# Ruslan361/iterative_solvers

Hardware: AMD Instinct MI355X
Metric: cg_iters_per_sec (higher is better)
Workload: dtype f64; 1 GPU; 4096x4096 L-shaped Dirichlet Poisson fp64, matrix-free CG, fixed 2641 iterations; n=4096, unknowns=12574721, rule=rel2

## Files before the change

### include/mi355cg.h

```cpp
#ifndef MI355CG_H
#define MI355CG_H

#include <stddef.h>

#ifdef __cplusplus
extern "C" {
#endif

#define MI355CG_OK            0
#define MI355CG_ERR_INVALID   1
#define MI355CG_ERR_HIP       2
#define MI355CG_ERR_STATE     3

#define MI355CG_F64           0
#define MI355CG_F32_MIXED     1

#define MI355CG_RULE_MSG_MAXNORM  0
#define MI355CG_RULE_REL_2NORM    1

#define MI355CG_STOP_ITERATIONS   0
#define MI355CG_STOP_PRECISION    1
#define MI355CG_STOP_RESIDUAL     2
#define MI355CG_STOP_EXACT_ERROR  3
#define MI355CG_STOP_INTERRUPTED  4

typedef struct mi355cg_ctx *mi355cg_handle;

typedef void (*mi355cg_iter_cb)(void *user, int iteration, double precision, double residual, double error);

typedef struct mi355cg_params {
    int    rule;
    int    max_iterations;
    double eps_precision;
    double eps_residual;
    double eps_exact_error;
    double eps_rel;
    int    use_true_solution;
    int    callback_every;
    int    diagnostics;
    int    sync_every;
    int    fixed_iterations;
    double inner_eps;
} mi355cg_params;

typedef struct mi355cg_results {
    int    iterations;
    int    converged;
    int    stop_reason;
    double final_residual_norm;
    double final_precision;
    double final_error_norm;
    double r_norm2;
    double initial_r_norm2;
    double solve_seconds;
    double refine_true_rel;
    int    refine_outer;
    double loop_seconds;
} mi355cg_results;

int  mi355cg_create(int n, int m, double a, double b, double c, double d,
                    int dtype, int device, mi355cg_handle *out);
int  mi355cg_create_csr(long long nrows, const int *row_map, const int *entries, const double *values,
                        int device, mi355cg_handle *out);
int  mi355cg_set_true_solution(mi355cg_handle h, const double *u);
void mi355cg_destroy(mi355cg_handle h);
const char *mi355cg_last_error(void);
const char *mi355cg_version(void);

long long mi355cg_size(mi355cg_handle h);
int  mi355cg_get_rhs(mi355cg_handle h, double *out);
int  mi355cg_get_true_solution(mi355cg_handle h, double *out);
int  mi355cg_get_node_coords(mi355cg_handle h, double *xs, double *ys);
int  mi355cg_set_rhs(mi355cg_handle h, const double *b);
int  mi355cg_setup_on_device(mi355cg_handle h);

int  mi355cg_apply(mi355cg_handle h, const double *x, double *y);
int  mi355cg_apply_device(mi355cg_handle h, const double *x_dev, double *y_dev);

void mi355cg_default_params(mi355cg_params *p, int rule);
int  mi355cg_solve(mi355cg_handle h, const mi355cg_params *params,
                   mi355cg_iter_cb cb, void *user, const volatile int *stop_flag,
                   mi355cg_results *out);
int  mi355cg_get_solution(mi355cg_handle h, double *x);
int  mi355cg_get_recursive_residual(mi355cg_handle h, double *r);
int  mi355cg_get_true_residual(mi355cg_handle h, double *ax_minus_b);

int  mi355cg_set_profiling(mi355cg_handle h, int enable);
int  mi355cg_get_kernel_time(mi355cg_handle h, int kernel, double *avg_ms, long long *launches);
int  mi355cg_get_layout(mi355cg_handle h, long long *padded_len, int *pitch_bottom, int *pitch_upper,
                        int *grid_stencil, int *grid_update, int *rows_per_item);

int  mi355cg_slab_rows(int n, int world, int rank, int *y_lo, int *y_hi);
int  mi355cg_create_part(int n, int m, double a, double b, double c, double d, int dtype, int device,
                         int y_lo, int y_hi, int x_lo, int x_hi, mi355cg_handle *out);
int  mi355cg_checksum(mi355cg_handle h, int which, double *out2);
int  mi355cg_create_slab(int n, int m, double a, double b, double c, double d, int dtype, int device,
                         int y_lo, int y_hi, mi355cg_handle *out);
int  mi355cg_owned_range(mi355cg_handle h, long long *packed_begin, long long *packed_len, int *y_lo, int *y_hi);
int  mi355cg_dist_begin(mi355cg_handle h, const mi355cg_params *params, void *stream);
int  mi355cg_dist_reduce(mi355cg_handle h, int which , int with_rows, void *stream);
int  mi355cg_dist_sums_ptr(mi355cg_handle h, int which, void **dev_ptr, int *count );
int  mi355cg_dist_record_layout(mi355cg_handle h, int *header, int *row_slot, int *width);
int  mi355cg_dist_scatter_ghosts(mi355cg_handle h, int vector ,
                                 const double *gathered_records, int nranks, int rank, void *stream);
int  mi355cg_dist_stencil(mi355cg_handle h, const double *gathered_update_sums, int nranks, int estride,
                          int rows , void *stream);
int  mi355cg_dist_flip(mi355cg_handle h);
int  mi355cg_dist_update(mi355cg_handle h, const double *gathered_stencil_sums, int nranks, int estride,
                         int rows , void *stream);
int  mi355cg_dist_update_reads_ghosts(mi355cg_handle h);
int  mi355cg_dist_check(mi355cg_handle h, const double *gathered_update_sums, int nranks, int estride, void *stream);
int  mi355cg_dist_summary(mi355cg_handle h, mi355cg_results *out, int *done);
int  mi355cg_dist_finish(mi355cg_handle h, void *stream);
int  mi355cg_dist_history(mi355cg_handle h, int iteration, double *precision, double *residual, double *error);
int  mi355cg_dist_halo(mi355cg_handle h, int vector ,
                       void **send_lo, void **recv_lo, long long *n_send_lo,
                       void **send_hi, void **recv_hi, long long *n_send_hi);
int  mi355cg_dist_halo_recv_counts(mi355cg_handle h, long long *n_from_lo, long long *n_from_hi);

#define MI355CG_DECOMP_ROWS 0
#define MI355CG_DECOMP_2D   1
typedef struct mi355cg_team_s *mi355cg_team;
typedef struct mi355cg_halo_msg {
    int id;
    int peer;
    int send;
    int kind;
    int y0, y1, x0, x1;
    long long count;
} mi355cg_halo_msg;
int  mi355cg_decompose(int n, int world, int decomp, int rank, int *y_lo, int *y_hi, int *x_lo, int *x_hi);
int  mi355cg_halo_plan(int n, int world, int decomp, int rank, int max_msgs, int *n_msgs, mi355cg_halo_msg *msgs);
int  mi355cg_debug_plan(int n, int world, int decomp, int rank, int which, int *n_panels, int *panels,
                        int *grid, int *n_items, int *cls);
int  mi355cg_team_create_local(int n, int m, double a, double b, double c, double d, int world,
                               const int *devices, int ndevices, int decomp, mi355cg_team *out);
int  mi355cg_team_unique_id(void *id128);
int  mi355cg_team_create_rccl(int n, int m, double a, double b, double c, double d, int world, int rank, int device,
                              const void *id128, int decomp, mi355cg_team *out);
void mi355cg_team_destroy(mi355cg_team t);
int  mi355cg_team_solve(mi355cg_team t, const mi355cg_params *params, mi355cg_iter_cb cb, void *user,
                        const volatile int *stop_flag, mi355cg_results *out);
int  mi355cg_team_info(mi355cg_team t, int *world, int *nlocal, int *decomp, long long *size);
int  mi355cg_team_describe(mi355cg_team t, char *buf, int len);
int  mi355cg_team_part(mi355cg_team t, int local_index, mi355cg_handle *part, int *rank);
int  mi355cg_team_get_vector(mi355cg_team t, int which, double *global_packed);
int  mi355cg_team_checksum(mi355cg_team t, int which, double *out2);
int  mi355cg_team_set_vector(mi355cg_team t, int which, const double *global_packed);
int  mi355cg_team_set_dtype(mi355cg_team t, int dtype);
int  mi355cg_team_setup_on_device(mi355cg_team t);
int  mi355cg_team_set_profiling(mi355cg_team t, int enable);
int  mi355cg_team_phase_times(mi355cg_team t, double *kernel_ms, double *comm_ms, double *wall_ms);

#ifdef __cplusplus
}
#endif
#endif
```

### iterative_solvers_amd/_capi.py

```python
from __future__ import annotations

import ctypes as C
import os

import numpy as np

from . import build as _build

OK, ERR_INVALID, ERR_HIP, ERR_STATE = 0, 1, 2, 3
F64, F32_MIXED = 0, 1
RULE_MSG_MAXNORM, RULE_REL_2NORM = 0, 1
STOP_ITERATIONS, STOP_PRECISION, STOP_RESIDUAL, STOP_EXACT_ERROR, STOP_INTERRUPTED = range(5)

EXPORTS = [
    "mi355cg_create", "mi355cg_create_csr", "mi355cg_set_true_solution", "mi355cg_destroy", "mi355cg_last_error", "mi355cg_version", "mi355cg_size",
    "mi355cg_get_rhs", "mi355cg_get_true_solution", "mi355cg_get_node_coords", "mi355cg_set_rhs",
    "mi355cg_apply", "mi355cg_apply_device", "mi355cg_default_params", "mi355cg_solve",
    "mi355cg_get_solution", "mi355cg_get_recursive_residual", "mi355cg_get_true_residual",
    "mi355cg_set_profiling", "mi355cg_get_kernel_time", "mi355cg_get_layout",
    "mi355cg_slab_rows", "mi355cg_create_slab", "mi355cg_owned_range", "mi355cg_dist_begin",
    "mi355cg_dist_reduce", "mi355cg_dist_sums_ptr", "mi355cg_dist_record_layout", "mi355cg_dist_scatter_ghosts", "mi355cg_dist_stencil", "mi355cg_dist_flip",
    "mi355cg_dist_update", "mi355cg_dist_update_reads_ghosts", "mi355cg_dist_check", "mi355cg_dist_summary", "mi355cg_dist_finish", "mi355cg_dist_history",
    "mi355cg_dist_halo", "mi355cg_dist_halo_recv_counts",
    "mi355cg_create_part", "mi355cg_checksum", "mi355cg_decompose", "mi355cg_halo_plan",
    "mi355cg_team_create_local", "mi355cg_team_unique_id", "mi355cg_team_create_rccl", "mi355cg_team_destroy",
    "mi355cg_team_solve", "mi355cg_team_info", "mi355cg_team_part", "mi355cg_team_get_vector", "mi355cg_team_set_vector", "mi355cg_team_checksum",
    "mi355cg_team_set_profiling", "mi355cg_team_phase_times", "mi355cg_team_describe", "mi355cg_setup_on_device", "mi355cg_team_setup_on_device", "mi355cg_debug_plan",
    "mi355cg_team_set_dtype",
]
DECOMP_ROWS, DECOMP_2D = 0, 1


class Params(C.Structure):
    _fields_ = [("rule", C.c_int), ("max_iterations", C.c_int),
                ("eps_precision", C.c_double), ("eps_residual", C.c_double),
                ("eps_exact_error", C.c_double), ("eps_rel", C.c_double),
                ("use_true_solution", C.c_int), ("callback_every", C.c_int),
                ("diagnostics", C.c_int), ("sync_every", C.c_int), ("fixed_iterations", C.c_int),
                ("inner_eps", C.c_double)]


class Results(C.Structure):
    _fields_ = [("iterations", C.c_int), ("converged", C.c_int), ("stop_reason", C.c_int),
                ("final_residual_norm", C.c_double), ("final_precision", C.c_double),
                ("final_error_norm", C.c_double), ("r_norm2", C.c_double),
                ("initial_r_norm2", C.c_double), ("solve_seconds", C.c_double),
                ("refine_true_rel", C.c_double), ("refine_outer", C.c_int), ("loop_seconds", C.c_double)]


class HaloMsg(C.Structure):
    _fields_ = [("id", C.c_int), ("peer", C.c_int), ("send", C.c_int), ("kind", C.c_int),
                ("y0", C.c_int), ("y1", C.c_int), ("x0", C.c_int), ("x1", C.c_int), ("count", C.c_longlong)]


ITER_CB = C.CFUNCTYPE(None, C.c_void_p, C.c_int, C.c_double, C.c_double, C.c_double)
_DP = np.ctypeslib.ndpointer(dtype=np.float64, flags="C_CONTIGUOUS")

_lib = None


class Mi355cgError(RuntimeError):
    def __init__(self, code: int, text: str):
        super().__init__(f"mi355cg error {code}: {text}")
        self.code = code


def lib_path() -> str:
    return _build.LIB_PATH


def load():
    global _lib
    if _lib is not None:
        return _lib
    path = os.environ.get("MI355CG_LIB") or _build.LIB_PATH
    if path == _build.LIB_PATH and _build.needs_build():
        try:
            _build.build()
        except Exception as e:
            if not os.path.exists(path):
                raise RuntimeError(f"libmi355cg.so is missing and could not be built: {e}") from e
    try:
        import torch
    except ImportError:
        pass
    L = C.CDLL(path)
    H = C.c_void_p
    L.mi355cg_create.argtypes = [C.c_int, C.c_int] + [C.c_double] * 4 + [C.c_int, C.c_int, C.POINTER(H)]
    _IPn = np.ctypeslib.ndpointer(dtype=np.int32, flags="C_CONTIGUOUS")
    L.mi355cg_create_csr.argtypes = [C.c_longlong, _IPn, _IPn, _DP, C.c_int, C.POINTER(H)]
    L.mi355cg_set_true_solution.argtypes = [H, _DP]
    L.mi355cg_destroy.argtypes = [H]
    L.mi355cg_destroy.restype = None
    L.mi355cg_last_error.restype = C.c_char_p
    L.mi355cg_version.restype = C.c_char_p
    L.mi355cg_size.argtypes = [H]
    L.mi355cg_size.restype = C.c_longlong
    for name in ("mi355cg_get_rhs", "mi355cg_get_true_solution", "mi355cg_set_rhs",
                 "mi355cg_get_solution", "mi355cg_get_recursive_residual", "mi355cg_get_true_residual"):
        getattr(L, name).argtypes = [H, _DP]
    L.mi355cg_get_node_coords.argtypes = [H, _DP, _DP]
    L.mi355cg_apply.argtypes = [H, _DP, _DP]
    L.mi355cg_apply_device.argtypes = [H, C.c_void_p, C.c_void_p]
    L.mi355cg_default_params.argtypes = [C.POINTER(Params), C.c_int]
    L.mi355cg_default_params.restype = None
    L.mi355cg_solve.argtypes = [H, C.POINTER(Params), ITER_CB, C.c_void_p, C.c_void_p, C.POINTER(Results)]
    L.mi355cg_set_profiling.argtypes = [H, C.c_int]
    L.mi355cg_get_kernel_time.argtypes = [H, C.c_int, C.POINTER(C.c_double), C.POINTER(C.c_longlong)]
    L.mi355cg_get_layout.argtypes = [H, C.POINTER(C.c_longlong)] + [C.POINTER(C.c_int)] * 5
    LLP, IP, VPP = C.POINTER(C.c_longlong), C.POINTER(C.c_int), C.POINTER(C.c_void_p)
    L.mi355cg_slab_rows.argtypes = [C.c_int, C.c_int, C.c_int, IP, IP]
    L.mi355cg_create_slab.argtypes = [C.c_int, C.c_int] + [C.c_double] * 4 + [C.c_int] * 4 + [C.POINTER(H)]
    L.mi355cg_owned_range.argtypes = [H, LLP, LLP, IP, IP]
    L.mi355cg_dist_begin.argtypes = [H, C.POINTER(Params), C.c_void_p]
    L.mi355cg_dist_reduce.argtypes = [H, C.c_int, C.c_int, C.c_void_p]
    L.mi355cg_dist_sums_ptr.argtypes = [H, C.c_int, VPP, IP]
    L.mi355cg_dist_record_layout.argtypes = [H, IP, IP, IP]
    L.mi355cg_dist_scatter_ghosts.argtypes = [H, C.c_int, C.c_void_p, C.c_int, C.c_int, C.c_void_p]
    L.mi355cg_dist_stencil.argtypes = [H, C.c_void_p, C.c_int, C.c_int, C.c_int, C.c_void_p]
    L.mi355cg_dist_flip.argtypes = [H]
    L.mi355cg_dist_update.argtypes = [H, C.c_void_p, C.c_int, C.c_int, C.c_int, C.c_void_p]
    L.mi355cg_dist_update_reads_ghosts.argtypes = [H]
    L.mi355cg_dist_check.argtypes = [H, C.c_void_p, C.c_int, C.c_int, C.c_void_p]
    L.mi355cg_dist_summary.argtypes = [H, C.POINTER(Results), IP]
    L.mi355cg_dist_finish.argtypes = [H, C.c_void_p]
    DBP = C.POINTER(C.c_double)
    L.mi355cg_dist_history.argtypes = [H, C.c_int, DBP, DBP, DBP]
    L.mi355cg_dist_halo.argtypes = [H, C.c_int, VPP, VPP, LLP, VPP, VPP, LLP]
    L.mi355cg_dist_halo_recv_counts.argtypes = [H, LLP, LLP]
    L.mi355cg_create_part.argtypes = [C.c_int, C.c_int] + [C.c_double] * 4 + [C.c_int] * 6 + [C.POINTER(H)]
    L.mi355cg_checksum.argtypes = [H, C.c_int, DBP]
    L.mi355cg_decompose.argtypes = [C.c_int] * 4 + [IP] * 4
    L.mi355cg_halo_plan.argtypes = [C.c_int] * 5 + [IP, C.POINTER(HaloMsg)]
    L.mi355cg_team_create_local.argtypes = [C.c_int, C.c_int] + [C.c_double] * 4 + [C.c_int, IP, C.c_int, C.c_int, C.POINTER(H)]
    L.mi355cg_team_unique_id.argtypes = [C.c_void_p]
    L.mi355cg_team_create_rccl.argtypes = [C.c_int, C.c_int] + [C.c_double] * 4 + [C.c_int, C.c_int, C.c_int, C.c_void_p, C.c_int, C.POINTER(H)]
    L.mi355cg_team_destroy.argtypes = [H]
    L.mi355cg_team_destroy.restype = None
    L.mi355cg_team_solve.argtypes = [H, C.POINTER(Params), ITER_CB, C.c_void_p, C.c_void_p, C.POINTER(Results)]
    L.mi355cg_team_info.argtypes = [H, IP, IP, IP, LLP]
    L.mi355cg_team_part.argtypes = [H, C.c_int, C.POINTER(H), IP]
    L.mi355cg_team_get_vector.argtypes = [H, C.c_int, _DP]
    L.mi355cg_team_set_vector.argtypes = [H, C.c_int, _DP]
    L.mi355cg_team_checksum.argtypes = [H, C.c_int, DBP]
    L.mi355cg_debug_plan.argtypes = [C.c_int] * 5 + [IP, IP, IP, IP, IP]
    L.mi355cg_setup_on_device.argtypes = [H]
    L.mi355cg_team_setup_on_device.argtypes = [H]
    L.mi355cg_team_set_dtype.argtypes = [H, C.c_int]
    L.mi355cg_team_set_profiling.argtypes = [H, C.c_int]
    L.mi355cg_team_phase_times.argtypes = [H, DBP, DBP, DBP]
    L.mi355cg_team_describe.argtypes = [H, C.c_char_p, C.c_int]
    _lib = L
    return L


def check(rc: int):
    if rc != OK:
        raise Mi355cgError(rc, load().mi355cg_last_error().decode("utf-8", "replace"))
```

### iterative_solvers_amd/csrc/cg_kernels.h

```cpp
#pragma once
#include <hip/hip_runtime.h>
#include <cfloat>
#include <cmath>

namespace mi355cg {

constexpr int kBlock = 256;
constexpr int kWave = 64;
constexpr int kWaves = kBlock / kWave;
constexpr int kHist = 512;
constexpr int kMaxPanels = 8;
constexpr int kRing = 8;

#ifdef MI355CG_WAVE_TIMING
constexpr int kWtWaves = 16384, kWtStamps = 6;
__device__ unsigned long long g_wave_dbg[2][kWtStamps * kWtWaves];
#define MI355CG_WT_BEGIN unsigned long long wt_[kWtStamps]; for (int i_ = 0; i_ < kWtStamps; ++i_) wt_[i_] = 0; wt_[0] = wall_clock64();
#define MI355CG_WT_STAMP(I) wt_[I] = wall_clock64();
#define MI355CG_WT_MID wt_[kWtStamps - 2] = wall_clock64();
#define MI355CG_WT_END(K) do { if ((threadIdx.x & 63) == 0) { const int w_ = blockIdx.x * 4 + threadIdx.x / 64; \
    if (w_ < kWtWaves) { wt_[kWtStamps - 1] = wall_clock64(); for (int i_ = 0; i_ < kWtStamps; ++i_) g_wave_dbg[K][kWtStamps * w_ + i_] = wt_[i_]; } } } while (0)
#else
#define MI355CG_WT_BEGIN
#define MI355CG_WT_STAMP(I)
#define MI355CG_WT_MID
#define MI355CG_WT_END(K)
#endif

struct Geom {
    int N, half, cb, xlim;
    int Pb, Pu;
    int y_lo, y_hi;
    long long base0;
    long long own_begin, own_len;
    double A, xk, yk;
};

__host__ __device__ inline long long row_off(const Geom& g, int y) {
    return y <= g.half ? (long long)y * g.Pb - g.cb
                       : (long long)(g.half + 1) * g.Pb + (long long)(y - g.half - 1) * g.Pu;
}
__host__ __device__ inline bool node_interior(const Geom& g, int x, int y) {
    return y >= 1 && y <= g.N - 1 && x <= g.N - 1 && x >= (y <= g.half ? g.half + 1 : 1);
}

struct Panel { int y0, y1, s0, ns, ty, nchunks, item0, gc; };
constexpr int kXcds = 8;
struct WorkList { Panel p[kMaxPanels]; int np; int nitems; int ncls; int cls0[kXcds + 1]; };
struct ItemSeq { int first, step, begin, end; };
__device__ inline ItemSeq item_seq(const WorkList& wl, int wave) {
    if (wl.ncls == kXcds) {
        const int cls = blockIdx.x % kXcds, nb = (gridDim.x - cls + kXcds - 1) / kXcds;
        int begin = wl.cls0[0], end = wl.cls0[1];
#pragma unroll
        for (int k = 1; k < kXcds; ++k) if (k == cls) { begin = wl.cls0[k]; end = wl.cls0[k + 1]; }
        return ItemSeq{begin + (int)(blockIdx.x / kXcds) * kWaves + wave, nb * kWaves, begin, end};
    }
    return ItemSeq{(int)blockIdx.x * kWaves + wave, (int)gridDim.x * kWaves, 0, wl.nitems};
}

struct CgState {
    double alpha, beta;
    double rr;
    double rr_prev;
    double rz;
    double r0norm;
    double rnorm2;
    double rmax, dmax, emax, d2, e2;
    int it, done, reason, converged, first;
    int stop;
    double alpha_hist[kRing];
};
struct HistEntry { double dmax, rmax, emax, rnorm2, d2, e2, tr2; };

struct StateLite { double alpha, rr, rr_prev, rz, r0norm; int it, done, first, stop; };
template <typename V> __device__ inline V scalar_load(const V* p) {
    return *(const __attribute__((address_space(4))) V*)p;
}
__device__ __attribute__((noinline)) void copy_state(CgState* dst, const CgState* src) { *dst = *src; }
__device__ inline StateLite load_state_lite(const CgState* p) {
    StateLite L;
    L.alpha = scalar_load(&p->alpha); L.rr = scalar_load(&p->rr); L.rr_prev = scalar_load(&p->rr_prev);
    L.rz = scalar_load(&p->rz); L.r0norm = scalar_load(&p->r0norm);
    L.it = scalar_load(&p->it); L.done = scalar_load(&p->done); L.first = scalar_load(&p->first); L.stop = scalar_load(&p->stop);
    return L;
}

struct RuleParams {
    int rule;
    int max_iterations;
    double eps_precision, eps_residual, eps_exact_error, eps_rel;
    int use_u;
    int fixed_iterations;
};

enum { FA_PAP = 0, FA_RZ = 1, FA_LO = 2, FA_COUNT = 4 };
enum { FB_RR = 0, FB_D2 = 1, FB_E2 = 2, FB_LO = 3, FB_RMAX = 6, FB_DMAX = 7, FB_EMAX = 8, FB_COUNT = 9 };
constexpr int kNumSumsA = 2, kNumSumsB = 3;
constexpr int FB_STOP = FB_COUNT, FB_LL_COUNT = FB_COUNT + 1;

struct dd { double hi, lo; };
__device__ inline dd dd_zero() { return dd{0.0, 0.0}; }
__device__ inline dd two_sum(double a, double b) { const double s = a + b, bb = s - a; return dd{s, (a - (s - bb)) + (b - bb)}; }
__device__ inline dd dd_add(dd a, dd b) {
    const dd s = two_sum(a.hi, b.hi);
    const double lo = s.lo + (a.lo + b.lo);
    const double hi = s.hi + lo;
    return dd{hi, lo - (hi - s.hi)};
}
__device__ inline void dd_acc_prod(dd& acc, double a, double b) {
#ifdef MI355CG_PLAIN_DOT
    acc.hi += a * b;
#elif defined(MI355CG_DOT2)
    const double p = a * b;
    const dd s = two_sum(acc.hi, p);
    acc.hi = s.hi;
    acc.lo += s.lo + fma(a, b, -p);
#else
    const double p = a * b;
    acc = dd_add(acc, dd{p, fma(a, b, -p)});
#endif
}
__device__ inline double dd_value(dd a) { return a.hi + a.lo; }

__device__ inline double wave_sum(double v) {
#pragma unroll
    for (int o = 32; o > 0; o >>= 1) v += __shfl_down(v, o, kWave);
    return v;
}
__device__ inline double wave_max(double v) {
#pragma unroll
    for (int o = 32; o > 0; o >>= 1) v = fmax(v, __shfl_down(v, o, kWave));
    return v;
}
template <bool IS_MAX>
__device__ inline double block_reduce(double v, double* lds ) {
    v = IS_MAX ? wave_max(v) : wave_sum(v);
    const int lane = threadIdx.x & (kWave - 1), w = threadIdx.x / kWave;
    __syncthreads();
    if (lane == 0) lds[w] = v;
    __syncthreads();
    double t = lds[0];
// ... 3 lines not shown
}
template <bool IS_MAX>
__device__ inline double reduce_parts(const double* __restrict__ part, int n, int es, double* lds) {
    double v = 0.0;
    for (int i = threadIdx.x; i < n; i += kBlock) v = IS_MAX ? fmax(v, part[(long long)i * es]) : v + part[(long long)i * es];
    return block_reduce<IS_MAX>(v, lds);
}

__device__ inline dd wave_sum_dd(dd v) {
#pragma unroll
    for (int o = 32; o > 0; o >>= 1) v = dd_add(v, dd{__shfl_down(v.hi, o, kWave), __shfl_down(v.lo, o, kWave)});
    return v;
}
__device__ inline dd block_reduce_dd(dd v, double* lds) {
    v = wave_sum_dd(v);
    const int lane = threadIdx.x & (kWave - 1), w = threadIdx.x / kWave;
    __syncthreads();
    if (lane == 0) { lds[2 * w] = v.hi; lds[2 * w + 1] = v.lo; }
    __syncthreads();
    dd t{lds[0], lds[1]};
#pragma unroll
    for (int k = 1; k < kWaves; ++k) t = dd_add(t, dd{lds[2 * k], lds[2 * k + 1]});
    return t;
}
struct PreParts { double hi0, lo0, hi1, lo1; };
__device__ inline PreParts prefetch_parts(const double* __restrict__ part_hi, const double* __restrict__ part_lo, int n, int es) {
    PreParts p{0.0, 0.0, 0.0, 0.0};
    const int i0 = threadIdx.x, i1 = threadIdx.x + kBlock;
    if (i0 < n) { p.hi0 = part_hi[(long long)i0 * es]; p.lo0 = part_lo[(long long)i0 * es]; }
    if (i1 < n) { p.hi1 = part_hi[(long long)i1 * es]; p.lo1 = part_lo[(long long)i1 * es]; }
    return p;
}
__device__ inline dd reduce_parts_dd_pre(const PreParts& pre, const double* __restrict__ part_hi, const double* __restrict__ part_lo, int n, int es, double* lds) {
    dd v = dd_zero();
    if ((int)threadIdx.x < n) v = dd_add(v, dd{pre.hi0, pre.lo0});
    if ((int)threadIdx.x + kBlock < n) v = dd_add(v, dd{pre.hi1, pre.lo1});
    for (int i = threadIdx.x + 2 * kBlock; i < n; i += kBlock) v = dd_add(v, dd{part_hi[(long long)i * es], part_lo[(long long)i * es]});
    return block_reduce_dd(v, lds);
}
struct PreMax { double v0, v1; };
__device__ inline PreMax prefetch_max(const double* __restrict__ part, int n, int es) {
    PreMax p{0.0, 0.0};
    if ((int)threadIdx.x < n) p.v0 = part[(long long)threadIdx.x * es];
    if ((int)threadIdx.x + kBlock < n) p.v1 = part[(long long)(threadIdx.x + kBlock) * es];
    return p;
}
template <bool IS_MAX> __device__ inline double block_reduce(double v, double* lds);
__device__ inline double reduce_max_pre(const PreMax& pre, const double* __restrict__ part, int n, int es, double* lds) {
    double v = fmax(pre.v0, pre.v1);
    for (int i = threadIdx.x + 2 * kBlock; i < n; i += kBlock) v = fmax(v, part[(long long)i * es]);
    return block_reduce<true>(v, lds);
}
__device__ inline dd reduce_parts_dd(const double* __restrict__ part_hi, const double* __restrict__ part_lo, int n, int es, double* lds) {
    dd v = dd_zero();
    for (int i = threadIdx.x; i < n; i += kBlock) v = dd_add(v, dd{part_hi[(long long)i * es], part_lo[(long long)i * es]});
    return block_reduce_dd(v, lds);
}

struct Decision { int done, reason, converged; double beta, rr, rnorm2, r0norm, rmax, dmax, emax, d2, e2; };

__device__ inline Decision decide_after_update(const StateLite& s, const RuleParams& rp, double rr, double rmax,
                                               double dmax, double emax, double d2, double e2, bool stop = false) {
    Decision d;
    d.rr = rr; d.rnorm2 = sqrt(rr); d.rmax = rmax; d.dmax = dmax; d.emax = emax; d.d2 = d2; d.e2 = e2;
    d.r0norm = s.first ? d.rnorm2 : s.r0norm;
    d.done = 0; d.reason = 0 ; d.converged = 0; d.beta = 0.0;
    if (rp.rule == 1 ) {
        const bool go = s.it < rp.max_iterations && (rp.fixed_iterations || d.rnorm2 > rp.eps_rel * d.r0norm);
        if (!go) { d.done = 1; d.converged = d.rnorm2 <= rp.eps_rel * d.r0norm; }
        if (!s.first) d.beta = rr / s.rr;
    } else {
        if (s.it >= 1 && !rp.fixed_iterations) {
            if (rp.eps_precision > 0 && dmax < rp.eps_precision) { d.done = 1; d.converged = 1; d.reason = 1; }
            else if (rp.eps_residual > 0 && rmax < rp.eps_residual) { d.done = 1; d.converged = 1; d.reason = 2; }
            else if (rp.eps_exact_error > 0 && rp.use_u && emax < rp.eps_exact_error) { d.done = 1; d.converged = 1; d.reason = 3; }
        }
        if (!d.done && !(s.it < rp.max_iterations)) d.done = 1;
        if (!s.first) d.beta = (d.rnorm2 * d.rnorm2) / s.rz;
    }
    if (!d.done && (stop || s.stop)) { d.done = 1; d.reason = 4 ; d.converged = 0; }
    return d;
}

__device__ inline void write_state_after_decision(CgState* out, HistEntry* hist, const CgState* in, const StateLite& s, const Decision& d) {
    copy_state(out, in);
    CgState* o = out;
    o->rr_prev = s.rr; o->rr = d.rr; o->rnorm2 = d.rnorm2; o->r0norm = d.r0norm; o->beta = d.beta;
    o->rmax = d.rmax; o->dmax = d.dmax; o->emax = d.emax; o->d2 = d.d2; o->e2 = d.e2;
    o->done = d.done; o->reason = d.reason; o->converged = d.converged;
    if (hist) {
        HistEntry* h = hist + (s.it % kHist);
        h->dmax = d.dmax; h->rmax = d.rmax; h->emax = d.emax; h->rnorm2 = d.rnorm2; h->d2 = d.d2; h->e2 = d.e2;
    }
}

__device__ inline Decision reduce_and_decide(const StateLite& s, const RuleParams& rp, const double* partB,
                                             int nB, int strideB, int esB, int want_diag, double* lds, const PreParts* pre_rr = nullptr,
                                             const PreMax* pre_max = nullptr ) {
    const double rr = pre_rr ? dd_value(reduce_parts_dd_pre(*pre_rr, partB + FB_RR * strideB, partB + (FB_RR + FB_LO) * strideB, nB, esB, lds))
                             : dd_value(reduce_parts_dd(partB + FB_RR * strideB, partB + (FB_RR + FB_LO) * strideB, nB, esB, lds));
    double rmax = 0, dmax = 0, emax = 0, d2 = 0, e2 = 0;
    if (rp.rule == 0 || want_diag) {
        if (pre_max) {
            rmax = reduce_max_pre(pre_max[0], partB + FB_RMAX * strideB, nB, esB, lds);
            dmax = reduce_max_pre(pre_max[1], partB + FB_DMAX * strideB, nB, esB, lds);
            if (rp.use_u) emax = reduce_max_pre(pre_max[2], partB + FB_EMAX * strideB, nB, esB, lds);
        } else {
            rmax = reduce_parts<true>(partB + FB_RMAX * strideB, nB, esB, lds);
            dmax = reduce_parts<true>(partB + FB_DMAX * strideB, nB, esB, lds);
            if (rp.use_u) emax = reduce_parts<true>(partB + FB_EMAX * strideB, nB, esB, lds);
        }
    }
    if (want_diag) {
        d2 = dd_value(reduce_parts_dd(partB + FB_D2 * strideB, partB + (FB_D2 + FB_LO) * strideB, nB, esB, lds));
        if (rp.use_u) e2 = dd_value(reduce_parts_dd(partB + FB_E2 * strideB, partB + (FB_E2 + FB_LO) * strideB, nB, esB, lds));
    }
    return decide_after_update(s, rp, rr, rmax, dmax, emax, d2, e2);
}
typedef unsigned long long u64;
constexpr int kRecWords = 16;
constexpr int kLLWords = 2 * kRecWords;
constexpr int kRecStopWord = 9;
constexpr int kMaxRecDst = 16;
constexpr int kReasonTransport = 5;
constexpr int kMaxPartSlots = 1024;
__device__ inline u64 ld_sys(const u64* p) { return __hip_atomic_load(p, __ATOMIC_RELAXED, __HIP_MEMORY_SCOPE_SYSTEM); }
__device__ inline void st_sys(u64* p, u64 v) { __hip_atomic_store(p, v, __ATOMIC_RELAXED, __HIP_MEMORY_SCOPE_SYSTEM); }
__device__ inline u64 flagged(unsigned stamp, unsigned data) { return ((u64)stamp << 32) | data; }

struct FlagSpec {
    u64* part;
    unsigned stamp;
};
__device__ inline void store_flagged(const FlagSpec& fs, int slot, int nfields, const double* v) {
    u64* w = fs.part + (long long)slot * (2 * nfields);
    for (int f = 0; f < nfields; ++f) {
        const u64 bits = __builtin_bit_cast(u64, v[f]);
        st_sys(w + 2 * f, flagged(fs.stamp, (unsigned)bits));
        st_sys(w + 2 * f + 1, flagged(fs.stamp, (unsigned)(bits >> 32)));
    }
}
__device__ inline void store_flagged_zero(const FlagSpec& fs, int slot, int nfields) {
    if (!fs.part) return;
    u64* w = fs.part + (long long)slot * (2 * nfields);
    for (int k = 0; k < 2 * nfields; ++k) st_sys(w + k, flagged(fs.stamp, 0u));
}

struct RecSpec {
    int ndst;
    u64* const* dst;
    u64* const* flag;
    int slot_words;
    int slot;
    unsigned seq;
    u64 flag_value;
};
struct RecSrc {
    const u64* mbox;
    int world, me;
    unsigned stamp;
    u64 budget;
};
__device__ inline bool gather_records(const RecSrc& src, double* recs) {
    unsigned* out = reinterpret_cast<unsigned*>(recs);
    const int n = src.world * kLLWords;
    int bad = 0;
    for (int i = threadIdx.x; i < n; i += kBlock) {
        if (i / kLLWords == src.me) continue;
        u64 v = ld_sys(src.mbox + i);
        if ((unsigned)(v >> 32) != src.stamp) {
            const u64 t0 = wall_clock64();
            unsigned spins = 0;
            for (;;) {
                __builtin_amdgcn_s_sleep(2);
                v = ld_sys(src.mbox + i);
                if ((unsigned)(v >> 32) == src.stamp) break;
// ... 181 lines not shown
    if constexpr (sizeof(V) == 16) return __builtin_bit_cast(V, __builtin_amdgcn_raw_buffer_load_b128(r, voff, soff, 0));
    else if constexpr (sizeof(V) == 8) return __builtin_bit_cast(V, __builtin_amdgcn_raw_buffer_load_b64(r, voff, soff, 0));
    else { static_assert(sizeof(V) == 4, "buf_load: 4, 8 or 16 bytes"); return __builtin_bit_cast(V, __builtin_amdgcn_raw_buffer_load_b32(r, voff, soff, 0)); }
}
template <typename V> __device__ inline void buf_store(V v, rsrc_t r, int voff, int soff) {
    typedef unsigned int u4 __attribute__((ext_vector_type(4)));
    typedef unsigned int u2 __attribute__((ext_vector_type(2)));
    if constexpr (sizeof(V) == 16) {
        u4 d = __builtin_bit_cast(u4, v);
        __builtin_amdgcn_raw_buffer_store_b128(d, r, voff, soff, 0);
        asm volatile("s_nop 1" : "+v"(d));
    }
    else if constexpr (sizeof(V) == 8) __builtin_amdgcn_raw_buffer_store_b64(__builtin_bit_cast(u2, v), r, voff, soff, 0);
    else { static_assert(sizeof(V) == 4, "buf_store: 4, 8 or 16 bytes"); __builtin_amdgcn_raw_buffer_store_b32(__builtin_bit_cast(unsigned int, v), r, voff, soff, 0); }
}
__device__ inline int dpp_from_below(int v) { return __builtin_amdgcn_update_dpp(0, v, 0x138 , 0xf, 0xf, false); }
__device__ inline int dpp_from_above(int v) { return __builtin_amdgcn_update_dpp(0, v, 0x130 , 0xf, 0xf, false); }
__device__ inline float lane_below(float v) { return __builtin_bit_cast(float, dpp_from_below(__builtin_bit_cast(int, v))); }
__device__ inline float lane_above(float v) { return __builtin_bit_cast(float, dpp_from_above(__builtin_bit_cast(int, v))); }
__device__ inline double lane_below(double v) {
    const unsigned long long u = __builtin_bit_cast(unsigned long long, v);
    const unsigned lo = (unsigned)dpp_from_below((int)(unsigned)u), hi = (unsigned)dpp_from_below((int)(unsigned)(u >> 32));
    return __builtin_bit_cast(double, ((unsigned long long)hi << 32) | lo);
}
__device__ inline double lane_above(double v) {
    const unsigned long long u = __builtin_bit_cast(unsigned long long, v);
    const unsigned lo = (unsigned)dpp_from_above((int)(unsigned)u), hi = (unsigned)dpp_from_above((int)(unsigned)(u >> 32));
    return __builtin_bit_cast(double, ((unsigned long long)hi << 32) | lo);
}
template <typename T> __device__ inline int row_step(const Geom& g, int y) { return (y + 1 <= g.half ? g.Pb : g.Pu) * (int)sizeof(T); }

template <typename T> __device__ inline int lane_off(const Geom& g, int x, bool bottom_row) {
    return (x < g.xlim && x >= (bottom_row ? g.cb : 0)) ? x * (int)sizeof(T) : kOob;
}
template <typename T, int VEC> __device__ inline int edge_off(const Geom& g, int x, int lane, bool bottom_row) {
    const int xe = lane == 0 ? x - 1 : x + VEC;
    const bool edge = lane == 0 || lane == kWave - 1;
    return (edge && xe >= (bottom_row ? g.cb : 0) && xe < g.xlim) ? xe * (int)sizeof(T) : kOob;
}

struct Item { int strip, ya, yb, gc; };
__device__ inline Item decode_item(const WorkList& wl, int item) {
    Panel P = wl.p[0];
#pragma unroll
    for (int k = 1; k < kMaxPanels; ++k) if (k < wl.np && item >= wl.p[k].item0) P = wl.p[k];
    const int local = item - P.item0;
    const int chunk = local / P.ns;
    Item it;
    it.strip = P.s0 + (local - chunk * P.ns);
    it.ya = P.y0 + chunk * P.ty;
    it.yb = min(P.y1, it.ya + P.ty - 1);
    it.gc = (it.strip == P.s0 ? (P.gc & 1) : 0) | (it.strip == P.s0 + P.ns - 1 ? (P.gc & 2) : 0);
    return it;
}

struct ItemAddr {
    int nrows, ystart;
    long long base_el;
    int so_first, so_c0;
    int gc; bool bot;
    int x;
    int vo_own, ve_own, vo_first, vo_last;
};
template <typename T, int VEC, bool DESC>
__device__ inline ItemAddr item_addr(const Geom& g, const Item& it, int lane) {
    constexpr int DIR = DESC ? -1 : 1;
    ItemAddr A;
    A.x = it.strip * (kWave * VEC) + lane * VEC;
    A.nrows = it.yb - it.ya + 1;
    A.ystart = DESC ? it.yb : it.ya;
    const int y0 = it.ya - 1;
    A.base_el = row_off(g, y0) - g.base0;
    A.bot = it.ya <= g.half;
    A.vo_own = lane_off<T>(g, A.x, A.bot);
    A.ve_own = edge_off<T, VEC>(g, A.x, lane, A.bot);
    A.vo_first = lane_off<T>(g, A.x, A.ystart - DIR <= g.half);
    A.vo_last = lane_off<T>(g, A.x, A.ystart + DIR * A.nrows <= g.half);
    A.so_first = DESC ? (int)((row_off(g, it.yb + 1) - row_off(g, y0)) * (long long)sizeof(T)) : 0;
    A.so_c0 = DESC ? (int)((row_off(g, it.yb) - row_off(g, y0)) * (long long)sizeof(T)) : row_step<T>(g, y0);
    A.gc = it.gc;
    return A;
}

template <typename T, int VEC, bool FUSED, bool MSG, int DEPTH, bool NOAP, bool GC>
__global__ __launch_bounds__(kBlock) void k_stencil(const StencilArgs<T> a) {
    static_assert(DEPTH >= 1 && DEPTH <= 3, "the compute cursor takes its item from the fetch cursor: DEPTH <= rows fetched per item (>= 3)");
    typedef typename VecOf<T, VEC>::type vec_t;
    __shared__ double lds[2 * kWaves];
    const Geom& g = a.g;
    const int lane = threadIdx.x & (kWave - 1);
    const int wave = __builtin_amdgcn_readfirstlane(threadIdx.x / kWave);
    const ItemSeq seq = item_seq(a.wl, wave);
    MI355CG_WT_BEGIN
    struct Raw { vec_t r, p; T re, pe; };

    int f_item = seq.first;
    bool f_have = f_item < seq.end;
    ItemAddr F{};
    int f_idx = 0, f_so = 0, f_y = 0;
    rsrc_t rs_p = make_rsrc(a.pin), rs_r = make_rsrc(a.pin);
    const int dq_nsub = min(kQueueSubs, (int)(gridDim.x / kXcds)), dq_sub = (int)(blockIdx.x / kXcds) % dq_nsub;
    int* const dq = a.dq.mine ? a.dq.mine + ((int)(blockIdx.x % kXcds) * kQueueSubs + dq_sub) * kQueuePitch : nullptr;
    if (a.dq.other && blockIdx.x == 0 && threadIdx.x < kXcds * kQueueSubs) a.dq.other[threadIdx.x * kQueuePitch] = 0;
    int dq_ticket = 0;
    auto enter = [&](int item) {
        if (dq) dq_ticket = queue_take(dq, lane);
        F = item_addr<T, VEC, false>(g, decode_item(a.wl, item), lane);
        rs_p = make_rsrc(a.pin + F.base_el);
        rs_r = make_rsrc(FUSED ? a.r + F.base_el : a.pin + F.base_el);
        f_idx = -1; f_so = F.so_first; f_y = F.ystart - 1;
    };
    auto fetch = [&]() -> Raw {
        if (f_have && f_idx > F.nrows) {
            f_item = dq ? seq.begin + seq.step + __builtin_amdgcn_readfirstlane(dq_ticket) * dq_nsub + dq_sub : f_item + seq.step;
            f_have = f_item < seq.end;
            if (f_have) enter(f_item);
        }
        const bool own = f_idx >= 0 && f_idx < F.nrows;
        int vo = own ? F.vo_own : (f_idx < 0 ? F.vo_first : F.vo_last);
        int ve = own ? F.ve_own : kOob;
        if (!f_have) { vo = kOob; ve = kOob; }
        Raw w;
        w.p = buf_load<vec_t>(rs_p, vo, f_so);
        if (FUSED) w.r = buf_load<vec_t>(rs_r, vo, f_so);
        else for (int j = 0; j < VEC; ++j) w.r[j] = (T)0;
        w.pe = buf_load<T>(rs_p, ve, f_so);
        if (FUSED) w.re = buf_load<T>(rs_r, ve, f_so); else w.re = (T)0;
        f_so += row_step<T>(g, f_y); ++f_y; ++f_idx;
        return w;
    };

    bool c_have = f_have;
    ItemAddr C{};
    int c_idx = -1, c_so = 0, c_y = 0, c_ve_gc = kOob;
    bool in_j[VEC];
#pragma unroll
    for (int j = 0; j < VEC; ++j) in_j[j] = false;
    rsrc_t rs_po = make_rsrc(a.pin), rs_ap = make_rsrc(a.pin);
    auto promote = [&]() {
        C = F;
        rs_po = make_rsrc(FUSED ? a.pout + C.base_el : a.pin + C.base_el);
        rs_ap = make_rsrc(NOAP ? a.pin + C.base_el : a.ap + C.base_el);
        c_idx = -1; c_so = C.so_c0; c_y = C.ystart;
        const int xint0 = C.bot ? g.half + 1 : 1;
#pragma unroll
        for (int j = 0; j < VEC; ++j) in_j[j] = (C.x + j >= xint0) && (C.x + j <= g.N - 1);
        if (GC) c_ve_gc = ((lane == 0 && (C.gc & 1)) || (lane == kWave - 1 && (C.gc & 2))) ? C.ve_own : kOob;
    };

    if (f_have) { enter(f_item); promote(); }
    Raw q[DEPTH];
#pragma unroll
    for (int k = 0; k < DEPTH; ++k) q[k] = fetch();

    T beta = (T)0;
    if (FUSED && a.src.mbox) {
        __shared__ double recs[kMaxRecDst * kRecWords];
        const PreParts pre = prefetch_parts(a.partB + FB_RR * a.strideB, a.partB + (FB_RR + FB_LO) * a.strideB, a.nB, 1);
        PreMax pmax[3] = {{0, 0}, {0, 0}, {0, 0}};
        if (MSG) {
#pragma unroll
            for (int k = 0; k < 3; ++k) pmax[k] = prefetch_max(a.partB + (FB_RMAX + k) * a.strideB, a.nB, 1);
        }
        const StateLite s = load_state_lite(a.s_in);
        if (s.done) {
            if (threadIdx.x == 0) { store_flagged_zero(a.fl, a.slotA + blockIdx.x, FA_COUNT); if (blockIdx.x == 0) copy_state(a.s_out, a.s_in); }
            return;
        }
        MI355CG_WT_STAMP(1)
        own_record_B(recs, a.src.me, a.partB, a.nB, a.strideB, MSG ? 1 : 0, lds, &pre, MSG ? pmax : nullptr);
        if (!gather_records(a.src, recs)) {
            if (threadIdx.x == 0) { store_flagged_zero(a.fl, a.slotA + blockIdx.x, FA_COUNT); if (blockIdx.x == 0) fail_transport(a.s_out, a.s_in); }
            return;
        }
        const Decision d = decide_from_records(s, a.rp, recs, a.src.world, MSG, false);
        MI355CG_WT_STAMP(2)
        if (blockIdx.x == 0 && threadIdx.x == 0) write_state_after_decision(a.s_out, a.hist, a.s_in, s, d);
        if (d.done) { if (threadIdx.x == 0) store_flagged_zero(a.fl, a.slotA + blockIdx.x, FA_COUNT); return; }
        beta = (T)d.beta;
    } else if (FUSED) {
        const PreParts pre = prefetch_parts(a.partB + FB_RR * a.strideB, a.partB + (FB_RR + FB_LO) * a.strideB, a.nB, a.esB);
        PreMax pmax[3] = {{0, 0}, {0, 0}, {0, 0}};
        if (MSG) {
#pragma unroll
            for (int k = 0; k < 3; ++k) pmax[k] = prefetch_max(a.partB + (FB_RMAX + k) * a.strideB, a.nB, a.esB);
        }
        const StateLite s = load_state_lite(a.s_in);
        if (s.done) { if (blockIdx.x == 0 && threadIdx.x == 0) copy_state(a.s_out, a.s_in); return; }
        MI355CG_WT_STAMP(1)
        const Decision d = reduce_and_decide(s, a.rp, a.partB, a.nB, a.strideB, a.esB, a.want_diag, lds, &pre, MSG ? pmax : nullptr);
        MI355CG_WT_STAMP(2)
        if (blockIdx.x == 0 && threadIdx.x == 0) write_state_after_decision(a.s_out, a.hist, a.s_in, s, d);
        if (d.done) return;
        beta = (T)d.beta;
    }

    MI355CG_WT_MID
    const T cA = (T)g.A, cxk = (T)g.xk, cyk = (T)g.yk;
    dd acc_pap = dd_zero(), acc_rz = dd_zero();
    auto is_ghost = [&](int yy) { return (yy == g.y_lo - 1 || yy == g.y_hi + 1) && yy >= 1 && yy <= g.N - 1; };
    vec_t pn_b, pn_c, r_c;
    T pne_c = (T)0;
#pragma unroll
    for (int j = 0; j < VEC; ++j) { pn_b[j] = (T)0; pn_c[j] = (T)0; r_c[j] = (T)0; }

    while (c_have) {
#pragma unroll
        for (int k = 0; k < DEPTH; ++k) {
            if (c_have) {
                const Raw w = q[k];
                q[k] = fetch();
                vec_t pn; T pne;
                if (FUSED) {
#pragma unroll
                    for (int j = 0; j < VEC; ++j) pn[j] = w.r[j] + beta * w.p[j];
                    pne = w.re + beta * w.pe;
                } else { pn = w.p; pne = w.pe; }

                if (c_idx < 0) {
                    pn_b = pn;
                    if (FUSED && a.store_ghosts && is_ghost(C.ystart - 1)) buf_store(pn, rs_po, C.vo_first, C.so_first);
                } else if (c_idx == 0) {
                    pn_c = pn; pne_c = pne; r_c = w.r;
                } else {
                    T left0 = lane_below(pn_c[VEC - 1]);
                    T rightL = lane_above(pn_c[0]);
                    if (lane == 0) left0 = pne_c;
                    if (lane == kWave - 1) rightL = pne_c;
                    vec_t out;
#pragma unroll
                    for (int j = 0; j < VEC; ++j) {
                        const T c = pn_c[j];
                        const T L = j == 0 ? left0 : pn_c[j - 1];
                        const T R = j == VEC - 1 ? rightL : pn_c[j + 1];
                        T v = cA * c;
                        v = v + cxk * L;
                        v = v + cxk * R;
                        v = v + cyk * pn[j];
                        v = v + cyk * pn_b[j];
                        out[j] = in_j[j] ? v : (T)0;
                        dd_acc_prod(acc_pap, (double)c, (double)out[j]);
                        if (MSG) dd_acc_prod(acc_rz, (double)r_c[j], (double)c);
                    }
                    if (!NOAP) buf_store(out, rs_ap, C.vo_own, c_so);
                    if (FUSED) buf_store(pn_c, rs_po, C.vo_own, c_so);
                    if (FUSED && GC) buf_store(pne_c, rs_po, c_ve_gc, c_so);
                    c_so += row_step<T>(g, c_y); ++c_y;
                    pn_b = pn_c; pn_c = pn; pne_c = pne; r_c = w.r;
                }
                if (c_idx == C.nrows) {
                    if (FUSED && a.store_ghosts && is_ghost(c_y)) buf_store(pn, rs_po, C.vo_last, c_so);
                    c_have = f_have;
                    if (c_have) promote();
                } else ++c_idx;
            }
        }
    }

    MI355CG_WT_END(0);
    const dd tp = block_reduce_dd(acc_pap, lds);
    dd tz = dd_zero();
    if (MSG) tz = block_reduce_dd(acc_rz, lds);
    if (threadIdx.x == 0 && a.partA) {
        const int b = a.slotA + blockIdx.x, st = a.strideA;
        a.partA[FA_PAP * st + b] = tp.hi; a.partA[(FA_PAP + FA_LO) * st + b] = tp.lo;
        a.partA[FA_RZ * st + b] = tz.hi;  a.partA[(FA_RZ + FA_LO) * st + b] = tz.lo;
        if (FUSED && a.fl.part) { const double v[FA_COUNT] = {tp.hi, tz.hi, tp.lo, tz.lo}; store_flagged(a.fl, b, FA_COUNT, v); }
    }
}

template <typename T>
struct UpdateArgs {
    long long begin, nvec;
    T* x; T* r; const T* p; const T* ap; const T* u;
    const double* partA; int nA, strideA, esA;
    double* partB; int strideB;
    const CgState* s_in; CgState* s_out;
    int rule;
    int init;
    double r0norm_resume;
};

template <typename T, int VEC, bool HAS_U>
__global__ __launch_bounds__(kBlock) void k_update(const UpdateArgs<T> a) {
    typedef typename VecOf<T, VEC>::type vec_t;
    __shared__ double lds[2 * kWaves];
    StateLite s{};
    double alpha_d = 0.0, rz = 0.0;
    if (a.init == 1) {
        s.first = 1; s.it = 0;
    } else if (a.init == 2) {
        s = load_state_lite(a.s_in);
    } else {
        s = load_state_lite(a.s_in);
        if (s.done) { if (blockIdx.x == 0 && threadIdx.x == 0) copy_state(a.s_out, a.s_in); return; }
        const double pap = dd_value(reduce_parts_dd(a.partA + FA_PAP * a.strideA, a.partA + (FA_PAP + FA_LO) * a.strideA, a.nA, a.esA, lds));
        if (a.rule == 0) {
            rz = dd_value(reduce_parts_dd(a.partA + FA_RZ * a.strideA, a.partA + (FA_RZ + FA_LO) * a.strideA, a.nA, a.esA, lds));
            alpha_d = rz / pap;
        } else {
            alpha_d = s.rr / pap;
        }
    }
    const T alpha = (T)alpha_d;

    dd s_rr = dd_zero(), s_d2 = dd_zero(), s_e2 = dd_zero();
    double s_rmax = 0, s_dmax = 0, s_emax = 0;
    const long long stride = (long long)gridDim.x * kBlock;
    vec_t* __restrict__ X = reinterpret_cast<vec_t*>(a.x);
    vec_t* __restrict__ R = reinterpret_cast<vec_t*>(a.r);
    const vec_t* __restrict__ Pp = reinterpret_cast<const vec_t*>(a.p);
    const vec_t* __restrict__ Q = reinterpret_cast<const vec_t*>(a.ap);
    const vec_t* __restrict__ Uu = reinterpret_cast<const vec_t*>(a.u);

    auto elem = [&](long long i, const vec_t& x0, const vec_t& pv, const vec_t& r0, const vec_t& qv, const vec_t& uv) {
        vec_t xn, rn;
#pragma unroll
        for (int j = 0; j < VEC; ++j) {
            xn[j] = x0[j] + alpha * pv[j];
            rn[j] = r0[j] - alpha * qv[j];
            const double rd = (double)rn[j];
            dd_acc_prod(s_rr, rd, rd);
            s_rmax = fmax(s_rmax, fabs(rd));
            const double dx = (double)(xn[j] - x0[j]);
            s_dmax = fmax(s_dmax, fabs(dx));
            dd_acc_prod(s_d2, dx, dx);
            if (HAS_U) {
                const double ee = (double)(xn[j] - uv[j]);
                s_emax = fmax(s_emax, fabs(ee));
                dd_acc_prod(s_e2, ee, ee);
            }
        }
        X[i] = xn; R[i] = rn;
    };
    long long i = a.begin + (long long)blockIdx.x * kBlock + threadIdx.x;
    const long long end = a.begin + a.nvec;
    for (; i + stride < end; i += 2 * stride) {
        const long long j0 = i, j1 = i + stride;
        const vec_t xa = X[j0], pa = Pp[j0], ra = R[j0], qa = Q[j0];
        const vec_t xb = X[j1], pb = Pp[j1], rb = R[j1], qb = Q[j1];
// ... 27 lines not shown
            } else {
                copy_state(a.s_out, a.s_in);
                if (a.init == 2) {
                    if (s.done) o->rr = s.rr_prev;
                    o->done = 0; o->reason = 0; o->converged = 0; o->alpha = 0.0; o->r0norm = a.r0norm_resume;
                    for (int i = 0; i < kRing; ++i) o->alpha_hist[i] = 0.0;
                } else { o->it = s.it + 1; o->first = 0; o->alpha = alpha_d; o->rz = rz; o->alpha_hist[(s.it + 1) & (kRing - 1)] = alpha_d; }
            }
        }
    }
}

template <typename T>
struct FreshArgs {
    long long begin, nvec;
    const T* b; T* x; T* r; T* p0; const T* u;
    double* partB; int strideB;
    CgState* s_out;
};
template <typename T, int VEC, bool HAS_U>
__global__ __launch_bounds__(kBlock) void k_init_fresh(const FreshArgs<T> a) {
    typedef typename VecOf<T, VEC>::type vec_t;
    __shared__ double lds[2 * kWaves];
    dd s_rr = dd_zero(), s_e2 = dd_zero();
    double s_rmax = 0, s_emax = 0;
    const long long stride = (long long)gridDim.x * kBlock;
    const vec_t* __restrict__ B = reinterpret_cast<const vec_t*>(a.b);
    const vec_t* __restrict__ Uu = reinterpret_cast<const vec_t*>(a.u);
    vec_t* __restrict__ X = reinterpret_cast<vec_t*>(a.x);
    vec_t* __restrict__ R = reinterpret_cast<vec_t*>(a.r);
    vec_t* __restrict__ P = reinterpret_cast<vec_t*>(a.p0);
    vec_t zero;
#pragma unroll
    for (int j = 0; j < VEC; ++j) zero[j] = (T)0;
    const long long end = a.begin + a.nvec;
    for (long long i = a.begin + (long long)blockIdx.x * kBlock + threadIdx.x; i < end; i += stride) {
        const vec_t bv = B[i];
        vec_t uv; if (HAS_U) uv = Uu[i];
#pragma unroll
        for (int j = 0; j < VEC; ++j) {
            const double rd = (double)bv[j];
            dd_acc_prod(s_rr, rd, rd);
            s_rmax = fmax(s_rmax, fabs(rd));
            if (HAS_U) {
                const double ee = (double)((T)0 - uv[j]);
                s_emax = fmax(s_emax, fabs(ee));
                dd_acc_prod(s_e2, ee, ee);
            }
        }
        X[i] = zero; R[i] = bv; P[i] = zero;
    }
    const dd t_rr = block_reduce_dd(s_rr, lds);
    const double t_rmax = block_reduce<true>(s_rmax, lds);
    double t_emax = 0; dd t_e2 = dd_zero();
    if (HAS_U) { t_emax = block_reduce<true>(s_emax, lds); t_e2 = block_reduce_dd(s_e2, lds); }
    if (threadIdx.x == 0) {
        const int b = blockIdx.x, st = a.strideB;
        a.partB[FB_RR * st + b] = t_rr.hi; a.partB[(FB_RR + FB_LO) * st + b] = t_rr.lo;
        a.partB[FB_D2 * st + b] = 0.0; a.partB[(FB_D2 + FB_LO) * st + b] = 0.0;
        a.partB[FB_E2 * st + b] = t_e2.hi; a.partB[(FB_E2 + FB_LO) * st + b] = t_e2.lo;
        a.partB[FB_RMAX * st + b] = t_rmax; a.partB[FB_DMAX * st + b] = 0.0; a.partB[FB_EMAX * st + b] = t_emax;
        if (blockIdx.x == 0) { *a.s_out = CgState{}; a.s_out->first = 1; }
    }
}

template <typename T>
struct UpdateStArgs {
    Geom g;
    WorkList wl;
    const T* p;
    const T* pprev[kRing - 1];
    T* r; T* x; const T* u;
    const double* partA; int nA, strideA, esA;
    RecSrc src;
    double* partB; int strideB, slotB;
    const CgState* s_in; CgState* s_out;
    int rule;
    int reverse;
    const int* stop_req;
    FlagSpec fl;
    QueueSpec dq;
};

template <typename T, int VEC, int XM, bool HAS_U, int DEPTH, bool DESC>
__global__ __launch_bounds__(kBlock) void k_update_st(const UpdateStArgs<T> a) {
    static_assert(DEPTH >= 1 && DEPTH <= 3, "see k_stencil");
    typedef typename VecOf<T, VEC>::type vec_t;
    __shared__ double lds[2 * kWaves];
    const Geom& g = a.g;
    const int lane = threadIdx.x & (kWave - 1);
    const int wave = __builtin_amdgcn_readfirstlane(threadIdx.x / kWave);
    const ItemSeq seq = item_seq(a.wl, wave);
    MI355CG_WT_BEGIN
    int stop_word = 0;
    if (blockIdx.x == 0 && a.stop_req) stop_word = scalar_load(a.stop_req);
    constexpr bool FULL = XM == 1;
    constexpr int NP = XM >= 2 ? XM - 1 : 0;
    struct Raw { vec_t p, r, x, u, pp[NP > 0 ? NP : 1]; T pe; };

    int f_item = seq.first;
    bool f_have = f_item < seq.end;
    ItemAddr F{};
    int f_idx = 0, f_so = 0, f_y = 0;
    rsrc_t rs_p = make_rsrc(a.p), rs_r = rs_p, rs_x = rs_p, rs_u = rs_p;
    rsrc_t rs_pp[NP > 0 ? NP : 1] = {rs_p};
    const int dq_nsub = min(kQueueSubs, (int)(gridDim.x / kXcds)), dq_sub = (int)(blockIdx.x / kXcds) % dq_nsub;
    int* const dq = a.dq.mine ? a.dq.mine + ((int)(blockIdx.x % kXcds) * kQueueSubs + dq_sub) * kQueuePitch : nullptr;
    if (a.dq.other && blockIdx.x == 0 && threadIdx.x < kXcds * kQueueSubs) a.dq.other[threadIdx.x * kQueuePitch] = 0;
    int dq_ticket = 0;
    auto enter = [&](int idx) {
        if (dq) dq_ticket = queue_take(dq, lane);
        F = item_addr<T, VEC, DESC>(g, decode_item(a.wl, a.reverse ? seq.end - 1 - (idx - seq.begin) : idx), lane);
        rs_p = make_rsrc(a.p + F.base_el);
        rs_r = make_rsrc(a.r + F.base_el);
        rs_x = make_rsrc(XM != 0 ? a.x + F.base_el : a.p + F.base_el);
#pragma unroll
        for (int i = 0; i < NP; ++i) rs_pp[i] = make_rsrc(a.pprev[i] + F.base_el);
        rs_u = make_rsrc((FULL && HAS_U) ? a.u + F.base_el : a.p + F.base_el);
        f_idx = -1; f_so = F.so_first; f_y = DESC ? F.ystart + 1 : F.ystart - 1;
    };
    auto fetch = [&]() -> Raw {
        if (f_have && f_idx > F.nrows) {
            f_item = dq ? seq.begin + seq.step + __builtin_amdgcn_readfirstlane(dq_ticket) * dq_nsub + dq_sub : f_item + seq.step;
            f_have = f_item < seq.end;
            if (f_have) enter(f_item);
        }
        const bool own = f_have && f_idx >= 0 && f_idx < F.nrows;
        int vo = own ? F.vo_own : (f_idx < 0 ? F.vo_first : F.vo_last);
        if (!f_have) vo = kOob;
        const int vown = own ? F.vo_own : kOob;
        Raw w;
        w.p = buf_load<vec_t>(rs_p, vo, f_so);
        w.r = buf_load<vec_t>(rs_r, vown, f_so);
        if (XM != 0) w.x = buf_load<vec_t>(rs_x, vown, f_so);
#pragma unroll
        for (int i = 0; i < NP; ++i) w.pp[i] = buf_load<vec_t>(rs_pp[i], vown, f_so);
        if (FULL && HAS_U) w.u = buf_load<vec_t>(rs_u, vown, f_so);
        w.pe = buf_load<T>(rs_p, own ? F.ve_own : kOob, f_so);
        if (DESC) { f_so -= row_step<T>(g, f_y - 1); --f_y; } else { f_so += row_step<T>(g, f_y); ++f_y; }
        ++f_idx;
        return w;
    };

    bool c_have = f_have;
    ItemAddr C{};
    int c_idx = -1, c_so = 0, c_y = 0;
    bool in_j[VEC];
#pragma unroll
    for (int j = 0; j < VEC; ++j) in_j[j] = false;
    rsrc_t rs_ro = rs_p, rs_xo = rs_p;
    auto promote = [&]() {
        C = F;
        rs_ro = make_rsrc(a.r + C.base_el);
        rs_xo = make_rsrc(XM != 0 ? a.x + C.base_el : a.p + C.base_el);
        c_idx = -1; c_so = C.so_c0; c_y = C.ystart;
        const int xint0 = C.bot ? g.half + 1 : 1;
#pragma unroll
        for (int j = 0; j < VEC; ++j) in_j[j] = (C.x + j >= xint0) && (C.x + j <= g.N - 1);
    };

    if (f_have) { enter(f_item); promote(); }
    Raw q[DEPTH];
#pragma unroll
    for (int k = 0; k < DEPTH; ++k) q[k] = fetch();

    double alpha_d, rz = 0.0;
    StateLite s;
    if (a.src.mbox) {
        __shared__ double recs[kMaxRecDst * kRecWords];
        const PreParts pre = prefetch_parts(a.partA + FA_PAP * a.strideA, a.partA + (FA_PAP + FA_LO) * a.strideA, a.nA, 1);
        PreParts pre_rz{0, 0, 0, 0};
        if (FULL) pre_rz = prefetch_parts(a.partA + FA_RZ * a.strideA, a.partA + (FA_RZ + FA_LO) * a.strideA, a.nA, 1);
        s = load_state_lite(a.s_in);
        if (s.done) {
            if (threadIdx.x == 0) { store_flagged_zero(a.fl, a.slotB + blockIdx.x, FB_LL_COUNT); if (blockIdx.x == 0) copy_state(a.s_out, a.s_in); }
            return;
        }
        {
            double* R = recs + a.src.me * kRecWords;
            if (threadIdx.x < kRecWords) R[threadIdx.x] = 0.0;
            const dd pap = reduce_parts_dd_pre(pre, a.partA + FA_PAP * a.strideA, a.partA + (FA_PAP + FA_LO) * a.strideA, a.nA, 1, lds);
            dd rzd = dd_zero();
            if (a.rule == 0) rzd = FULL ? reduce_parts_dd_pre(pre_rz, a.partA + FA_RZ * a.strideA, a.partA + (FA_RZ + FA_LO) * a.strideA, a.nA, 1, lds)
                                        : reduce_parts_dd(a.partA + FA_RZ * a.strideA, a.partA + (FA_RZ + FA_LO) * a.strideA, a.nA, 1, lds);
            __syncthreads();
            if (threadIdx.x == 0) { R[FA_PAP] = pap.hi; R[FA_PAP + FA_LO] = pap.lo; R[FA_RZ] = rzd.hi; R[FA_RZ + FA_LO] = rzd.lo; }
        }
        if (!gather_records(a.src, recs)) {
            if (threadIdx.x == 0) { store_flagged_zero(a.fl, a.slotB + blockIdx.x, FB_LL_COUNT); if (blockIdx.x == 0) fail_transport(a.s_out, a.s_in); }
            return;
        }
        alpha_from_records(s, a.rule, recs, a.src.world, &alpha_d, &rz);
    } else {
        const PreParts pre = prefetch_parts(a.partA + FA_PAP * a.strideA, a.partA + (FA_PAP + FA_LO) * a.strideA, a.nA, a.esA);
        PreParts pre_rz{0, 0, 0, 0};
        if (FULL) pre_rz = prefetch_parts(a.partA + FA_RZ * a.strideA, a.partA + (FA_RZ + FA_LO) * a.strideA, a.nA, a.esA);
        s = load_state_lite(a.s_in);
        if (s.done) { if (blockIdx.x == 0 && threadIdx.x == 0) copy_state(a.s_out, a.s_in); return; }
        const double pap = dd_value(reduce_parts_dd_pre(pre, a.partA + FA_PAP * a.strideA, a.partA + (FA_PAP + FA_LO) * a.strideA, a.nA, a.esA, lds));
        if (a.rule == 0) {
            rz = FULL ? dd_value(reduce_parts_dd_pre(pre_rz, a.partA + FA_RZ * a.strideA, a.partA + (FA_RZ + FA_LO) * a.strideA, a.nA, a.esA, lds))
                      : dd_value(reduce_parts_dd(a.partA + FA_RZ * a.strideA, a.partA + (FA_RZ + FA_LO) * a.strideA, a.nA, a.esA, lds));
            alpha_d = rz / pap;
        } else {
            alpha_d = s.rr / pap;
        }
    }
    const T alpha = (T)alpha_d;
    MI355CG_WT_MID
    T aprev[NP > 0 ? NP : 1] = {(T)0};
#pragma unroll
    for (int i = 0; i < NP; ++i) aprev[i] = (T)scalar_load(&a.s_in->alpha_hist[(s.it - i) & (kRing - 1)]);
    const T cA = (T)g.A, cxk = (T)g.xk, cyk = (T)g.yk;
    dd s_rr = dd_zero(), s_d2 = dd_zero(), s_e2 = dd_zero();
    double s_rmax = 0, s_dmax = 0, s_emax = 0;
    vec_t p_b;
    Raw c;
#pragma unroll
    for (int j = 0; j < VEC; ++j) { p_b[j] = (T)0; c.p[j] = (T)0; c.r[j] = (T)0; c.x[j] = (T)0; c.u[j] = (T)0; for (int i = 0; i < (NP > 0 ? NP : 1); ++i) c.pp[i][j] = (T)0; }
    c.pe = (T)0;

    while (c_have) {
#pragma unroll
        for (int k = 0; k < DEPTH; ++k) {
            if (c_have) {
                const Raw w = q[k];
                q[k] = fetch();
                if (c_idx < 0) {
                    p_b = w.p;
                } else if (c_idx == 0) {
                    c = w;
                } else {
                    T left0 = lane_below(c.p[VEC - 1]);
                    T rightL = lane_above(c.p[0]);
                    if (lane == 0) left0 = c.pe;
                    if (lane == kWave - 1) rightL = c.pe;
                    const vec_t& top = DESC ? p_b : w.p;
                    const vec_t& bot = DESC ? w.p : p_b;
                    vec_t rn, xn;
#pragma unroll
                    for (int j = 0; j < VEC; ++j) {
                        const T cc = c.p[j];
                        const T L = j == 0 ? left0 : c.p[j - 1];
                        const T R = j == VEC - 1 ? rightL : c.p[j + 1];
                        T v = cA * cc;
                        v = v + cxk * L;
                        v = v + cxk * R;
                        v = v + cyk * top[j];
                        v = v + cyk * bot[j];
                        const T apj = in_j[j] ? v : (T)0;
                        rn[j] = c.r[j] - alpha * apj;
                        const double rd = (double)rn[j];
                        dd_acc_prod(s_rr, rd, rd);
                        s_rmax = fmax(s_rmax, fabs(rd));
                        if (XM >= 2) {
                            T t = c.x[j];
#pragma unroll
                            for (int i = NP - 1; i >= 0; --i) t = t + aprev[i] * c.pp[i][j];
                            xn[j] = t + alpha * cc;
                        }
                        if (FULL) {
                            xn[j] = c.x[j] + alpha * cc;
                            const double dx = (double)(xn[j] - c.x[j]);
                            s_dmax = fmax(s_dmax, fabs(dx));
                            dd_acc_prod(s_d2, dx, dx);
                            if (HAS_U) {
                                const double ee = (double)(xn[j] - c.u[j]);
                                s_emax = fmax(s_emax, fabs(ee));
                                dd_acc_prod(s_e2, ee, ee);
                            }
                        }
                    }
                    buf_store(rn, rs_ro, C.vo_own, c_so);
                    if (XM != 0) buf_store(xn, rs_xo, C.vo_own, c_so);
                    if (DESC) { c_so -= row_step<T>(g, c_y - 1); --c_y; } else { c_so += row_step<T>(g, c_y); ++c_y; }
                    p_b = c.p; c = w;
                }
                if (c_idx == C.nrows) {
                    c_have = f_have;
                    if (c_have) promote();
                } else ++c_idx;
            }
        }
    }

    MI355CG_WT_END(1);
    const dd t_rr = block_reduce_dd(s_rr, lds);
    const double t_rmax = block_reduce<true>(s_rmax, lds);
    double t_dmax = 0, t_emax = 0; dd t_d2 = dd_zero(), t_e2 = dd_zero();
    if (FULL) { t_dmax = block_reduce<true>(s_dmax, lds); t_d2 = block_reduce_dd(s_d2, lds); }
    if (FULL && HAS_U) { t_emax = block_reduce<true>(s_emax, lds); t_e2 = block_reduce_dd(s_e2, lds); }
    if (threadIdx.x == 0) {
        const int b = a.slotB + blockIdx.x, st = a.strideB;
        a.partB[FB_RR * st + b] = t_rr.hi; a.partB[(FB_RR + FB_LO) * st + b] = t_rr.lo;
        a.partB[FB_D2 * st + b] = t_d2.hi; a.partB[(FB_D2 + FB_LO) * st + b] = t_d2.lo;
        a.partB[FB_E2 * st + b] = t_e2.hi; a.partB[(FB_E2 + FB_LO) * st + b] = t_e2.lo;
        a.partB[FB_RMAX * st + b] = t_rmax; a.partB[FB_DMAX * st + b] = t_dmax; a.partB[FB_EMAX * st + b] = t_emax;
        if (a.fl.part) {
            const double v[FB_LL_COUNT] = {t_rr.hi, t_d2.hi, t_e2.hi, t_rr.lo, t_d2.lo, t_e2.lo, t_rmax, t_dmax, t_emax, (blockIdx.x == 0 && stop_word) ? 1.0 : 0.0};
            store_flagged(a.fl, b, FB_LL_COUNT, v);
        }
        if (blockIdx.x == 0) {
            copy_state(a.s_out, a.s_in);
            CgState* o = a.s_out;
            o->it = s.it + 1; o->first = 0; o->alpha = alpha_d; o->rz = rz; o->alpha_hist[(s.it + 1) & (kRing - 1)] = alpha_d;
            o->stop = stop_word != 0;
        }
    }
}

struct CheckArgs {
    const double* partB; int nB, strideB, esB;
    RecSrc src;
    const CgState* s_in;
    CgState* summary;
    HistEntry* hist;
    RuleParams rp;
    int want_diag;
};
__global__ __launch_bounds__(kBlock) void k_check(const CheckArgs a) {
    __shared__ double lds[2 * kWaves];
    const StateLite s = load_state_lite(a.s_in);
    if (s.done) { if (threadIdx.x == 0) copy_state(a.summary, a.s_in); return; }
    Decision d;
    if (a.src.mbox) {
        __shared__ double recs[kMaxRecDst * kRecWords];
        own_record_B(recs, a.src.me, a.partB, a.nB, a.strideB, 2, lds);
        if (!gather_records(a.src, recs)) { if (threadIdx.x == 0) fail_transport(a.summary, a.s_in); return; }
        d = decide_from_records(s, a.rp, recs, a.src.world, true, true);
    } else d = reduce_and_decide(s, a.rp, a.partB, a.nB, a.strideB, a.esB, 1, lds);
    if (threadIdx.x == 0) write_state_after_decision(a.summary, a.hist, a.s_in, s, d);
}

template <typename T> struct FlushArgs { const T* p[kRing - 1]; T a[kRing - 1]; int n; };
template <typename T, int VEC>
__global__ __launch_bounds__(kBlock) void k_flush_x(const Geom g, const WorkList wl, T* x, const FlushArgs<T> f) {
    typedef typename VecOf<T, VEC>::type vec_t;
    const int lane = threadIdx.x & (kWave - 1);
    const int wave = __builtin_amdgcn_readfirstlane(threadIdx.x / kWave);
    for (int item = blockIdx.x * kWaves + wave; item < wl.nitems; item += gridDim.x * kWaves) {
        const Item it = decode_item(wl, item);
        const int x0 = it.strip * (kWave * VEC) + lane * VEC;
        if (x0 < (it.ya <= g.half ? g.cb : 0) || x0 >= g.xlim) continue;
        for (int y = it.ya; y <= it.yb; ++y) {
            const long long off = row_off(g, y) - g.base0 + x0;
            vec_t xn = *reinterpret_cast<const vec_t*>(x + off);
#pragma unroll
            for (int k = 0; k < kRing - 1; ++k) if (k < f.n) {
                const vec_t pv = *reinterpret_cast<const vec_t*>(f.p[k] + off);
#pragma unroll
                for (int j = 0; j < VEC; ++j) xn[j] = xn[j] + f.a[k] * pv[j];
            }
            *reinterpret_cast<vec_t*>(x + off) = xn;
        }
    }
}

template <typename T, int VEC>
__global__ __launch_bounds__(kBlock) void k_checksum(const Geom g, const WorkList wl, const T* v, double* part) {
    typedef typename VecOf<T, VEC>::type vec_t;
    __shared__ double lds[2 * kWaves];
    const int lane = threadIdx.x & (kWave - 1);
    const int wave = __builtin_amdgcn_readfirstlane(threadIdx.x / kWave);
    dd s1 = dd_zero(), s2 = dd_zero();
    for (int item = blockIdx.x * kWaves + wave; item < wl.nitems; item += gridDim.x * kWaves) {
        const Item it = decode_item(wl, item);
        const int x0 = it.strip * (kWave * VEC) + lane * VEC;
        if (x0 < (it.ya <= g.half ? g.cb : 0) || x0 >= g.xlim) continue;
        for (int y = it.ya; y <= it.yb; ++y) {
            const vec_t t = *reinterpret_cast<const vec_t*>(v + (row_off(g, y) - g.base0 + x0));
#pragma unroll
            for (int j = 0; j < VEC; ++j) { s1 = dd_add(s1, dd{(double)t[j], 0.0}); dd_acc_prod(s2, (double)t[j], (double)t[j]); }
        }
    }
    const dd t1 = block_reduce_dd(s1, lds), t2 = block_reduce_dd(s2, lds);
    if (threadIdx.x == 0) {
        const int n = gridDim.x, b = blockIdx.x;
        part[b] = t1.hi; part[n + b] = t1.lo; part[2 * n + b] = t2.hi; part[3 * n + b] = t2.lo;
    }
}

template <typename T>
__global__ __launch_bounds__(kBlock) void k_err_maxnorm(long long begin, long long len, const T* x, const T* u, double* part) {
    __shared__ double lds[2 * kWaves];
    const long long stride = (long long)gridDim.x * kBlock;
    double m = 0.0;
    for (long long i = begin + (long long)blockIdx.x * kBlock + threadIdx.x; i < begin + len; i += stride)
        m = fmax(m, fabs((double)(x[i] - u[i])));
    const double t = block_reduce<true>(m, lds);
    if (threadIdx.x == 0) part[blockIdx.x] = t;
}
// ... 130 lines not shown
```

### iterative_solvers_amd/csrc/mi355cg.hip

```cpp
#include "../../include/mi355cg.h"
#include "cg_kernels.h"
#include "csr_kernels.h"
#include "grid_setup.h"

#include <algorithm>
#include <chrono>
#include <cstdarg>
#include <cstdio>
#include <cstdlib>
#include <cstring>
#include <string>
#include <thread>
#include <vector>

using namespace mi355cg;

namespace {

thread_local std::string g_err;

int fail(int code, const char* fmt, ...) {
    char buf[512];
    va_list ap; va_start(ap, fmt); vsnprintf(buf, sizeof buf, fmt, ap); va_end(ap);
    g_err = buf;
// ... 4 lines not shown
    do {                                                                                             \
        hipError_t e_ = (expr);                                                                      \
        if (e_ != hipSuccess)                                                                        \
            return fail(MI355CG_ERR_HIP, "%s failed: %s (%s:%d)", #expr, hipGetErrorString(e_), __FILE__, __LINE__); \
    } while (0)

int env_int(const char* name, int dflt) {
    const char* v = getenv(name);
    return (v && *v) ? atoi(v) : dflt;
}

inline long long round_up(long long v, long long m) { return (v + m - 1) / m * m; }

constexpr int kRecHeader = kRecWords;
constexpr int kStripCols = 128;

struct EventPool {
    std::vector<hipEvent_t> ev;
    size_t used = 0;
    hipEvent_t get() {
        if (used == ev.size()) { hipEvent_t e; if (hipEventCreate(&e) != hipSuccess) return nullptr; ev.push_back(e); }
        return ev[used++];
    }
    void reset() { used = 0; }
    void destroy() { for (auto e : ev) hipEventDestroy(e); ev.clear(); used = 0; }
};

struct Plan { WorkList wl{}; int grid = 0; int ty = 0; };

}

struct mi355cg_ctx {
    int device = 0;
    int dtype = MI355CG_F64;
    hipStream_t stream = nullptr;
    GridParams gp;
    Geom g{};
    int s_lo = 0, s_hi = 0;
    long long storage_len = 0;
    long long pk_begin = 0, pk_len = 0;
    PackGeom pg{};
    Plan whole, interior, edge;
    Plan whole32;
    int depth = 2;
    bool has_gc = false;
    int nB_own = 0;
    int strideA = 0, strideB = 0;

    double *x = nullptr, *r = nullptr, *p[kRing] = {}, *ap = nullptr, *b = nullptr, *u = nullptr;
    int xsteps = 4;
    double* scratch[2] = {nullptr, nullptr};
    float *xf = nullptr, *rf = nullptr, *pf[kRing] = {}, *apf = nullptr;
    double* packed = nullptr;
    double *partA = nullptr, *partB = nullptr, *partR = nullptr;
    double *sumsA = nullptr, *sumsB = nullptr;
    int rec_width = 0;
    mi355cg_params dist_prm{};
    bool dist_active = false, is_slab = false;
    CgState *sA = nullptr, *sB = nullptr, *summary = nullptr;
    int* qctr = nullptr;
    int dyn_rows = 0;
    int* stop_h = nullptr;
    int* stop_dev = nullptr;
    HistEntry* hist = nullptr;
    CgState* summary_h = nullptr;
    HistEntry* hist_h = nullptr;
    double* partR_h = nullptr;

    std::vector<double> rhs_h, u_h;
    bool host_rhs_valid = true, host_u_valid = true;
    bool have_u_dev = false, solved = false;
    bool is_csr = false;
    long long csr_n = 0, csr_nnz = 0;
    int *csr_row_map = nullptr, *csr_entries = nullptr; double* csr_values = nullptr;
    int grid_csr = 0, grid_update = 0;
    int cur = 0;
    int nA_dist = 0;

    struct ChunkGraph { int m, cur; std::vector<char> flags; hipGraphExec_t exec; };
    std::vector<ChunkGraph> graphs;
    mi355cg_params graph_prm{};
    bool graph_stop = false;
    int use_graph = -1;

    hipEvent_t ev_loop[2] = {nullptr, nullptr};
    bool profiling = false;
    EventPool events;
    std::vector<std::pair<hipEvent_t, hipEvent_t>> ev_pairs[2];
    double kernel_ms[2] = {0, 0};
    long long kernel_launches[2] = {0, 0};
};

namespace {

long long phys_start(const Geom& g, int y) { return row_off(g, y) + (y <= g.half ? g.cb : 0); }
long long phys_end(const Geom& g, int y) { return phys_start(g, y) + (y <= g.half ? g.Pb : g.Pu); }
int strips_total(const GridParams& gp, int vec) { return (gp.n - 1) / (kWave * vec) + 1; }
int first_bottom_strip(const GridParams& gp, int vec) { return (gp.half + 1) / (kWave * vec); }

void own_cols(const mi355cg_ctx* c, int y, int* xa, int* xb) {
    const int lo = y <= c->gp.half ? c->gp.half + 1 : 1, hi = c->gp.n;
    *xa = std::max(lo, c->s_lo * kStripCols);
    *xb = std::max(*xa, std::min(hi, c->s_hi * kStripCols));
}

void build_geom(mi355cg_ctx* c, int vec, int y_lo, int y_hi) {
    Geom& g = c->g;
    const GridParams& gp = c->gp;
    g.N = gp.n; g.half = gp.half;
    g.Pu = (int)round_up(g.N + 1, 32);
    g.cb = g.half & ~31;
    g.Pb = g.Pu - g.cb;
    g.xlim = (int)round_up(g.N + 1, vec);
    g.y_lo = y_lo; g.y_hi = y_hi;
    g.base0 = 0;
    g.base0 = phys_start(g, y_lo - 1);
    c->storage_len = phys_end(g, y_hi + 1) - g.base0;
    g.own_begin = phys_start(g, y_lo) - g.base0;
    g.own_len = phys_end(g, y_hi) - phys_start(g, y_lo);
    g.A = gp.A; g.xk = gp.x_k; g.yk = gp.y_k;
    PackGeom& pg = c->pg;
    pg.g = g;
    const int yb0 = y_lo, yb1 = std::min(y_hi, gp.half), yu0 = std::max(y_lo, gp.half + 1), yu1 = y_hi;
    int xa = 0, xb = 0;
    pg.nb_rows = std::max(0, yb1 - yb0 + 1); pg.yb0 = yb0;
    own_cols(c, gp.half, &xa, &xb); pg.xb0 = xa; pg.wb = pg.nb_rows ? xb - xa : 0;
    pg.nu_rows = std::max(0, yu1 - yu0 + 1); pg.yu0 = yu0;
    own_cols(c, gp.half + 1, &xa, &xb); pg.xu0 = xa; pg.wu = pg.nu_rows ? xb - xa : 0;
    pg.pk_len = (long long)pg.nb_rows * pg.wb + (long long)pg.nu_rows * pg.wu;
    c->pk_len = pg.pk_len;
    c->pk_begin = packed_row_begin(gp, y_lo);
}

struct Rect { int y0, y1, s0, s1, gc; };
int region_rects(const GridParams& gp, int vec, int ya, int yb, int sa, int sb, Rect out[2]) {
    const int ns_all = strips_total(gp, vec), s0b = first_bottom_strip(gp, vec);
    int nr = 0;
    sb = std::min(sb, ns_all);
    if (ya <= gp.half && yb >= 1) {
        const int s0 = std::max(sa, s0b);
        if (s0 < sb) out[nr++] = Rect{std::max(ya, 1), std::min(yb, gp.half), s0, sb, (sa > s0b ? 1 : 0) | (sb < ns_all ? 2 : 0)};
    }
    if (yb > gp.half && sa < sb)
        out[nr++] = Rect{std::max(ya, gp.half + 1), std::min(yb, gp.n - 1), sa, sb, (sa > 0 ? 1 : 0) | (sb < ns_all ? 2 : 0)};
    return nr;
}

long long add_panel(WorkList& wl, int y0, int y1, int s0, int s1, int ty, int gc) {
    const int rows = y1 - y0 + 1, ns = s1 - s0;
    if (rows <= 0 || ns <= 0) return 0;
    if (ty <= 0) return (long long)rows * ns;
    if (wl.np >= kMaxPanels) return 0;
    Panel& P = wl.p[wl.np++];
    P.y0 = y0; P.y1 = y1; P.s0 = s0; P.ns = ns; P.gc = gc;
    P.nchunks = (rows + ty - 1) / ty;
    P.ty = (rows + P.nchunks - 1) / P.nchunks;
    P.nchunks = (rows + P.ty - 1) / P.ty;
    P.item0 = wl.nitems;
    wl.nitems += P.ns * P.nchunks;
    return (long long)rows * ns;
}

Plan make_plan(const std::vector<Rect>& rects, int max_rows, int fixed_ty = 0, int dyn_rows = 0) {
    Plan pl{};
    const int target_waves = std::max(kWaves, env_int("MI355CG_WAVES", 2048));
    const int max_blocks = std::max(1, env_int("MI355CG_BLOCKS", 512));
    const int waves = std::min(target_waves, max_blocks * kWaves);
    const long long item_rows = std::max(1, env_int("MI355CG_ITEM_ROWS", max_rows));
    long long strip_rows = 0;
    WorkList dry{};
    for (auto& r : rects) strip_rows += add_panel(dry, r.y0, r.y1, r.s0, r.s1, 0, 0);
    if (strip_rows == 0) return pl;
    const bool classes = env_int("MI355CG_XCD_CLASSES", 1) != 0 && fixed_ty == 0 && max_blocks >= kXcds && strip_rows >= 4LL * waves;
    auto build = [&](int ty) {
        WorkList wl{};
        wl.ncls = 1;
        for (auto& r : rects) add_panel(wl, r.y0, r.y1, r.s0, r.s1, ty, r.gc);
        if (classes) {
            wl.ncls = kXcds;
            for (int k = 0; k <= kXcds; ++k) wl.cls0[k] = (int)((long long)wl.nitems * k / kXcds);
        }
        return wl;
    };
    auto fits = [&](const WorkList& wl, long long rounds) {
        if (wl.ncls == kXcds) { for (int k = 0; k < kXcds; ++k) if (wl.cls0[k + 1] - wl.cls0[k] > rounds * (waves / kXcds)) return false; return true; }
        return wl.nitems <= rounds * waves;
    };
    int ty = fixed_ty;
    if (ty <= 0 && dyn_rows > 0 && classes) {
        ty = dyn_rows;
        pl.wl = build(ty);
    } else if (ty <= 0) {
        const long long rounds = std::max<long long>(1, (strip_rows + waves * item_rows - 1) / (waves * item_rows));
        ty = (int)std::max<long long>(std::min<long long>(8, item_rows), (strip_rows + rounds * waves - 1) / (rounds * waves));
        for (int tries = 0; tries < 64; ++tries) {
            pl.wl = build(ty);
            if (fits(pl.wl, rounds)) break;
            ++ty;
        }
    } else {
        pl.wl = build(ty);
    }
    pl.ty = ty;
    pl.grid = std::max(1, std::min(max_blocks, (pl.wl.nitems + kWaves - 1) / kWaves));
    if (pl.wl.ncls == kXcds) pl.grid = std::min(max_blocks / kXcds * kXcds, (pl.grid + kXcds - 1) / kXcds * kXcds);
    return pl;
}
constexpr int kMaxRowsF64 = 800, kMaxRowsF32 = 64;

void build_plans(mi355cg_ctx* c) {
    const Geom& g = c->g;
    const GridParams& gp = c->gp;
    Rect rr[2];
    const int nr = region_rects(gp, 2, g.y_lo, g.y_hi, c->s_lo, c->s_hi, rr);
    std::vector<Rect> whole(rr, rr + nr);
    c->whole = make_plan(whole, kMaxRowsF64);
    c->dyn_rows = std::max(0, env_int("MI355CG_DYN_ROWS", c->whole.ty >= 96 ? 16 : 0));
    if (c->dyn_rows > 0) {
        const Plan dyn = make_plan(whole, kMaxRowsF64, 0, c->dyn_rows);
        if (dyn.wl.ncls == kXcds && dyn.wl.nitems >= 2 * kWaves * dyn.grid) c->whole = dyn; else c->dyn_rows = 0;
    }
    c->has_gc = false;
    for (auto& r : whole) if (r.gc) c->has_gc = true;
    std::vector<Rect> inner, rows, cols;
    for (auto& r : whole) {
        const int yi0 = std::max(r.y0, g.y_lo + 1), yi1 = std::min(r.y1, g.y_hi - 1);
        const int si0 = r.s0 + ((r.gc & 1) ? 1 : 0), si1 = r.s1 - ((r.gc & 2) ? 1 : 0);
        if (r.y0 <= g.y_lo && g.y_lo <= r.y1) rows.push_back(Rect{g.y_lo, g.y_lo, r.s0, r.s1, r.gc});
        if (g.y_hi > g.y_lo && r.y0 <= g.y_hi && g.y_hi <= r.y1) rows.push_back(Rect{g.y_hi, g.y_hi, r.s0, r.s1, r.gc});
        if (yi0 > yi1) continue;
        if (si0 < si1) inner.push_back(Rect{yi0, yi1, si0, si1, 0});
        if (si0 >= si1) { cols.push_back(Rect{yi0, yi1, r.s0, r.s1, r.gc}); continue; }
        if (r.gc & 1) cols.push_back(Rect{yi0, yi1, r.s0, r.s0 + 1, 1});
        if (r.gc & 2) cols.push_back(Rect{yi0, yi1, r.s1 - 1, r.s1, 2});
    }
    c->interior = make_plan(inner, kMaxRowsF64);
    Plan e_rows = make_plan(rows, kMaxRowsF64, 1), e_cols = make_plan(cols, kMaxRowsF64, c->interior.ty > 0 ? c->interior.ty : 0);
    c->edge = e_rows;
    c->edge.wl.ncls = 1;
    for (int k = 0; k < e_cols.wl.np && c->edge.wl.np < kMaxPanels; ++k) {
        Panel P = e_cols.wl.p[k];
        P.item0 = c->edge.wl.nitems;
        c->edge.wl.p[c->edge.wl.np++] = P;
        c->edge.wl.nitems += P.ns * P.nchunks;
    }
    c->edge.grid = std::max(1, std::min(std::max(1, env_int("MI355CG_BLOCKS", 512)), (c->edge.wl.nitems + kWaves - 1) / kWaves));
    if (c->edge.wl.nitems == 0) c->edge.grid = 0;
    if (c->dtype == MI355CG_F32_MIXED || (c->s_lo == 0 && c->s_hi == strips_total(gp, 2))) {
        Rect r4[2];
        const int n4 = region_rects(gp, 4, g.y_lo, g.y_hi, 0, strips_total(gp, 4), r4);
        c->whole32 = make_plan(std::vector<Rect>(r4, r4 + n4), kMaxRowsF32);
    }
    c->depth = env_int("MI355CG_DEPTH", 3) == 2 ? 2 : 3;
    c->use_graph = env_int("MI355CG_GRAPH", -1);
    c->nB_own = c->whole.grid;
}

int flat_grid(long long n) { return (int)std::max<long long>(1, std::min<long long>(2048, (n + kBlock - 1) / kBlock)); }

struct PartSrc { const double* ptr; int n, fstride, estride; RecSrc rec; };
struct Where { hipStream_t stream; const Plan* plan; int slot; };

Where whole_part(const mi355cg_ctx* c) { return Where{c->stream, &c->whole, 0}; }
PartSrc own_partB(const mi355cg_ctx* c) { return PartSrc{c->partB, c->nB_own, c->strideB, 1}; }
PartSrc own_partA(const mi355cg_ctx* c) { return PartSrc{c->partA, c->whole.grid, c->strideA, 1}; }

template <typename T, int VEC> Geom kernel_geom(const mi355cg_ctx* c) { Geom g = c->g; g.xlim = (int)round_up(c->g.N + 1, VEC); return g; }

template <typename T, int VEC>
void launch_apply(const mi355cg_ctx* c, const T* v, T* out, const Where& w) {
    if (w.plan->wl.nitems == 0) return;
    StencilArgs<T> a{};
    a.g = kernel_geom<T, VEC>(c); a.wl = w.plan->wl;
    a.pin = v; a.ap = out; a.partA = nullptr;
    hipLaunchKernelGGL((k_stencil<T, VEC, false, false, 2, false, false>), dim3(w.plan->grid), dim3(kBlock), 0, w.stream, a);
}

struct IterCfg { RuleParams rp; int want_diag; bool has_u; bool x2 = false; };

template <typename T, int VEC>
void launch_iteration_stencil(mi355cg_ctx* c, const IterCfg& cfg, const T* r, T* const p[kRing], const Where& w, const PartSrc& pb, const FlagSpec* fl = nullptr) {
    if (w.plan->wl.nitems == 0) return;
    StencilArgs<T> a{};
    a.g = kernel_geom<T, VEC>(c); a.wl = w.plan->wl;
    a.r = r; a.pin = p[c->cur]; a.pout = p[(c->cur + 1) % c->xsteps]; a.ap = nullptr;
    a.partB = pb.ptr; a.nB = pb.n; a.strideB = pb.fstride; a.esB = pb.estride; a.src = pb.rec;
    a.partA = c->partA; a.strideA = c->strideA; a.slotA = w.slot;
    a.s_in = c->sB; a.s_out = c->sA; a.hist = c->hist; a.rp = cfg.rp; a.want_diag = cfg.want_diag;
    a.store_ghosts = c->is_slab ? 1 : 0;
    if (fl) a.fl = *fl;
    if (VEC == 2 && c->dyn_rows > 0 && w.plan == &c->whole) a.dq = QueueSpec{c->qctr, c->qctr + kXcds * kQueueSubs * kQueuePitch};
    const dim3 grid(w.plan->grid), block(kBlock);
    const bool msg = cfg.rp.rule == MI355CG_RULE_MSG_MAXNORM, gc = c->has_gc, d3 = c->depth == 3;
#define MI355CG_ST(MSG, D, GC) hipLaunchKernelGGL((k_stencil<T, VEC, true, MSG, D, true, GC>), grid, block, 0, w.stream, a)
    if constexpr (VEC == 2) {
        if (msg) { if (gc) { if (d3) MI355CG_ST(true, 3, true); else MI355CG_ST(true, 2, true); } else { if (d3) MI355CG_ST(true, 3, false); else MI355CG_ST(true, 2, false); } }
        else     { if (gc) { if (d3) MI355CG_ST(false, 3, true); else MI355CG_ST(false, 2, true); } else { if (d3) MI355CG_ST(false, 3, false); else MI355CG_ST(false, 2, false); } }
    } else {
        if (d3) MI355CG_ST(false, 3, false); else MI355CG_ST(false, 2, false);
    }
#undef MI355CG_ST
}

template <typename T, int VEC>
void launch_iteration_update(mi355cg_ctx* c, const IterCfg& cfg, T* x, T* r, T* const p[kRing], const T* u, const Where& w, const PartSrc& pa, const FlagSpec* fl = nullptr) {
    if (w.plan->wl.nitems == 0) return;
    UpdateStArgs<T> a{};
    a.g = kernel_geom<T, VEC>(c); a.wl = w.plan->wl;
    a.p = p[c->cur]; a.r = r; a.x = x; a.u = u;
    for (int i = 0; i < kRing - 1; ++i) a.pprev[i] = p[(c->cur + 2 * kRing * c->xsteps - 1 - i) % c->xsteps];
    a.partA = pa.ptr; a.nA = pa.n; a.strideA = pa.fstride; a.esA = pa.estride; a.src = pa.rec;
    a.partB = c->partB; a.strideB = c->strideB; a.slotB = w.slot;
    a.s_in = c->sA; a.s_out = c->sB; a.rule = cfg.rp.rule; a.reverse = 1;
    if (fl) a.fl = *fl;
    if (VEC == 2 && c->dyn_rows > 0 && w.plan == &c->whole) a.dq = QueueSpec{c->qctr + kXcds * kQueueSubs * kQueuePitch, c->qctr};
    a.stop_req = w.slot == 0 ? c->stop_dev : nullptr;
    const dim3 grid(w.plan->grid), block(kBlock);
    const bool d3 = c->depth == 3 && !(cfg.x2 && c->cur == 0 && c->xsteps == 8);
#define MI355CG_UST(XM, HASU) do { if (d3) hipLaunchKernelGGL((k_update_st<T, VEC, XM, HASU, 3, true>), grid, block, 0, w.stream, a); \
                                   else hipLaunchKernelGGL((k_update_st<T, VEC, XM, HASU, 2, true>), grid, block, 0, w.stream, a); } while (0)
    if (cfg.x2) {
        if (c->cur != 0) MI355CG_UST(0, false); else if (c->xsteps == 8) MI355CG_UST(8, false); else if (c->xsteps == 4) MI355CG_UST(4, false); else MI355CG_UST(2, false);
    }
    else if constexpr (VEC == 2) { if (cfg.has_u) MI355CG_UST(1, true); else MI355CG_UST(1, false); }
#undef MI355CG_UST
}

template <typename T, int VEC>
void launch_update_flat(mi355cg_ctx* c, const IterCfg& cfg, T* x, T* r, const T* p, const T* ap, const T* u, hipStream_t stream,
                        int grid, double resume_r0norm = -1.0) {
    UpdateArgs<T> a{};
    a.begin = c->g.own_begin / VEC; a.nvec = c->g.own_len / VEC;
    a.x = x; a.r = r; a.p = p; a.ap = ap; a.u = u;
    a.partA = c->partA; a.nA = 0; a.strideA = c->strideA; a.esA = 1;
    a.partB = c->partB; a.strideB = c->strideB;
    a.s_in = c->sA; a.s_out = c->sB; a.rule = cfg.rp.rule; a.init = 1;
    if (resume_r0norm >= 0.0) { a.init = 2; a.r0norm_resume = resume_r0norm; a.s_in = c->sB; }
    if (cfg.has_u) hipLaunchKernelGGL((k_update<T, VEC, true>), dim3(grid), dim3(kBlock), 0, stream, a);
    else hipLaunchKernelGGL((k_update<T, VEC, false>), dim3(grid), dim3(kBlock), 0, stream, a);
}

template <typename T, int VEC>
void launch_flush_x(const mi355cg_ctx* c, const Plan& plan, T* x, T* const p[kRing], const CgState& fin, hipStream_t stream) {
    const int pending = fin.it % c->xsteps;
    if (plan.wl.nitems == 0 || pending == 0) return;
    FlushArgs<T> f{};
    f.n = pending;
    for (int j = 0; j < pending; ++j) { const int k = fin.it - pending + 1 + j; f.p[j] = p[k % c->xsteps]; f.a[j] = (T)fin.alpha_hist[k & (kRing - 1)]; }
    hipLaunchKernelGGL((k_flush_x<T, VEC>), dim3(std::max(1, std::min(1024, (plan.wl.nitems + kWaves - 1) / kWaves))), dim3(kBlock), 0, stream,
                       kernel_geom<T, VEC>(c), plan.wl, x, f);
}

void launch_check(mi355cg_ctx* c, const IterCfg& cfg, hipStream_t stream, const PartSrc& pb) {
    CheckArgs a{};
    a.partB = pb.ptr; a.nB = pb.n; a.strideB = pb.fstride; a.esB = pb.estride; a.src = pb.rec;
    a.s_in = c->sB; a.summary = c->summary; a.hist = c->hist; a.rp = cfg.rp; a.want_diag = cfg.want_diag;
    hipLaunchKernelGGL(k_check, dim3(1), dim3(kBlock), 0, stream, a);
}

IterCfg make_cfg(const mi355cg_params* prm) {
    IterCfg cfg{};
    const bool msg = prm->rule == MI355CG_RULE_MSG_MAXNORM;
    cfg.rp.rule = prm->rule; cfg.rp.max_iterations = prm->max_iterations;
    cfg.rp.eps_precision = prm->eps_precision; cfg.rp.eps_residual = prm->eps_residual;
    cfg.rp.eps_exact_error = prm->eps_exact_error; cfg.rp.eps_rel = prm->eps_rel;
    cfg.rp.fixed_iterations = prm->fixed_iterations;
    const bool diag = !msg && prm->diagnostics;
    cfg.has_u = (msg && prm->use_true_solution) || diag;
    cfg.rp.use_u = cfg.has_u ? 1 : 0;
    cfg.want_diag = diag ? 1 : 0;
    cfg.x2 = !msg && !diag;
    return cfg;
}

template <typename T>
int upload_packed(mi355cg_ctx* c, const double* host_packed, T* storage) {
    if (c->is_csr) {
        HIPCK(hipMemcpyAsync(storage, host_packed, sizeof(double) * c->pk_len, hipMemcpyHostToDevice, c->stream));
        HIPCK(hipStreamSynchronize(c->stream));
        return MI355CG_OK;
    }
    if (c->is_slab) HIPCK(hipDeviceSynchronize());
    if (c->pk_len == 0) return MI355CG_OK;
    HIPCK(hipMemcpyAsync(c->packed, host_packed, sizeof(double) * c->pk_len, hipMemcpyHostToDevice, c->stream));
    hipLaunchKernelGGL((k_unpack<T>), dim3(flat_grid(c->pk_len)), dim3(kBlock), 0, c->stream, c->pg, c->packed, storage);
    HIPCK(hipGetLastError());
    HIPCK(hipStreamSynchronize(c->stream));
    return MI355CG_OK;
}
template <typename T>
int download_packed(mi355cg_ctx* c, const T* storage, double* host_packed) {
    if (c->is_csr) {
        HIPCK(hipMemcpyAsync(host_packed, storage, sizeof(double) * c->pk_len, hipMemcpyDeviceToHost, c->stream));
        HIPCK(hipStreamSynchronize(c->stream));
        return MI355CG_OK;
    }
    if (c->is_slab) HIPCK(hipDeviceSynchronize());
    if (c->pk_len == 0) return MI355CG_OK;
    hipLaunchKernelGGL((k_pack<T>), dim3(flat_grid(c->pk_len)), dim3(kBlock), 0, c->stream, c->pg, storage, c->packed);
    HIPCK(hipGetLastError());
    HIPCK(hipMemcpyAsync(host_packed, c->packed, sizeof(double) * c->pk_len, hipMemcpyDeviceToHost, c->stream));
    HIPCK(hipStreamSynchronize(c->stream));
    return MI355CG_OK;
}

int alloc_vec(double** p, long long n) {
    HIPCK(hipMalloc((void**)p, sizeof(double) * n));
    HIPCK(hipMemset(*p, 0, sizeof(double) * n));
    return MI355CG_OK;
}

int ensure_host_copies(mi355cg_ctx* c) {
    if (!c->host_rhs_valid) { c->rhs_h.resize(c->pk_len); if (int rc = download_packed<double>(c, c->b, c->rhs_h.data())) return rc; c->host_rhs_valid = true; }
    if (!c->host_u_valid) { c->u_h.resize(c->pk_len); if (int rc = download_packed<double>(c, c->u, c->u_h.data())) return rc; c->host_u_valid = true; }
    return MI355CG_OK;
}
int ensure_f32_vectors(mi355cg_ctx* c) {
    if (c->xsteps > 4) return fail(MI355CG_ERR_INVALID, "MI355CG_XSTEPS=8 is fp64 only");
    if (c->whole32.wl.nitems == 0) return fail(MI355CG_ERR_INVALID, "the fp32 kernels march 256-column strips: a part of a 2-D decomposition (cut on 128 columns) cannot run them; use row slabs");
    if (c->g.own_begin % 4 != 0 || c->g.own_len % 4 != 0) return fail(MI355CG_ERR_STATE, "a part's owned range is not a whole number of float4");
    float** fv[] = {&c->xf, &c->apf, &c->pf[0], &c->pf[1], &c->pf[2], &c->pf[3]};
    for (int k = 0; k < 2 + c->xsteps; ++k) {
        if (*fv[k]) continue;
        if (hipMalloc((void**)fv[k], sizeof(float) * c->storage_len) != hipSuccess || hipMemset(*fv[k], 0, sizeof(float) * c->storage_len) != hipSuccess)
            return fail(MI355CG_ERR_HIP, "fp32 vector allocation failed");
    }
    HIPCK(hipDeviceSynchronize());
    return MI355CG_OK;
}

int ensure_u_on_device(mi355cg_ctx* c) {
    if (c->have_u_dev) return MI355CG_OK;
    if (!c->host_u_valid) return fail(MI355CG_ERR_STATE, "no exact solution on host or device");
    if (int rc = upload_packed<double>(c, c->u_h.data(), c->u)) return rc;
    c->have_u_dev = true;
    return MI355CG_OK;
}
int ensure_scratch(mi355cg_ctx* c) {
    for (auto& s : c->scratch) if (!s) { if (int rc = alloc_vec(&s, c->storage_len)) return rc; }
    HIPCK(hipDeviceSynchronize());
// ... 239 lines not shown
    prof_collect(c);
    mi355cg_results res{};
    res.iterations = total; res.converged = converged ? 1 : 0;
    res.stop_reason = interrupted ? MI355CG_STOP_INTERRUPTED : (converged ? MI355CG_STOP_RESIDUAL : MI355CG_STOP_ITERATIONS);
    res.final_residual_norm = res.final_precision = res.final_error_norm = DBL_MAX;
    res.r_norm2 = rnorm; res.initial_r_norm2 = bnorm;
    res.refine_outer = outer; res.refine_true_rel = bnorm > 0 ? rnorm / bnorm : 0.0;
    res.solve_seconds = std::chrono::duration<double>(std::chrono::steady_clock::now() - t0).count();
    if (out) *out = res;
    return MI355CG_OK;
}

}

extern "C" {

const char* mi355cg_last_error(void) { return g_err.c_str(); }
const char* mi355cg_version(void) { return "mi355cg 0.2 (gfx950)"; }

static int create_impl(int n, int m, double a, double b, double c_, double d, int dtype, int device,
                       int y_lo, int y_hi, int s_lo, int s_hi, bool part, mi355cg_handle* out) {
    if (!out) return fail(MI355CG_ERR_INVALID, "out is null");
    *out = nullptr;
    if (dtype != MI355CG_F64 && dtype != MI355CG_F32_MIXED) return fail(MI355CG_ERR_INVALID, "unknown dtype %d", dtype);
    GridParams gp;
    if (!grid_params_init(&gp, n, m, a, b, c_, d))
        return fail(MI355CG_ERR_INVALID, "grid %dx%d rejected: the L-shaped index map is only consistent for n == m, even, >= 6", n, m);
    int ndev = 0;
    if (hipGetDeviceCount(&ndev) != hipSuccess || ndev <= 0)
        return fail(MI355CG_ERR_HIP, "no HIP device available (libmi355cg has no CPU fallback)");
    if (device < 0 || device >= ndev) return fail(MI355CG_ERR_INVALID, "device %d out of range (0..%d)", device, ndev - 1);
    HIPCK(hipSetDevice(device));

    const int ns_all = strips_total(gp, 2);
    if (!part) { y_lo = 1; y_hi = gp.n - 1; s_lo = 0; s_hi = ns_all; }
    if (y_lo < 1 || y_hi > gp.n - 1 || y_lo > y_hi)
        return fail(MI355CG_ERR_INVALID, "part rows [%d, %d] outside 1..%d", y_lo, y_hi, gp.n - 1);
    if (s_lo < 0 || s_hi > ns_all || s_lo >= s_hi)
        return fail(MI355CG_ERR_INVALID, "part strips [%d, %d) outside 0..%d", s_lo, s_hi, ns_all);
    if (dtype == MI355CG_F32_MIXED && part) return fail(MI355CG_ERR_INVALID, "F32_MIXED is single-GPU only");
    mi355cg_ctx* c = new mi355cg_ctx();
    c->device = device; c->dtype = dtype; c->gp = gp; c->is_slab = part;
    c->s_lo = s_lo; c->s_hi = s_hi;
    build_geom(c, 2, y_lo, y_hi);
    build_plans(c);
    c->strideA = std::max({c->whole.grid, c->interior.grid + c->edge.grid, c->whole32.grid, 1});
    c->strideB = c->strideA;

    int rc = MI355CG_OK;
    auto cleanup = [&]() { mi355cg_destroy(c); return rc; };
    if (hipStreamCreateWithFlags(&c->stream, hipStreamNonBlocking) != hipSuccess) { rc = fail(MI355CG_ERR_HIP, "hipStreamCreate failed"); return cleanup(); }
    const long long L = c->storage_len;
    { const int m = env_int("MI355CG_XSTEPS", 4); c->xsteps = m == 2 ? 2 : ((m == 8 && dtype == MI355CG_F64) ? 8 : 4); }
    double** vecs[] = {&c->x, &c->r, &c->p[0], &c->p[1], &c->ap, &c->b, &c->u, &c->p[2], &c->p[3], &c->p[4], &c->p[5], &c->p[6], &c->p[7]};
    for (int k = 0; k < 7 + (c->xsteps - 2); ++k) if ((rc = alloc_vec(vecs[k], L))) return cleanup();
    if (dtype == MI355CG_F32_MIXED) {
        float** fv[] = {&c->xf, &c->rf, &c->pf[0], &c->pf[1], &c->apf, &c->pf[2], &c->pf[3], &c->pf[4], &c->pf[5], &c->pf[6], &c->pf[7]};
        const int nfv = 5 + (c->xsteps - 2);
        for (int k = 0; k < nfv; ++k) {
            float** v = fv[k];
            if (hipMalloc((void**)v, sizeof(float) * L) != hipSuccess || hipMemset(*v, 0, sizeof(float) * L) != hipSuccess) {
                rc = fail(MI355CG_ERR_HIP, "fp32 vector allocation failed"); return cleanup();
            }
        }
    }
    if ((rc = alloc_vec(&c->packed, std::max<long long>(c->pk_len, 1)))) return cleanup();
    if ((rc = alloc_vec(&c->partA, (long long)FA_COUNT * c->strideA))) return cleanup();
    if ((rc = alloc_vec(&c->partB, (long long)FB_COUNT * c->strideB))) return cleanup();
    if ((rc = alloc_vec(&c->partR, 2048))) return cleanup();
    c->rec_width = kRecHeader + 2 * c->g.Pu;
    if ((rc = alloc_vec(&c->sumsA, c->rec_width))) return cleanup();
    if ((rc = alloc_vec(&c->sumsB, c->rec_width))) return cleanup();
    if (hipMalloc((void**)&c->sA, sizeof(CgState)) != hipSuccess || hipMalloc((void**)&c->sB, sizeof(CgState)) != hipSuccess ||
        hipMalloc((void**)&c->summary, sizeof(CgState)) != hipSuccess || hipMalloc((void**)&c->hist, sizeof(HistEntry) * kHist) != hipSuccess ||
        hipHostMalloc((void**)&c->summary_h, sizeof(CgState)) != hipSuccess || hipHostMalloc((void**)&c->hist_h, sizeof(HistEntry) * kHist) != hipSuccess ||
        hipHostMalloc((void**)&c->partR_h, sizeof(double) * 2048) != hipSuccess) {
        rc = fail(MI355CG_ERR_HIP, "state allocation failed"); return cleanup();
    }
    hipMemset(c->sA, 0, sizeof(CgState)); hipMemset(c->sB, 0, sizeof(CgState)); hipMemset(c->summary, 0, sizeof(CgState));
    hipMemset(c->hist, 0, sizeof(HistEntry) * kHist);
    if (hipMalloc((void**)&c->qctr, sizeof(int) * 2 * kXcds * kQueueSubs * kQueuePitch) != hipSuccess || hipMemset(c->qctr, 0, sizeof(int) * 2 * kXcds * kQueueSubs * kQueuePitch) != hipSuccess) { rc = fail(MI355CG_ERR_HIP, "queue counter allocation failed"); return cleanup(); }
    if (hipHostMalloc((void**)&c->stop_h, sizeof(int)) != hipSuccess) { rc = fail(MI355CG_ERR_HIP, "stop word allocation failed"); return cleanup(); }
    *c->stop_h = 0;
    HIPCK(hipDeviceSynchronize());

    if (env_int("MI355CG_DEVICE_SETUP", 0)) {
        c->host_rhs_valid = false; c->host_u_valid = false;
        if ((rc = mi355cg_setup_on_device(c))) return cleanup();
    } else {
        c->rhs_h.resize(c->pk_len); c->u_h.resize(c->pk_len);
        grid_fill_box(gp, c->g.y_lo, c->g.y_hi, s_lo * kStripCols, s_hi == ns_all ? gp.n : s_hi * kStripCols, c->rhs_h.data(), c->u_h.data(), nullptr, nullptr);
        if ((rc = upload_packed<double>(c, c->rhs_h.data(), c->b))) return cleanup();
    }
    *out = c;
    return MI355CG_OK;
}

int mi355cg_create(int n, int m, double a, double b, double c_, double d, int dtype, int device, mi355cg_handle* out) {
    return create_impl(n, m, a, b, c_, d, dtype, device, 0, 0, 0, 0, false, out);
}
int mi355cg_create_slab(int n, int m, double a, double b, double c_, double d, int dtype, int device,
                        int y_lo, int y_hi, mi355cg_handle* out) {
    GridParams gp;
    if (!grid_params_init(&gp, n, m, a, b, c_, d)) return fail(MI355CG_ERR_INVALID, "grid %dx%d rejected: the L-shaped index map is only consistent for n == m, even, >= 6", n, m);
    return create_impl(n, m, a, b, c_, d, dtype, device, y_lo, y_hi, 0, strips_total(gp, 2), true, out);
}
int mi355cg_create_part(int n, int m, double a, double b, double c_, double d, int dtype, int device,
                        int y_lo, int y_hi, int x_lo, int x_hi, mi355cg_handle* out) {
    GridParams gp;
    if (!grid_params_init(&gp, n, m, a, b, c_, d)) return fail(MI355CG_ERR_INVALID, "grid %dx%d rejected: the L-shaped index map is only consistent for n == m, even, >= 6", n, m);
    const int ns_all = strips_total(gp, 2);
    if (x_lo % kStripCols != 0 || (x_hi % kStripCols != 0 && x_hi < gp.n))
        return fail(MI355CG_ERR_INVALID, "part columns [%d, %d): x-cuts must be multiples of %d", x_lo, x_hi, kStripCols);
    return create_impl(n, m, a, b, c_, d, dtype, device, y_lo, y_hi, x_lo / kStripCols, x_hi >= gp.n ? ns_all : x_hi / kStripCols, true, out);
}

int mi355cg_create_csr(long long nrows, const int* row_map, const int* entries, const double* values,
                       int device, mi355cg_handle* out) {
    if (!out) return fail(MI355CG_ERR_INVALID, "out is null");
    *out = nullptr;
    if (nrows <= 0 || !row_map || !entries || !values) return fail(MI355CG_ERR_INVALID, "bad CSR arguments");
    if (row_map[0] != 0) return fail(MI355CG_ERR_INVALID, "row_map[0] must be 0");
    const long long nnz = row_map[nrows];
    for (long long i = 0; i < nrows; ++i) if (row_map[i + 1] < row_map[i]) return fail(MI355CG_ERR_INVALID, "row_map is not monotone at row %lld", i);
    for (long long j = 0; j < nnz; ++j) if (entries[j] < 0 || entries[j] >= nrows) return fail(MI355CG_ERR_INVALID, "column index %d out of range at entry %lld", entries[j], j);
    int ndev = 0;
    if (hipGetDeviceCount(&ndev) != hipSuccess || ndev <= 0) return fail(MI355CG_ERR_HIP, "no HIP device available (libmi355cg has no CPU fallback)");
    if (device < 0 || device >= ndev) return fail(MI355CG_ERR_INVALID, "device %d out of range (0..%d)", device, ndev - 1);
    HIPCK(hipSetDevice(device));
    mi355cg_ctx* c = new mi355cg_ctx();
    c->device = device; c->dtype = MI355CG_F64; c->is_csr = true;
    c->csr_n = nrows; c->csr_nnz = nnz;
    c->gp.size = nrows; c->pk_begin = 0; c->pk_len = nrows; c->storage_len = nrows; c->pg.pk_len = nrows;
    c->g.own_begin = 0; c->g.own_len = nrows;
    const long long nblk = (nrows + kBlock - 1) / kBlock;
    c->grid_csr = (int)std::max<long long>(1, std::min<long long>(2048, nblk));
    c->grid_update = (int)std::max<long long>(1, std::min<long long>(512, nblk));
    c->strideA = c->grid_csr; c->strideB = c->grid_update; c->nB_own = c->grid_update;
    int rc = MI355CG_OK;
    auto cleanup = [&]() { mi355cg_destroy(c); return rc; };
    if (hipStreamCreateWithFlags(&c->stream, hipStreamNonBlocking) != hipSuccess) { rc = fail(MI355CG_ERR_HIP, "hipStreamCreate failed"); return cleanup(); }
    double** vecs[] = {&c->x, &c->r, &c->p[0], &c->p[1], &c->ap, &c->b, &c->u};
    for (auto v : vecs) if ((rc = alloc_vec(v, nrows))) return cleanup();
    if ((rc = alloc_vec(&c->partA, (long long)FA_COUNT * c->strideA))) return cleanup();
    if ((rc = alloc_vec(&c->partB, (long long)FB_COUNT * c->strideB))) return cleanup();
    if ((rc = alloc_vec(&c->partR, 2048))) return cleanup();
    if (hipMalloc((void**)&c->csr_row_map, sizeof(int) * (nrows + 1)) != hipSuccess || hipMalloc((void**)&c->csr_entries, sizeof(int) * std::max<long long>(nnz, 1)) != hipSuccess ||
        hipMalloc((void**)&c->csr_values, sizeof(double) * std::max<long long>(nnz, 1)) != hipSuccess ||
        hipMalloc((void**)&c->sA, sizeof(CgState)) != hipSuccess || hipMalloc((void**)&c->sB, sizeof(CgState)) != hipSuccess ||
        hipMalloc((void**)&c->summary, sizeof(CgState)) != hipSuccess || hipMalloc((void**)&c->hist, sizeof(HistEntry) * kHist) != hipSuccess ||
        hipHostMalloc((void**)&c->summary_h, sizeof(CgState)) != hipSuccess || hipHostMalloc((void**)&c->hist_h, sizeof(HistEntry) * kHist) != hipSuccess ||
        hipHostMalloc((void**)&c->partR_h, sizeof(double) * 2048) != hipSuccess) {
        rc = fail(MI355CG_ERR_HIP, "allocation failed"); return cleanup();
    }
    if (hipMemcpy(c->csr_row_map, row_map, sizeof(int) * (nrows + 1), hipMemcpyHostToDevice) != hipSuccess ||
        hipMemcpy(c->csr_entries, entries, sizeof(int) * nnz, hipMemcpyHostToDevice) != hipSuccess ||
        hipMemcpy(c->csr_values, values, sizeof(double) * nnz, hipMemcpyHostToDevice) != hipSuccess) {
        rc = fail(MI355CG_ERR_HIP, "CSR upload failed"); return cleanup();
    }
    hipMemset(c->sA, 0, sizeof(CgState)); hipMemset(c->sB, 0, sizeof(CgState)); hipMemset(c->summary, 0, sizeof(CgState));
    hipMemset(c->hist, 0, sizeof(HistEntry) * kHist);
    HIPCK(hipDeviceSynchronize());
    c->rhs_h.assign(nrows, 0.0); c->u_h.assign(nrows, 0.0);
    *out = c;
    return MI355CG_OK;
}

int mi355cg_set_true_solution(mi355cg_handle c, const double* u) {
    if (!c || !u) return fail(MI355CG_ERR_INVALID, "null argument");
    HIPCK(hipSetDevice(c->device));
    c->host_u_valid = true;
    c->u_h.resize(c->pk_len);
    std::memcpy(c->u_h.data(), u, sizeof(double) * c->pk_len);
    if (int rc = upload_packed<double>(c, c->u_h.data(), c->u)) return rc;
    c->have_u_dev = true;
    return MI355CG_OK;
}

void mi355cg_destroy(mi355cg_handle c) {
    if (!c) return;
    hipSetDevice(c->device);
    if (c->stream) hipStreamSynchronize(c->stream);
    void* dev[] = {c->x, c->r, c->p[0], c->p[1], c->p[2], c->p[3], c->p[4], c->p[5], c->p[6], c->p[7], c->ap, c->b, c->u, c->scratch[0], c->scratch[1], c->xf, c->rf,
                   c->pf[0], c->pf[1], c->pf[2], c->pf[3], c->pf[4], c->pf[5], c->pf[6], c->pf[7], c->apf,
                   c->packed, c->partA, c->partB, c->partR, c->sumsA, c->sumsB, c->sA, c->sB, c->summary, c->hist, c->qctr};
    for (void* p : dev) if (p) hipFree(p);
    if (c->csr_row_map) hipFree(c->csr_row_map);
    if (c->csr_entries) hipFree(c->csr_entries);
    if (c->csr_values) hipFree(c->csr_values);
    if (c->summary_h) hipHostFree(c->summary_h);
    if (c->hist_h) hipHostFree(c->hist_h);
    if (c->partR_h) hipHostFree(c->partR_h);
    if (c->stop_h) hipHostFree(c->stop_h);
    clear_graphs(c);
    c->events.destroy();
    for (hipEvent_t e : c->ev_loop) if (e) hipEventDestroy(e);
    if (c->stream) hipStreamDestroy(c->stream);
    delete c;
}

long long mi355cg_size(mi355cg_handle c) { return c ? c->gp.size : -1; }

int mi355cg_get_rhs(mi355cg_handle c, double* out) {
    if (!c || !out) return fail(MI355CG_ERR_INVALID, "null argument");
    if (int rc = ensure_host_copies(c)) return rc;
    std::memcpy(out, c->rhs_h.data(), sizeof(double) * c->pk_len);
    return MI355CG_OK;
}
int mi355cg_get_true_solution(mi355cg_handle c, double* out) {
    if (!c || !out) return fail(MI355CG_ERR_INVALID, "null argument");
    if (int rc = ensure_host_copies(c)) return rc;
    std::memcpy(out, c->u_h.data(), sizeof(double) * c->pk_len);
    return MI355CG_OK;
}
int mi355cg_get_node_coords(mi355cg_handle c, double* xs, double* ys) {
    if (!c || !xs || !ys) return fail(MI355CG_ERR_INVALID, "null argument");
    if (c->is_csr) return fail(MI355CG_ERR_INVALID, "a CSR handle has no grid coordinates");
    const int ns_all = strips_total(c->gp, 2);
    grid_fill_box(c->gp, c->g.y_lo, c->g.y_hi, c->s_lo * kStripCols, c->s_hi == ns_all ? c->gp.n : c->s_hi * kStripCols, nullptr, nullptr, xs, ys);
    return MI355CG_OK;
}
int mi355cg_setup_on_device(mi355cg_handle c) {
    if (!c) return fail(MI355CG_ERR_INVALID, "null handle");
    if (c->is_csr) return fail(MI355CG_ERR_INVALID, "a CSR handle has no grid to set up");
    HIPCK(hipSetDevice(c->device));
    if (c->is_slab) HIPCK(hipDeviceSynchronize());
    SetupArgs s{};
    s.pg = c->pg; s.a = c->gp.a; s.c = c->gp.c; s.x_step = c->gp.x_step; s.y_step = c->gp.y_step; s.xk = c->gp.x_k; s.yk = c->gp.y_k;
    s.n = c->gp.n; s.m = c->gp.m;
    if (c->pk_len > 0) hipLaunchKernelGGL(k_setup, dim3(flat_grid(c->pk_len)), dim3(kBlock), 0, c->stream, s, c->b, c->u);
    HIPCK(hipGetLastError());
    HIPCK(hipStreamSynchronize(c->stream));
    c->have_u_dev = true; c->host_rhs_valid = false; c->host_u_valid = false;
    return MI355CG_OK;
}
int mi355cg_set_rhs(mi355cg_handle c, const double* b) {
    if (!c || !b) return fail(MI355CG_ERR_INVALID, "null argument");
    HIPCK(hipSetDevice(c->device));
    c->host_rhs_valid = true;
    c->rhs_h.resize(c->pk_len);
    std::memcpy(c->rhs_h.data(), b, sizeof(double) * c->pk_len);
    return upload_packed<double>(c, c->rhs_h.data(), c->b);
}

int mi355cg_apply_device(mi355cg_handle c, const double* x_dev, double* y_dev) {
    if (!c || !x_dev || !y_dev) return fail(MI355CG_ERR_INVALID, "null argument");
    if (c->is_slab) return fail(MI355CG_ERR_STATE, "this handle owns one part of a decomposed grid: use the mi355cg_team_* / mi355cg_dist_* entry points");
    HIPCK(hipSetDevice(c->device));
    if (c->is_csr) {
        launch_csr_spmv(c, x_dev, y_dev, nullptr, nullptr, nullptr);
        HIPCK(hipGetLastError());
        HIPCK(hipStreamSynchronize(c->stream));
        return MI355CG_OK;
    }
    if (int rc = ensure_scratch(c)) return rc;
    hipLaunchKernelGGL((k_unpack<double>), dim3(flat_grid(c->pk_len)), dim3(kBlock), 0, c->stream, c->pg, x_dev, c->scratch[0]);
    launch_apply<double, 2>(c, c->scratch[0], c->scratch[1], whole_part(c));
    hipLaunchKernelGGL((k_pack<double>), dim3(flat_grid(c->pk_len)), dim3(kBlock), 0, c->stream, c->pg, c->scratch[1], y_dev);
    HIPCK(hipGetLastError());
    HIPCK(hipStreamSynchronize(c->stream));
    return MI355CG_OK;
}

int mi355cg_apply(mi355cg_handle c, const double* x, double* y) {
    if (!c || !x || !y) return fail(MI355CG_ERR_INVALID, "null argument");
    if (c->is_slab) return fail(MI355CG_ERR_STATE, "this handle owns one part of a decomposed grid: use the mi355cg_team_* / mi355cg_dist_* entry points");
    HIPCK(hipSetDevice(c->device));
    if (int rc = ensure_scratch(c)) return rc;
    if (int rc = upload_packed<double>(c, x, c->scratch[0])) return rc;
    if (c->is_csr) launch_csr_spmv(c, c->scratch[0], c->scratch[1], nullptr, nullptr, nullptr);
    else launch_apply<double, 2>(c, c->scratch[0], c->scratch[1], whole_part(c));
    HIPCK(hipGetLastError());
    return download_packed<double>(c, c->scratch[1], y);
}

void mi355cg_default_params(mi355cg_params* p, int rule) {
    if (!p) return;
    std::memset(p, 0, sizeof *p);
    p->rule = rule;
    p->max_iterations = 10000;
    p->eps_precision = 1e-6; p->eps_residual = 1e-6; p->eps_exact_error = 1e-6;
    p->eps_rel = 1e-6;
    p->use_true_solution = 1;
    p->callback_every = rule == MI355CG_RULE_MSG_MAXNORM ? 100 : 1;
    p->diagnostics = 0;
    p->sync_every = 0;
    p->fixed_iterations = 0;
    p->inner_eps = 0.0;
}

int mi355cg_solve(mi355cg_handle c, const mi355cg_params* prm, mi355cg_iter_cb cb, void* user,
                  const volatile int* stop_flag, mi355cg_results* out) {
    if (!c || !prm) return fail(MI355CG_ERR_INVALID, "null argument");
    if (prm->rule != MI355CG_RULE_MSG_MAXNORM && prm->rule != MI355CG_RULE_REL_2NORM) return fail(MI355CG_ERR_INVALID, "unknown rule %d", prm->rule);
    if (c->is_slab) return fail(MI355CG_ERR_STATE, "this handle owns one part of a decomposed grid: use the mi355cg_team_* / mi355cg_dist_* entry points");
    HIPCK(hipSetDevice(c->device));
    if (c->is_csr) return solve_csr(c, prm, cb, user, stop_flag, out);
    if (c->dtype == MI355CG_F32_MIXED) return solve_mixed(c, prm, cb, user, stop_flag, out);
    const bool msg = prm->rule == MI355CG_RULE_MSG_MAXNORM;
    const IterCfg cfg = make_cfg(prm);
    const bool diag = cfg.want_diag != 0;
    c->nB_own = c->whole.grid;
    if (cfg.has_u) if (int rc = ensure_u_on_device(c)) return rc;
    if (diag) if (int rc = ensure_scratch(c)) return rc;

    const auto t0 = std::chrono::steady_clock::now();
    c->events.reset(); c->ev_pairs[0].clear(); c->ev_pairs[1].clear();

    c->cur = 0;
    if (c->qctr && c->dyn_rows > 0) HIPCK(hipMemsetAsync(c->qctr, 0, sizeof(int) * 2 * kXcds * kQueueSubs * kQueuePitch, c->stream));
    {
        FreshArgs<double> f{};
        f.begin = c->g.own_begin / 2; f.nvec = c->g.own_len / 2;
        f.b = c->b; f.x = c->x; f.r = c->r; f.p0 = c->p[0]; f.u = c->u;
        f.partB = c->partB; f.strideB = c->strideB; f.s_out = c->sB;
        if (cfg.has_u) hipLaunchKernelGGL((k_init_fresh<double, 2, true>), dim3(c->whole.grid), dim3(kBlock), 0, c->stream, f);
        else hipLaunchKernelGGL((k_init_fresh<double, 2, false>), dim3(c->whole.grid), dim3(kBlock), 0, c->stream, f);
    }
    HIPCK(hipGetLastError());

    *c->stop_h = 0;
    c->stop_dev = nullptr;
    if (stop_flag) HIPCK(hipHostGetDevicePointer((void**)&c->stop_dev, c->stop_h, 0));
    auto wait_stream = [&]() -> int {
        if (!stop_flag) { HIPCK(hipStreamSynchronize(c->stream)); return MI355CG_OK; }
        for (;;) {
            if (*stop_flag) *c->stop_h = 1;
            const hipError_t q = hipStreamQuery(c->stream);
            if (q == hipSuccess) break;
            if (q != hipErrorNotReady) HIPCK(q);
            std::this_thread::yield();
        }
        return MI355CG_OK;
    };
    auto poll = [&]() -> int {
        launch_check(c, cfg, c->stream, own_partB(c));
        HIPCK(hipMemcpyAsync(c->summary_h, c->summary, sizeof(CgState), hipMemcpyDeviceToHost, c->stream));
        HIPCK(hipMemcpyAsync(c->hist_h, c->hist, sizeof(HistEntry) * kHist, hipMemcpyDeviceToHost, c->stream));
        return wait_stream();
    };
    *c->summary_h = CgState{};
    if (msg && cb) {
        if (int rc = poll()) return rc;
        cb(user, 0, DBL_MAX, c->summary_h->rmax, cfg.has_u ? c->summary_h->emax : DBL_MAX);
    }
    if (!c->ev_loop[0]) { HIPCK(hipEventCreate(&c->ev_loop[0])); HIPCK(hipEventCreate(&c->ev_loop[1])); }
    HIPCK(hipEventRecord(c->ev_loop[0], c->stream));

    const int every = prm->callback_every;
    auto need_u = [&](int it) { return diag || cfg.rp.eps_exact_error > 0 || it == 1 || (every > 0 && it % every == 0); };
    int sync_every = prm->sync_every > 0 ? prm->sync_every : (msg ? 100 : 200);
    sync_every = std::min(sync_every, kHist);
    int it_done = 0;
    bool interrupted = false;
    bool first_chunk = cb != nullptr || stop_flag != nullptr;
    if (std::memcmp(&c->graph_prm, prm, sizeof *prm) != 0 || c->graph_stop != (stop_flag != nullptr)) {
        clear_graphs(c); c->graph_prm = *prm; c->graph_stop = stop_flag != nullptr;
    }
    const bool graph_ok = !c->profiling && !diag &&
                          (c->use_graph == 1 || (c->use_graph < 0 && c->g.own_len < (4LL << 20) && prm->max_iterations >= 4 * sync_every));
    while (!c->summary_h->done) {
        if (stop_flag && *stop_flag) { interrupted = true; break; }
        int m = std::min(sync_every, prm->max_iterations - it_done);
        if (msg && every > 0) m = std::min(m, every - it_done % every);
        if (first_chunk) { m = 1; first_chunk = false; }
        if (m <= 0) m = 1;
        auto enqueue_chunk = [&]() -> int {
            for (int k = 0; k < m; ++k) {
                hipEvent_t e0 = nullptr;
                prof_begin(c, &e0);
                launch_iteration_stencil<double, 2>(c, cfg, c->r, c->p, whole_part(c), own_partB(c));
                c->cur = (c->cur + 1) % c->xsteps;
                prof_end(c, 0, e0);
                prof_begin(c, &e0);
                IterCfg ucfg = cfg;
                ucfg.has_u = cfg.has_u && need_u(it_done + k + 1);
                launch_iteration_update<double, 2>(c, ucfg, c->x, c->r, c->p, c->u, whole_part(c), own_partA(c));
                prof_end(c, 1, e0);
                if (diag) {
                    launch_apply<double, 2>(c, c->x, c->scratch[0], whole_part(c));
                    hipLaunchKernelGGL((k_resid2<double>), dim3(1024), dim3(kBlock), 0, c->stream, c->g.own_begin, c->g.own_len, c->b, c->scratch[0], c->partR);
                    hipLaunchKernelGGL(k_resid2_hist, dim3(1), dim3(kBlock), 0, c->stream, c->partR, 1024, c->sB, c->hist);
                }
            }
            return MI355CG_OK;
        };
        if (graph_ok && m >= 8) {
            std::vector<char> flags(m);
            for (int k = 0; k < m; ++k) flags[k] = cfg.has_u && need_u(it_done + k + 1);
            mi355cg_ctx::ChunkGraph* hit = nullptr;
            for (auto& g : c->graphs) if (g.m == m && g.cur == c->cur && g.flags == flags) hit = &g;
            if (!hit) {
                hipGraph_t graph = nullptr; hipGraphExec_t exec = nullptr;
                const int cur0 = c->cur;
                HIPCK(hipStreamBeginCapture(c->stream, hipStreamCaptureModeThreadLocal));
                const int rc = enqueue_chunk();
                const hipError_t e1 = hipStreamEndCapture(c->stream, &graph);
                c->cur = cur0;
                if (rc) return rc;
                HIPCK(e1);
                HIPCK(hipGraphInstantiate(&exec, graph, nullptr, nullptr, 0));
                HIPCK(hipGraphDestroy(graph));
                c->graphs.push_back({m, cur0, flags, exec});
                hit = &c->graphs.back();
            }
            HIPCK(hipGraphLaunch(hit->exec, c->stream));
            c->cur = (c->cur + m) % c->xsteps;
        } else {
            if (int rc = enqueue_chunk()) return rc;
        }
        HIPCK(hipGetLastError());
        if (int rc = poll()) return rc;
        const int it_now = c->summary_h->it;
        if (cb) for (int it = it_done + 1; it <= it_now; ++it) {
            const HistEntry& h = c->hist_h[it % kHist];
            if (diag) {
                cb(user, it - 1, std::sqrt(h.d2), std::sqrt(h.tr2), std::sqrt(h.e2));
            } else if (msg) {
                const bool stopped_here = c->summary_h->done && c->summary_h->reason != MI355CG_STOP_ITERATIONS &&
                                          c->summary_h->reason != MI355CG_STOP_INTERRUPTED && it == it_now;
                if ((it == 1 || (every > 0 && it % every == 0)) && !stopped_here) cb(user, it, h.dmax, h.rmax, cfg.has_u ? h.emax : DBL_MAX);
            }
        }
        it_done = it_now;
    }
    HIPCK(hipEventRecord(c->ev_loop[1], c->stream));
    CgState fin = *c->summary_h;
    c->stop_dev = nullptr;
    if (fin.done && fin.reason == MI355CG_STOP_INTERRUPTED) interrupted = true;
    c->cur = fin.it % c->xsteps;
    if (cfg.x2) {
        launch_flush_x<double, 2>(c, c->whole, c->x, c->p, fin, c->stream);
        HIPCK(hipGetLastError());
        HIPCK(hipStreamSynchronize(c->stream));
    }
    if (cfg.has_u && fin.it > 0 && !need_u(fin.it)) {
        hipLaunchKernelGGL((k_err_maxnorm<double>), dim3(1024), dim3(kBlock), 0, c->stream, c->g.own_begin, c->g.own_len, c->x, c->u, c->partR);
        HIPCK(hipGetLastError());
        HIPCK(hipMemcpyAsync(c->partR_h, c->partR, sizeof(double) * 1024, hipMemcpyDeviceToHost, c->stream));
        HIPCK(hipStreamSynchronize(c->stream));
        double m = 0; for (int i = 0; i < 1024; ++i) m = std::max(m, c->partR_h[i]);
        fin.emax = m;
    }
    c->solved = true;
    prof_collect(c);
#ifdef MI355CG_WAVE_TIMING
    if (const char* path = getenv("MI355CG_WAVE_TIMING_OUT")) {
        std::vector<unsigned long long> buf(2 * kWtStamps * kWtWaves);
        HIPCK(hipMemcpyFromSymbol(buf.data(), HIP_SYMBOL(g_wave_dbg), buf.size() * sizeof(unsigned long long)));
        if (FILE* f = fopen(path, "wb")) { fwrite(buf.data(), sizeof(unsigned long long), buf.size(), f); fclose(f); }
    }
#endif
    mi355cg_results res{};
    res.iterations = fin.it;
    res.converged = interrupted ? 0 : fin.converged;
    res.stop_reason = interrupted ? MI355CG_STOP_INTERRUPTED : fin.reason;
    res.final_residual_norm = fin.rmax;
    res.final_precision = fin.it > 0 ? fin.dmax : DBL_MAX;
    res.final_error_norm = cfg.has_u ? fin.emax : DBL_MAX;
    res.r_norm2 = fin.rnorm2;
    res.initial_r_norm2 = fin.r0norm;
    res.solve_seconds = std::chrono::duration<double>(std::chrono::steady_clock::now() - t0).count();
    { float ms = 0; HIPCK(hipEventSynchronize(c->ev_loop[1])); if (hipEventElapsedTime(&ms, c->ev_loop[0], c->ev_loop[1]) == hipSuccess) res.loop_seconds = 1e-3 * ms; }
    if (msg && cb) cb(user, res.iterations, res.final_precision, res.final_residual_norm, res.final_error_norm);
    if (out) *out = res;
    return MI355CG_OK;
}

int mi355cg_get_solution(mi355cg_handle c, double* x) {
    if (!c || !x) return fail(MI355CG_ERR_INVALID, "null argument");
    if (!c->solved) return fail(MI355CG_ERR_STATE, "no solve has run on this handle");
    HIPCK(hipSetDevice(c->device));
    return download_packed<double>(c, c->x, x);
}
int mi355cg_get_recursive_residual(mi355cg_handle c, double* r) {
    if (!c || !r) return fail(MI355CG_ERR_INVALID, "null argument");
    if (!c->solved) return fail(MI355CG_ERR_STATE, "no solve has run on this handle");
    HIPCK(hipSetDevice(c->device));
    return download_packed<double>(c, c->r, r);
}
int mi355cg_get_true_residual(mi355cg_handle c, double* out) {
    if (!c || !out) return fail(MI355CG_ERR_INVALID, "null argument");
    if (c->is_slab) return fail(MI355CG_ERR_STATE, "this handle owns one part of a decomposed grid: use the mi355cg_team_* / mi355cg_dist_* entry points");
    if (!c->solved) return fail(MI355CG_ERR_STATE, "no solve has run on this handle");
    HIPCK(hipSetDevice(c->device));
    if (int rc = ensure_scratch(c)) return rc;
    if (c->is_csr) launch_csr_spmv(c, c->x, c->scratch[0], nullptr, nullptr, nullptr);
    else launch_apply<double, 2>(c, c->x, c->scratch[0], whole_part(c));
    hipLaunchKernelGGL((k_sub<double>), dim3(flat_grid(c->g.own_len)), dim3(kBlock), 0, c->stream, c->g.own_begin, c->g.own_len, c->scratch[0], c->b, c->scratch[1]);
    HIPCK(hipGetLastError());
    return download_packed<double>(c, c->scratch[1], out);
}

int mi355cg_set_profiling(mi355cg_handle c, int enable) {
    if (!c) return fail(MI355CG_ERR_INVALID, "null handle");
    c->profiling = enable != 0;
    return MI355CG_OK;
}
int mi355cg_get_kernel_time(mi355cg_handle c, int kernel, double* avg_ms, long long* launches) {
    if (!c || kernel < 0 || kernel > 1) return fail(MI355CG_ERR_INVALID, "bad argument");
    if (avg_ms) *avg_ms = c->kernel_ms[kernel];
    if (launches) *launches = c->kernel_launches[kernel];
    return MI355CG_OK;
}
int mi355cg_get_layout(mi355cg_handle c, long long* padded_len, int* pitch_bottom, int* pitch_upper,
                       int* grid_stencil, int* grid_update, int* rows_per_item) {
    if (!c) return fail(MI355CG_ERR_INVALID, "null handle");
    if (padded_len) *padded_len = c->g.own_len;
    if (pitch_bottom) *pitch_bottom = c->g.Pb;
    if (pitch_upper) *pitch_upper = c->g.Pu;
    if (grid_stencil) *grid_stencil = c->whole.grid;
    if (grid_update) *grid_update = c->whole.grid;
    if (rows_per_item) *rows_per_item = c->whole.ty;
    return MI355CG_OK;
}

namespace {
struct hdd { double hi, lo; };
inline hdd hdd_add(hdd a, hdd b) {
    const double s = a.hi + b.hi, bb = s - a.hi, e = (a.hi - (s - bb)) + (b.hi - bb);
    const double lo = e + (a.lo + b.lo), hi = s + lo;
    return hdd{hi, lo - (hi - s)};
}
int ctx_checksum(mi355cg_ctx* c, int which, hdd out[2]) {
    const double* v = which == 0 ? c->x : which == 1 ? c->r : which == 2 ? c->b : which == 3 ? c->u : nullptr;
    if (!v) return fail(MI355CG_ERR_INVALID, "checksum: vector %d (0 x, 1 r, 2 b, 3 u)", which);
    if (c->is_csr) return fail(MI355CG_ERR_INVALID, "checksum: grid handles only");
    HIPCK(hipSetDevice(c->device));
    if (c->is_slab) HIPCK(hipDeviceSynchronize());
    if (which == 3) if (int rc = ensure_u_on_device(c)) return rc;
    const int grid = 512;
    hipLaunchKernelGGL((k_checksum<double, 2>), dim3(grid), dim3(kBlock), 0, c->stream, kernel_geom<double, 2>(c), c->whole.wl, v, c->partR);
    HIPCK(hipGetLastError());
    HIPCK(hipMemcpyAsync(c->partR_h, c->partR, sizeof(double) * 4 * grid, hipMemcpyDeviceToHost, c->stream));
    HIPCK(hipStreamSynchronize(c->stream));
    for (int b = 0; b < grid; ++b) {
        out[0] = hdd_add(out[0], hdd{c->partR_h[b], c->partR_h[grid + b]});
        out[1] = hdd_add(out[1], hdd{c->partR_h[2 * grid + b], c->partR_h[3 * grid + b]});
    }
    return MI355CG_OK;
}
}

int mi355cg_checksum(mi355cg_handle c, int which, double* out2) {
    if (!c || !out2) return fail(MI355CG_ERR_INVALID, "null argument");
    hdd s[2] = {{0, 0}, {0, 0}};
    if (int rc = ctx_checksum(c, which, s)) return rc;
    out2[0] = s[0].hi + s[0].lo; out2[1] = s[1].hi + s[1].lo;
    return MI355CG_OK;
}

int mi355cg_slab_rows(int n, int world, int rank, int* y_lo, int* y_hi) {
    GridParams gp;
    if (!grid_params_init(&gp, n, n, 0, 1, 0, 1)) return fail(MI355CG_ERR_INVALID, "grid %d rejected", n);
    if (world < 1 || rank < 0 || rank >= world || world > n - 1) return fail(MI355CG_ERR_INVALID, "bad world/rank %d/%d", rank, world);
    std::vector<int> first(world + 1);
    first[0] = 1; first[world] = n;
    for (int k = 1; k < world; ++k) {
        const long long target = (gp.size * k + world / 2) / world;
        int lo = 1, hi = n;
        while (lo < hi) { const int mid = (lo + hi) / 2; if (packed_row_begin(gp, mid) >= target) hi = mid; else lo = mid + 1; }
        first[k] = lo;
    }
    for (int k = 1; k < world; ++k) first[k] = std::max(first[k], first[k - 1] + 1);
    for (int k = world - 1; k >= 1; --k) first[k] = std::min(first[k], first[k + 1] - 1);
    const int a = first[rank], b = first[rank + 1] - 1;
    if (y_lo) *y_lo = a;
    if (y_hi) *y_hi = b;
    return MI355CG_OK;
}

int mi355cg_owned_range(mi355cg_handle c, long long* packed_begin, long long* packed_len, int* y_lo, int* y_hi) {
    if (!c) return fail(MI355CG_ERR_INVALID, "null handle");
    if (packed_begin) *packed_begin = c->pk_begin;
    if (packed_len) *packed_len = c->pk_len;
    if (y_lo) *y_lo = c->g.y_lo;
    if (y_hi) *y_hi = c->g.y_hi;
    return MI355CG_OK;
}

static hipStream_t pick_stream(mi355cg_ctx*, void* stream) { return (hipStream_t)stream; }
static Where part_where(const mi355cg_ctx* c, hipStream_t st, int rows) {
    if (rows == 1) return Where{st, &c->interior, 0};
    if (rows == 2) return Where{st, &c->edge, c->interior.grid};
    return Where{st, &c->whole, 0};
// ... 174 lines not shown
```

### iterative_solvers_amd/solver.py

```python
from __future__ import annotations

import ctypes as C
import enum
import sys
from dataclasses import dataclass, field
from typing import Callable, Optional

import numpy as np

from . import _capi

DBL_MAX = sys.float_info.max


class StopCriterion(enum.IntEnum):
    ITERATIONS = 0
    PRECISION = 1
    RESIDUAL = 2
    EXACT_ERROR = 3
    INTERRUPTED = 4


_STOP_TEXT = {
    StopCriterion.ITERATIONS: "Достигнуто максимальное число итераций",
# ... 18 lines not shown

    @classmethod
    def from_csr(cls, row_map, entries, values, device=0):
        self = cls.__new__(cls)
        self._lib = _capi.load()
        self._h = C.c_void_p()
        row_map = np.ascontiguousarray(row_map, dtype=np.int32)
        entries = np.ascontiguousarray(entries, dtype=np.int32)
        values = np.ascontiguousarray(values, dtype=np.float64)
        rc = self._lib.mi355cg_create_csr(len(row_map) - 1, row_map, entries, values, int(device), C.byref(self._h))
        if rc == _capi.ERR_INVALID:
            raise ValueError(self._lib.mi355cg_last_error().decode())
        _capi.check(rc)
        self.size = int(self._lib.mi355cg_size(self._h))
        return self

    def set_true_solution(self, u):
        u = np.ascontiguousarray(u, dtype=np.float64)
        if u.shape != (self.size,):
            raise ValueError(f"true solution has shape {u.shape}, expected ({self.size},)")
        _capi.check(self._lib.mi355cg_set_true_solution(self._h, u))

    def close(self):
        if getattr(self, "_h", None) is not None and self._h:
            self._lib.mi355cg_destroy(self._h)
            self._h = None

    def __del__(self):
        try:
            self.close()
        except Exception:
            pass

    def _vec_out(self, fn) -> np.ndarray:
        out = np.empty(self.size)
        _capi.check(fn(self._h, out))
        return out

    def rhs(self): return self._vec_out(self._lib.mi355cg_get_rhs)
    def true_solution(self): return self._vec_out(self._lib.mi355cg_get_true_solution)
    def solution(self): return self._vec_out(self._lib.mi355cg_get_solution)
    def recursive_residual(self): return self._vec_out(self._lib.mi355cg_get_recursive_residual)
    def true_residual(self): return self._vec_out(self._lib.mi355cg_get_true_residual)

    def node_coords(self):
        xs, ys = np.empty(self.size), np.empty(self.size)
        _capi.check(self._lib.mi355cg_get_node_coords(self._h, xs, ys))
        return xs, ys

    def set_rhs(self, b):
        b = np.ascontiguousarray(b, dtype=np.float64)
        if b.shape != (self.size,):
            raise ValueError(f"rhs has shape {b.shape}, expected ({self.size},)")
        _capi.check(self._lib.mi355cg_set_rhs(self._h, b))

    def apply(self, x):
        x = np.ascontiguousarray(x, dtype=np.float64)
        if x.shape != (self.size,):
            raise ValueError(f"vector has shape {x.shape}, expected ({self.size},)")
        y = np.empty(self.size)
        _capi.check(self._lib.mi355cg_apply(self._h, x, y))
        return y

    def solve(self, params: _capi.Params, callback=None, stop_flag: Optional[C.c_int] = None) -> _capi.Results:
        res = _capi.Results()
        cb = _capi.ITER_CB(lambda user, it, p, r, e: callback(it, p, r, e)) if callback else _capi.ITER_CB()
        sp = C.cast(C.pointer(stop_flag), C.c_void_p) if stop_flag is not None else None
        rc = self._lib.mi355cg_solve(self._h, C.byref(params), cb, None, sp, C.byref(res))
        if rc == _capi.ERR_INVALID:
            raise ValueError(self._lib.mi355cg_last_error().decode())
        _capi.check(rc)
        return res

    def setup_on_device(self):
        _capi.check(self._lib.mi355cg_setup_on_device(self._h))

    def set_profiling(self, on: bool):
        _capi.check(self._lib.mi355cg_set_profiling(self._h, 1 if on else 0))

    def kernel_time(self, kernel: int):
        ms, n = C.c_double(), C.c_longlong()
        _capi.check(self._lib.mi355cg_get_kernel_time(self._h, kernel, C.byref(ms), C.byref(n)))
        return ms.value, n.value

    def layout(self):
        L = C.c_longlong()
        v = [C.c_int() for _ in range(5)]
        _capi.check(self._lib.mi355cg_get_layout(self._h, C.byref(L), *[C.byref(i) for i in v]))
        return {"padded_len": L.value, "pitch_bottom": v[0].value, "pitch_upper": v[1].value,
                "grid_stencil": v[2].value, "grid_update": v[3].value, "rows_per_item": v[4].value}


def default_params(rule: int) -> _capi.Params:
    p = _capi.Params()
    _capi.load().mi355cg_default_params(C.byref(p), rule)
    return p


class MatrixFreeSystem:

    def __init__(self, m, n, a, b, c, d, device: int = 0, dtype: int = _capi.F64):
        self.n, self.m = n, m
        self.domain = (a, b, c, d)
        self._handle = _Handle(n, m, a, b, c, d, dtype=dtype, device=device)

    def get_rhs(self) -> np.ndarray: return self._handle.rhs()
    def get_true_solution_vector(self) -> np.ndarray: return self._handle.true_solution()
    def size(self) -> int: return self._handle.size

    def apply(self, x, y=None) -> np.ndarray:
        out = self._handle.apply(x)
        if y is not None:
            y[...] = out
            return y
        return out

    def __mul__(self, x): return self.apply(x)


class GridSystem(MatrixFreeSystem):

    def get_matrix(self): return self
    def get_x_coords(self): return self._handle.node_coords()[0]
    def get_y_coords(self): return self._handle.node_coords()[1]

    def get_node_coordinates(self, solution_index: int):
        if solution_index < 0 or solution_index >= self.size():
            return (0.0, 0.0)
        xs, ys = self._handle.node_coords()
        return (float(xs[solution_index]), float(ys[solution_index]))


class CrsMatrix:

    def __init__(self, row_map, entries, values, device: int = 0):
        self._handle = _Handle.from_csr(row_map, entries, values, device=device)

    def numRows(self): return self._handle.size
    def numCols(self): return self._handle.size
    def size(self): return self._handle.size
    def apply(self, x): return self._handle.apply(x)
    def __mul__(self, x): return self.apply(x)


class MatrixFreeSolver:

    def __init__(self, system: MatrixFreeSystem, b, eps: float = 1e-6, maxIterations: int = 10000,
                 name: str = "Matrix-free solver"):
        self.system, self.b, self.eps, self.maxIterations, self.name = system, b, eps, maxIterations, name
        self.iterations = 0
        self.iteration_callback = None
        self.completion_callback = None
        self.last_results = None

    def setIterationCallback(self, cb): self.iteration_callback = cb
    def setCompletionCallback(self, cb): self.completion_callback = cb
    def getIterations(self): return self.iterations
    def getName(self): return self.name

    def solve(self, true_solution=None, fixed_iterations: bool = False, sync_every: int = 0,
              inner_eps: float = 0.0) -> np.ndarray:
        h = self.system._handle
        h.set_rhs(self.b)
        if true_solution is not None and len(true_solution) > 0:
            h.set_true_solution(true_solution)
        p = default_params(_capi.RULE_REL_2NORM)
# ... 148 lines not shown
```

Baseline: 7205 iters/s.

## Add persistent cooperative CG kernel keeping part of the residual resident in LDS

```diff
diff --git a/include/mi355cg.h b/include/mi355cg.h
--- a/include/mi355cg.h
+++ b/include/mi355cg.h
@@ -89,6 +89,7 @@
 int  mi355cg_get_kernel_time(mi355cg_handle h, int kernel, double *avg_ms, long long *launches);
 int  mi355cg_get_layout(mi355cg_handle h, long long *padded_len, int *pitch_bottom, int *pitch_upper,
                         int *grid_stencil, int *grid_update, int *rows_per_item);
+int  mi355cg_get_resident(mi355cg_handle h, int *active, int *grid, int *rows_per_wave, long long *resident_cells);
 
 int  mi355cg_slab_rows(int n, int world, int rank, int *y_lo, int *y_hi);
 int  mi355cg_create_part(int n, int m, double a, double b, double c, double d, int dtype, int device,
diff --git a/iterative_solvers_amd/_capi.py b/iterative_solvers_amd/_capi.py
--- a/iterative_solvers_amd/_capi.py
+++ b/iterative_solvers_amd/_capi.py
@@ -17,7 +17,7 @@
     "mi355cg_get_rhs", "mi355cg_get_true_solution", "mi355cg_get_node_coords", "mi355cg_set_rhs",
     "mi355cg_apply", "mi355cg_apply_device", "mi355cg_default_params", "mi355cg_solve",
     "mi355cg_get_solution", "mi355cg_get_recursive_residual", "mi355cg_get_true_residual",
-    "mi355cg_set_profiling", "mi355cg_get_kernel_time", "mi355cg_get_layout",
+    "mi355cg_set_profiling", "mi355cg_get_kernel_time", "mi355cg_get_layout", "mi355cg_get_resident",
     "mi355cg_slab_rows", "mi355cg_create_slab", "mi355cg_owned_range", "mi355cg_dist_begin",
     "mi355cg_dist_reduce", "mi355cg_dist_sums_ptr", "mi355cg_dist_record_layout", "mi355cg_dist_scatter_ghosts", "mi355cg_dist_stencil", "mi355cg_dist_flip",
     "mi355cg_dist_update", "mi355cg_dist_update_reads_ghosts", "mi355cg_dist_check", "mi355cg_dist_summary", "mi355cg_dist_finish", "mi355cg_dist_history",
@@ -108,6 +108,7 @@
     L.mi355cg_set_profiling.argtypes = [H, C.c_int]
     L.mi355cg_get_kernel_time.argtypes = [H, C.c_int, C.POINTER(C.c_double), C.POINTER(C.c_longlong)]
     L.mi355cg_get_layout.argtypes = [H, C.POINTER(C.c_longlong)] + [C.POINTER(C.c_int)] * 5
+    L.mi355cg_get_resident.argtypes = [H] + [C.POINTER(C.c_int)] * 3 + [C.POINTER(C.c_longlong)]
     LLP, IP, VPP = C.POINTER(C.c_longlong), C.POINTER(C.c_int), C.POINTER(C.c_void_p)
     L.mi355cg_slab_rows.argtypes = [C.c_int, C.c_int, C.c_int, IP, IP]
     L.mi355cg_create_slab.argtypes = [C.c_int, C.c_int] + [C.c_double] * 4 + [C.c_int] * 4 + [C.POINTER(H)]
diff --git a/iterative_solvers_amd/csrc/cg_kernels.h b/iterative_solvers_amd/csrc/cg_kernels.h
--- a/iterative_solvers_amd/csrc/cg_kernels.h
+++ b/iterative_solvers_amd/csrc/cg_kernels.h
@@ -48,16 +48,17 @@
 constexpr int kXcds = 8;
 struct WorkList { Panel p[kMaxPanels]; int np; int nitems; int ncls; int cls0[kXcds + 1]; };
 struct ItemSeq { int first, step, begin, end; };
-__device__ inline ItemSeq item_seq(const WorkList& wl, int wave) {
+__device__ inline ItemSeq item_seq(const WorkList& wl, int wave, int block, int nblocks) {
     if (wl.ncls == kXcds) {
-        const int cls = blockIdx.x % kXcds, nb = (gridDim.x - cls + kXcds - 1) / kXcds;
+        const int cls = block % kXcds, nb = (nblocks - cls + kXcds - 1) / kXcds;
         int begin = wl.cls0[0], end = wl.cls0[1];
 #pragma unroll
         for (int k = 1; k < kXcds; ++k) if (k == cls) { begin = wl.cls0[k]; end = wl.cls0[k + 1]; }
-        return ItemSeq{begin + (int)(blockIdx.x / kXcds) * kWaves + wave, nb * kWaves, begin, end};
-    }
-    return ItemSeq{(int)blockIdx.x * kWaves + wave, (int)gridDim.x * kWaves, 0, wl.nitems};
-}
+        return ItemSeq{begin + (block / kXcds) * kWaves + wave, nb * kWaves, begin, end};
+    }
+    return ItemSeq{block * kWaves + wave, nblocks * kWaves, 0, wl.nitems};
+}
+__device__ inline ItemSeq item_seq(const WorkList& wl, int wave) { return item_seq(wl, wave, (int)blockIdx.x, (int)gridDim.x); }
 
 struct CgState {
     double alpha, beta;
@@ -227,9 +228,7 @@
     return d;
 }
 
-__device__ inline void write_state_after_decision(CgState* out, HistEntry* hist, const CgState* in, const StateLite& s, const Decision& d) {
-    copy_state(out, in);
-    CgState* o = out;
+__device__ inline void apply_decision(CgState* o, HistEntry* hist, const StateLite& s, const Decision& d) {
     o->rr_prev = s.rr; o->rr = d.rr; o->rnorm2 = d.rnorm2; o->r0norm = d.r0norm; o->beta = d.beta;
     o->rmax = d.rmax; o->dmax = d.dmax; o->emax = d.emax; o->d2 = d.d2; o->e2 = d.e2;
     o->done = d.done; o->reason = d.reason; o->converged = d.converged;
@@ -237,6 +236,10 @@
         HistEntry* h = hist + (s.it % kHist);
         h->dmax = d.dmax; h->rmax = d.rmax; h->emax = d.emax; h->rnorm2 = d.rnorm2; h->d2 = d.d2; h->e2 = d.e2;
     }
+}
+__device__ inline void write_state_after_decision(CgState* out, HistEntry* hist, const CgState* in, const StateLite& s, const Decision& d) {
+    copy_state(out, in);
+    apply_decision(out, hist, s, d);
 }
 
 __device__ inline Decision reduce_and_decide(const StateLite& s, const RuleParams& rp, const double* partB,
@@ -584,16 +587,27 @@
     return A;
 }
 
-template <typename T, int VEC, bool FUSED, bool MSG, int DEPTH, bool NOAP, bool GC>
-__global__ __launch_bounds__(kBlock) void k_stencil(const StencilArgs<T> a) {
+struct NoRes { static constexpr bool on = false; };
+struct LdsRes {
+    static constexpr bool on = true;
+    double* slots;
+    double* dummy;
+    int item, y0, n;
+};
+template <class Res> __device__ inline bool res_row(const Res& rs, bool have, int item, int y) {
+    if constexpr (Res::on) return have && item == rs.item && (unsigned)(y - rs.y0) < (unsigned)rs.n;
+    else return false;
+}
+__device__ inline double* res_slot(const LdsRes& rs, bool res, int y, int lane) { return (res ? rs.slots + (y - rs.y0) * (2 * kWave) : rs.dummy) + 2 * lane; }
+__device__ inline double* res_slot(const NoRes&, bool, int, int) { return nullptr; }
+
+template <typename T, int VEC, bool FUSED, bool MSG, int DEPTH, bool NOAP, bool GC, class Res, class Pre, class Pro>
+__device__ inline bool stencil_sweep(const StencilArgs<T>& a, const ItemSeq& seq, const int lane, const Res& res, Pre&& pre, Pro&& prologue,
+                                     dd& acc_pap, dd& acc_rz) {
     static_assert(DEPTH >= 1 && DEPTH <= 3, "the compute cursor takes its item from the fetch cursor: DEPTH <= rows fetched per item (>= 3)");
+    static_assert(!Res::on || (FUSED && VEC == 2 && sizeof(T) == 8), "resident r: fp64 fused stencil only");
     typedef typename VecOf<T, VEC>::type vec_t;
-    __shared__ double lds[2 * kWaves];
     const Geom& g = a.g;
-    const int lane = threadIdx.x & (kWave - 1);
-    const int wave = __builtin_amdgcn_readfirstlane(threadIdx.x / kWave);
-    const ItemSeq seq = item_seq(a.wl, wave);
-    MI355CG_WT_BEGIN
     struct Raw { vec_t r, p; T re, pe; };
 
     int f_item = seq.first;
@@ -624,7 +638,13 @@
         if (!f_have) { vo = kOob; ve = kOob; }
         Raw w;
         w.p = buf_load<vec_t>(rs_p, vo, f_so);
-        if (FUSED) w.r = buf_load<vec_t>(rs_r, vo, f_so);
+        if constexpr (Res::on) {
+            const bool rr = res_row(res, f_have && own, f_item, f_y);
+            const vec_t l = *reinterpret_cast<const vec_t*>(res_slot(res, rr, f_y, lane));
+            w.r = buf_load<vec_t>(rs_r, rr ? kOob : vo, f_so);
+#pragma unroll
+            for (int j = 0; j < VEC; ++j) w.r[j] = rr ? l[j] : w.r[j];
+        } else if (FUSED) w.r = buf_load<vec_t>(rs_r, vo, f_so);
         else for (int j = 0; j < VEC; ++j) w.r[j] = (T)0;
         w.pe = buf_load<T>(rs_p, ve, f_so);
         if (FUSED) w.re = buf_load<T>(rs_r, ve, f_so); else w.re = (T)0;
@@ -650,56 +670,15 @@
         if (GC) c_ve_gc = ((lane == 0 && (C.gc & 1)) || (lane == kWave - 1 && (C.gc & 2))) ? C.ve_own : kOob;
     };
 
+    pre();
     if (f_have) { enter(f_item); promote(); }
     Raw q[DEPTH];
 #pragma unroll
     for (int k = 0; k < DEPTH; ++k) q[k] = fetch();
 
     T beta = (T)0;
-    if (FUSED && a.src.mbox) {
-        __shared__ double recs[kMaxRecDst * kRecWords];
-        const PreParts pre = prefetch_parts(a.partB + FB_RR * a.strideB, a.partB + (FB_RR + FB_LO) * a.strideB, a.nB, 1);
-        PreMax pmax[3] = {{0, 0}, {0, 0}, {0, 0}};
-        if (MSG) {
-#pragma unroll
-            for (int k = 0; k < 3; ++k) pmax[k] = prefetch_max(a.partB + (FB_RMAX + k) * a.strideB, a.nB, 1);
-        }
-        const StateLite s = load_state_lite(a.s_in);
-        if (s.done) {
-            if (threadIdx.x == 0) { store_flagged_zero(a.fl, a.slotA + blockIdx.x, FA_COUNT); if (blockIdx.x == 0) copy_state(a.s_out, a.s_in); }
-            return;
-        }
-        MI355CG_WT_STAMP(1)
-        own_record_B(recs, a.src.me, a.partB, a.nB, a.strideB, MSG ? 1 : 0, lds, &pre, MSG ? pmax : nullptr);
-        if (!gather_records(a.src, recs)) {
-            if (threadIdx.x == 0) { store_flagged_zero(a.fl, a.slotA + blockIdx.x, FA_COUNT); if (blockIdx.x == 0) fail_transport(a.s_out, a.s_in); }
-            return;
-        }
-        const Decision d = decide_from_records(s, a.rp, recs, a.src.world, MSG, false);
-        MI355CG_WT_STAMP(2)
-        if (blockIdx.x == 0 && threadIdx.x == 0) write_state_after_decision(a.s_out, a.hist, a.s_in, s, d);
-        if (d.done) { if (threadIdx.x == 0) store_flagged_zero(a.fl, a.slotA + blockIdx.x, FA_COUNT); return; }
-        beta = (T)d.beta;
-    } else if (FUSED) {
-        const PreParts pre = prefetch_parts(a.partB + FB_RR * a.strideB, a.partB + (FB_RR + FB_LO) * a.strideB, a.nB, a.esB);
-        PreMax pmax[3] = {{0, 0}, {0, 0}, {0, 0}};
-        if (MSG) {
-#pragma unroll
-            for (int k = 0; k < 3; ++k) pmax[k] = prefetch_max(a.partB + (FB_RMAX + k) * a.strideB, a.nB, a.esB);
-        }
-        const StateLite s = load_state_lite(a.s_in);
-        if (s.done) { if (blockIdx.x == 0 && threadIdx.x == 0) copy_state(a.s_out, a.s_in); return; }
-        MI355CG_WT_STAMP(1)
-        const Decision d = reduce_and_decide(s, a.rp, a.partB, a.nB, a.strideB, a.esB, a.want_diag, lds, &pre, MSG ? pmax : nullptr);
-        MI355CG_WT_STAMP(2)
-        if (blockIdx.x == 0 && threadIdx.x == 0) write_state_after_decision(a.s_out, a.hist, a.s_in, s, d);
-        if (d.done) return;
-        beta = (T)d.beta;
-    }
-
-    MI355CG_WT_MID
+    if (!prologue(beta)) return false;
     const T cA = (T)g.A, cxk = (T)g.xk, cyk = (T)g.yk;
-    dd acc_pap = dd_zero(), acc_rz = dd_zero();
     auto is_ghost = [&](int yy) { return (yy == g.y_lo - 1 || yy == g.y_hi + 1) && yy >= 1 && yy <= g.N - 1; };
     vec_t pn_b, pn_c, r_c;
     T pne_c = (T)0;
@@ -758,6 +737,62 @@
             }
         }
     }
+    return true;
+}
+
+template <typename T, int VEC, bool FUSED, bool MSG, int DEPTH, bool NOAP, bool GC>
+__global__ __launch_bounds__(kBlock) void k_stencil(const StencilArgs<T> a) {
+    __shared__ double lds[2 * kWaves];
+    const int lane = threadIdx.x & (kWave - 1);
+    const int wave = __builtin_amdgcn_readfirstlane(threadIdx.x / kWave);
+    const ItemSeq seq = item_seq(a.wl, wave);
+    MI355CG_WT_BEGIN
+    auto prologue = [&](T& beta) -> bool {
+        if (FUSED && a.src.mbox) {
+            __shared__ double recs[kMaxRecDst * kRecWords];
+            const PreParts pre = prefetch_parts(a.partB + FB_RR * a.strideB, a.partB + (FB_RR + FB_LO) * a.strideB, a.nB, 1);
+            PreMax pmax[3] = {{0, 0}, {0, 0}, {0, 0}};
+            if (MSG) {
+#pragma unroll
+                for (int k = 0; k < 3; ++k) pmax[k] = prefetch_max(a.partB + (FB_RMAX + k) * a.strideB, a.nB, 1);
+            }
+            const StateLite s = load_state_lite(a.s_in);
+            if (s.done) {
+                if (threadIdx.x == 0) { store_flagged_zero(a.fl, a.slotA + blockIdx.x, FA_COUNT); if (blockIdx.x == 0) copy_state(a.s_out, a.s_in); }
+                return false;
+            }
+            MI355CG_WT_STAMP(1)
+            own_record_B(recs, a.src.me, a.partB, a.nB, a.strideB, MSG ? 1 : 0, lds, &pre, MSG ? pmax : nullptr);
+            if (!gather_records(a.src, recs)) {
+                if (threadIdx.x == 0) { store_flagged_zero(a.fl, a.slotA + blockIdx.x, FA_COUNT); if (blockIdx.x == 0) fail_transport(a.s_out, a.s_in); }
+                return false;
+            }
+            const Decision d = decide_from_records(s, a.rp, recs, a.src.world, MSG, false);
+            MI355CG_WT_STAMP(2)
+            if (blockIdx.x == 0 && threadIdx.x == 0) write_state_after_decision(a.s_out, a.hist, a.s_in, s, d);
+            if (d.done) { if (threadIdx.x == 0) store_flagged_zero(a.fl, a.slotA + blockIdx.x, FA_COUNT); return false; }
+            beta = (T)d.beta;
+        } else if (FUSED) {
+            const PreParts pre = prefetch_parts(a.partB + FB_RR * a.strideB, a.partB + (FB_RR + FB_LO) * a.strideB, a.nB, a.esB);
+            PreMax pmax[3] = {{0, 0}, {0, 0}, {0, 0}};
+            if (MSG) {
+#pragma unroll
+                for (int k = 0; k < 3; ++k) pmax[k] = prefetch_max(a.partB + (FB_RMAX + k) * a.strideB, a.nB, a.esB);
+            }
+            const StateLite s = load_state_lite(a.s_in);
+            if (s.done) { if (blockIdx.x == 0 && threadIdx.x == 0) copy_state(a.s_out, a.s_in); return false; }
+            MI355CG_WT_STAMP(1)
+            const Decision d = reduce_and_decide(s, a.rp, a.partB, a.nB, a.strideB, a.esB, a.want_diag, lds, &pre, MSG ? pmax : nullptr);
+            MI355CG_WT_STAMP(2)
+            if (blockIdx.x == 0 && threadIdx.x == 0) write_state_after_decision(a.s_out, a.hist, a.s_in, s, d);
+            if (d.done) return false;
+            beta = (T)d.beta;
+        }
+        MI355CG_WT_MID
+        return true;
+    };
+    dd acc_pap = dd_zero(), acc_rz = dd_zero();
+    if (!stencil_sweep<T, VEC, FUSED, MSG, DEPTH, NOAP, GC>(a, seq, lane, NoRes{}, [] {}, prologue, acc_pap, acc_rz)) return;
 
     MI355CG_WT_END(0);
     const dd tp = block_reduce_dd(acc_pap, lds);
@@ -951,18 +986,14 @@
     QueueSpec dq;
 };
 
-template <typename T, int VEC, int XM, bool HAS_U, int DEPTH, bool DESC>
-__global__ __launch_bounds__(kBlock) void k_update_st(const UpdateStArgs<T> a) {
+struct UpdAcc { dd rr, d2, e2; double rmax, dmax, emax; };
+
+template <typename T, int VEC, int XM, bool HAS_U, int DEPTH, bool DESC, class Res, class Pre, class Pro>
+__device__ inline bool update_sweep(const UpdateStArgs<T>& a, const ItemSeq& seq, const int lane, const Res& res, Pre&& pre, Pro&& prologue, UpdAcc& acc) {
     static_assert(DEPTH >= 1 && DEPTH <= 3, "see k_stencil");
+    static_assert(!Res::on || (VEC == 2 && sizeof(T) == 8), "resident r: fp64 only");
     typedef typename VecOf<T, VEC>::type vec_t;
-    __shared__ double lds[2 * kWaves];
     const Geom& g = a.g;
-    const int lane = threadIdx.x & (kWave - 1);
-    const int wave = __builtin_amdgcn_readfirstlane(threadIdx.x / kWave);
-    const ItemSeq seq = item_seq(a.wl, wave);
-    MI355CG_WT_BEGIN
-    int stop_word = 0;
-    if (blockIdx.x == 0 && a.stop_req) stop_word = scalar_load(a.stop_req);
     constexpr bool FULL = XM == 1;
     constexpr int NP = XM >= 2 ? XM - 1 : 0;
     struct Raw { vec_t p, r, x, u, pp[NP > 0 ? NP : 1]; T pe; };
@@ -1000,7 +1031,13 @@
         const int vown = own ? F.vo_own : kOob;
         Raw w;
         w.p = buf_load<vec_t>(rs_p, vo, f_so);
-        w.r = buf_load<vec_t>(rs_r, vown, f_so);
+        if constexpr (Res::on) {
+            const bool rr = res_row(res, own, f_item, f_y);
+            const vec_t l = *reinterpret_cast<const vec_t*>(res_slot(res, rr, f_y, lane));
+            w.r = buf_load<vec_t>(rs_r, rr ? kOob : vown, f_so);
+#pragma unroll
+            for (int j = 0; j < VEC; ++j) w.r[j] = rr ? l[j] : w.r[j];
+        } else w.r = buf_load<vec_t>(rs_r, vown, f_so);
         if (XM != 0) w.x = buf_load<vec_t>(rs_x, vown, f_so);
 #pragma unroll
         for (int i = 0; i < NP; ++i) w.pp[i] = buf_load<vec_t>(rs_pp[i], vown, f_so);
@@ -1013,13 +1050,13 @@
 
     bool c_have = f_have;
     ItemAddr C{};
-    int c_idx = -1, c_so = 0, c_y = 0;
+    int c_idx = -1, c_so = 0, c_y = 0, c_item = -1;
     bool in_j[VEC];
 #pragma unroll
     for (int j = 0; j < VEC; ++j) in_j[j] = false;
     rsrc_t rs_ro = rs_p, rs_xo = rs_p;
     auto promote = [&]() {
-        C = F;
+        C = F; c_item = f_item;
         rs_ro = make_rsrc(a.r + C.base_el);
         rs_xo = make_rsrc(XM != 0 ? a.x + C.base_el : a.p + C.base_el);
         c_idx = -1; c_so = C.so_c0; c_y = C.ystart;
@@ -1028,61 +1065,18 @@
         for (int j = 0; j < VEC; ++j) in_j[j] = (C.x + j >= xint0) && (C.x + j <= g.N - 1);
     };
 
+    pre();
     if (f_have) { enter(f_item); promote(); }
     Raw q[DEPTH];
 #pragma unroll
     for (int k = 0; k < DEPTH; ++k) q[k] = fetch();
 
-    double alpha_d, rz = 0.0;
-    StateLite s;
-    if (a.src.mbox) {
-        __shared__ double recs[kMaxRecDst * kRecWords];
-        const PreParts pre = prefetch_parts(a.partA + FA_PAP * a.strideA, a.partA + (FA_PAP + FA_LO) * a.strideA, a.nA, 1);
-        PreParts pre_rz{0, 0, 0, 0};
-        if (FULL) pre_rz = prefetch_parts(a.partA + FA_RZ * a.strideA, a.partA + (FA_RZ + FA_LO) * a.strideA, a.nA, 1);
-        s = load_state_lite(a.s_in);
-        if (s.done) {
-            if (threadIdx.x == 0) { store_flagged_zero(a.fl, a.slotB + blockIdx.x, FB_LL_COUNT); if (blockIdx.x == 0) copy_state(a.s_out, a.s_in); }
-            return;
-        }
-        {
-            double* R = recs + a.src.me * kRecWords;
-            if (threadIdx.x < kRecWords) R[threadIdx.x] = 0.0;
-            const dd pap = reduce_parts_dd_pre(pre, a.partA + FA_PAP * a.strideA, a.partA + (FA_PAP + FA_LO) * a.strideA, a.nA, 1, lds);
-            dd rzd = dd_zero();
-            if (a.rule == 0) rzd = FULL ? reduce_parts_dd_pre(pre_rz, a.partA + FA_RZ * a.strideA, a.partA + (FA_RZ + FA_LO) * a.strideA, a.nA, 1, lds)
-                                        : reduce_parts_dd(a.partA + FA_RZ * a.strideA, a.partA + (FA_RZ + FA_LO) * a.strideA, a.nA, 1, lds);
-            __syncthreads();
-            if (threadIdx.x == 0) { R[FA_PAP] = pap.hi; R[FA_PAP + FA_LO] = pap.lo; R[FA_RZ] = rzd.hi; R[FA_RZ + FA_LO] = rzd.lo; }
-        }
-        if (!gather_records(a.src, recs)) {
-            if (threadIdx.x == 0) { store_flagged_zero(a.fl, a.slotB + blockIdx.x, FB_LL_COUNT); if (blockIdx.x == 0) fail_transport(a.s_out, a.s_in); }
-            return;
-        }
-        alpha_from_records(s, a.rule, recs, a.src.world, &alpha_d, &rz);
-    } else {
-        const PreParts pre = prefetch_parts(a.partA + FA_PAP * a.strideA, a.partA + (FA_PAP + FA_LO) * a.strideA, a.nA, a.esA);
-        PreParts pre_rz{0, 0, 0, 0};
-        if (FULL) pre_rz = prefetch_parts(a.partA + FA_RZ * a.strideA, a.partA + (FA_RZ + FA_LO) * a.strideA, a.nA, a.esA);
-        s = load_state_lite(a.s_in);
-        if (s.done) { if (blockIdx.x == 0 && threadIdx.x == 0) copy_state(a.s_out, a.s_in); return; }
-        const double pap = dd_value(reduce_parts_dd_pre(pre, a.partA + FA_PAP * a.strideA, a.partA + (FA_PAP + FA_LO) * a.strideA, a.nA, a.esA, lds));
-        if (a.rule == 0) {
-            rz = FULL ? dd_value(reduce_parts_dd_pre(pre_rz, a.partA + FA_RZ * a.strideA, a.partA + (FA_RZ + FA_LO) * a.strideA, a.nA, a.esA, lds))
-                      : dd_value(reduce_parts_dd(a.partA + FA_RZ * a.strideA, a.partA + (FA_RZ + FA_LO) * a.strideA, a.nA, a.esA, lds));
-            alpha_d = rz / pap;
-        } else {
-            alpha_d = s.rr / pap;
-        }
-    }
-    const T alpha = (T)alpha_d;
-    MI355CG_WT_MID
+    T alpha = (T)0;
     T aprev[NP > 0 ? NP : 1] = {(T)0};
-#pragma unroll
-    for (int i = 0; i < NP; ++i) aprev[i] = (T)scalar_load(&a.s_in->alpha_hist[(s.it - i) & (kRing - 1)]);
+    if (!prologue(alpha, aprev, NP)) return false;
     const T cA = (T)g.A, cxk = (T)g.xk, cyk = (T)g.yk;
-    dd s_rr = dd_zero(), s_d2 = dd_zero(), s_e2 = dd_zero();
-    double s_rmax = 0, s_dmax = 0, s_emax = 0;
+    dd& s_rr = acc.rr; dd& s_d2 = acc.d2; dd& s_e2 = acc.e2;
+    double& s_rmax = acc.rmax; double& s_dmax = acc.dmax; double& s_emax = acc.emax;
     vec_t p_b;
     Raw c;
 #pragma unroll
@@ -1140,7 +1134,11 @@
                             }
                         }
                     }
-                    buf_store(rn, rs_ro, C.vo_own, c_so);
+                    if constexpr (Res::on) {
+                        const bool rr = res_row(res, true, c_item, c_y);
+                        *reinterpret_cast<vec_t*>(res_slot(res, rr, c_y, lane)) = rn;
+                        buf_store(rn, rs_ro, (rr && lane != 0 && lane != kWave - 1) ? kOob : C.vo_own, c_so);
+                    } else buf_store(rn, rs_ro, C.vo_own, c_so);
                     if (XM != 0) buf_store(xn, rs_xo, C.vo_own, c_so);
                     if (DESC) { c_so -= row_step<T>(g, c_y - 1); --c_y; } else { c_so += row_step<T>(g, c_y); ++c_y; }
                     p_b = c.p; c = w;
@@ -1153,7 +1151,75 @@
         }
     }
 
+    return true;
+}
+
+template <typename T, int VEC, int XM, bool HAS_U, int DEPTH, bool DESC>
+__global__ __launch_bounds__(kBlock) void k_update_st(const UpdateStArgs<T> a) {
+    constexpr bool FULL = XM == 1;
+    constexpr int NP = XM >= 2 ? XM - 1 : 0;
+    __shared__ double lds[2 * kWaves];
+    const int lane = threadIdx.x & (kWave - 1);
+    const int wave = __builtin_amdgcn_readfirstlane(threadIdx.x / kWave);
+    const ItemSeq seq = item_seq(a.wl, wave);
+    MI355CG_WT_BEGIN
+    int stop_word = 0;
+    if (blockIdx.x == 0 && a.stop_req) stop_word = scalar_load(a.stop_req);
+    double alpha_d, rz = 0.0;
+    StateLite s;
+    auto prologue = [&](T& alpha, T* aprev, int ) -> bool {
+        if (a.src.mbox) {
+            __shared__ double recs[kMaxRecDst * kRecWords];
+            const PreParts pre = prefetch_parts(a.partA + FA_PAP * a.strideA, a.partA + (FA_PAP + FA_LO) * a.strideA, a.nA, 1);
+            PreParts pre_rz{0, 0, 0, 0};
+            if (FULL) pre_rz = prefetch_parts(a.partA + FA_RZ * a.strideA, a.partA + (FA_RZ + FA_LO) * a.strideA, a.nA, 1);
+            s = load_state_lite(a.s_in);
+            if (s.done) {
+                if (threadIdx.x == 0) { store_flagged_zero(a.fl, a.slotB + blockIdx.x, FB_LL_COUNT); if (blockIdx.x == 0) copy_state(a.s_out, a.s_in); }
+                return false;
+            }
+            {
+                double* R = recs + a.src.me * kRecWords;
+                if (threadIdx.x < kRecWords) R[threadIdx.x] = 0.0;
+                const dd pap = reduce_parts_dd_pre(pre, a.partA + FA_PAP * a.strideA, a.partA + (FA_PAP + FA_LO) * a.strideA, a.nA, 1, lds);
+                dd rzd = dd_zero();
+                if (a.rule == 0) rzd = FULL ? reduce_parts_dd_pre(pre_rz, a.partA + FA_RZ * a.strideA, a.partA + (FA_RZ + FA_LO) * a.strideA, a.nA, 1, lds)
+                                            : reduce_parts_dd(a.partA + FA_RZ * a.strideA, a.partA + (FA_RZ + FA_LO) * a.strideA, a.nA, 1, lds);
+                __syncthreads();
+                if (threadIdx.x == 0) { R[FA_PAP] = pap.hi; R[FA_PAP + FA_LO] = pap.lo; R[FA_RZ] = rzd.hi; R[FA_RZ + FA_LO] = rzd.lo; }
+            }
+            if (!gather_records(a.src, recs)) {
+                if (threadIdx.x == 0) { store_flagged_zero(a.fl, a.slotB + blockIdx.x, FB_LL_COUNT); if (blockIdx.x == 0) fail_transport(a.s_out, a.s_in); }
+                return false;
+            }
+            alpha_from_records(s, a.rule, recs, a.src.world, &alpha_d, &rz);
+        } else {
+            const PreParts pre = prefetch_parts(a.partA + FA_PAP * a.strideA, a.partA + (FA_PAP + FA_LO) * a.strideA, a.nA, a.esA);
+            PreParts pre_rz{0, 0, 0, 0};
+            if (FULL) pre_rz = prefetch_parts(a.partA + FA_RZ * a.strideA, a.partA + (FA_RZ + FA_LO) * a.strideA, a.nA, a.esA);
+            s = load_state_lite(a.s_in);
+            if (s.done) { if (blockIdx.x == 0 && threadIdx.x == 0) copy_state(a.s_out, a.s_in); return false; }
+            const double pap = dd_value(reduce_parts_dd_pre(pre, a.partA + FA_PAP * a.strideA, a.partA + (FA_PAP + FA_LO) * a.strideA, a.nA, a.esA, lds));
+            if (a.rule == 0) {
+                rz = FULL ? dd_value(reduce_parts_dd_pre(pre_rz, a.partA + FA_RZ * a.strideA, a.partA + (FA_RZ + FA_LO) * a.strideA, a.nA, a.esA, lds))
+                          : dd_value(reduce_parts_dd(a.partA + FA_RZ * a.strideA, a.partA + (FA_RZ + FA_LO) * a.strideA, a.nA, a.esA, lds));
+                alpha_d = rz / pap;
+            } else {
+                alpha_d = s.rr / pap;
+            }
+        }
+        alpha = (T)alpha_d;
+        MI355CG_WT_MID
+#pragma unroll
+        for (int i = 0; i < NP; ++i) aprev[i] = (T)scalar_load(&a.s_in->alpha_hist[(s.it - i) & (kRing - 1)]);
+        return true;
+    };
+    UpdAcc acc{dd_zero(), dd_zero(), dd_zero(), 0.0, 0.0, 0.0};
+    if (!update_sweep<T, VEC, XM, HAS_U, DEPTH, DESC>(a, seq, lane, NoRes{}, [] {}, prologue, acc)) return;
+
     MI355CG_WT_END(1);
+    const dd& s_rr = acc.rr; const dd& s_d2 = acc.d2; const dd& s_e2 = acc.e2;
+    const double& s_rmax = acc.rmax; const double& s_dmax = acc.dmax; const double& s_emax = acc.emax;
     const dd t_rr = block_reduce_dd(s_rr, lds);
     const double t_rmax = block_reduce<true>(s_rmax, lds);
     double t_dmax = 0, t_emax = 0; dd t_d2 = dd_zero(), t_e2 = dd_zero();
@@ -1176,6 +1242,200 @@
             o->stop = stop_word != 0;
         }
     }
+}
+
+constexpr int kResWaves = 2 * kWaves, kResBlock = kResWaves * kWave;
+constexpr int kSyncLine = 64;
+constexpr int kSyncTop = kXcds * kSyncLine, kSyncGen = kSyncTop + kSyncLine, kSyncFail = kSyncGen + kXcds * kSyncLine,
+              kSyncStop = kSyncFail + kSyncLine, kSyncWords = kSyncStop + kSyncLine;
+constexpr unsigned long long kResBudget = 1ull << 28;
+
+struct ResidentArgs {
+    Geom g;
+    WorkList wl;
+    double* r; double* x; double* p[kRing];
+    double* partA; double* partB; int nparts, stride;
+    CgState* sA; CgState* sB; HistEntry* hist;
+    RuleParams rp;
+    const int* stop_req;
+    unsigned* sync;
+    int m, cur0;
+    int res_rows;
+};
+
+__device__ inline dd group_reduce_dd(dd v, double* lds) {
+    v = wave_sum_dd(v);
+    const int lane = threadIdx.x & (kWave - 1), w = threadIdx.x / kWave, g0 = w / kWaves * kWaves;
+    __syncthreads();
+    if (lane == 0) { lds[2 * w] = v.hi; lds[2 * w + 1] = v.lo; }
+    __syncthreads();
+    dd t{lds[2 * g0], lds[2 * g0 + 1]};
+#pragma unroll
+    for (int k = 1; k < kWaves; ++k) t = dd_add(t, dd{lds[2 * (g0 + k)], lds[2 * (g0 + k) + 1]});
+    return t;
+}
+__device__ inline double group_reduce_max(double v, double* lds) {
+    v = wave_max(v);
+    const int lane = threadIdx.x & (kWave - 1), w = threadIdx.x / kWave, g0 = w / kWaves * kWaves;
+    __syncthreads();
+    if (lane == 0) lds[w] = v;
+    __syncthreads();
+    double t = lds[g0];
+#pragma unroll
+    for (int k = 1; k < kWaves; ++k) t = fmax(t, lds[g0 + k]);
+    return t;
+}
+__device__ inline dd group_reduce_parts_dd(const double* part_hi, const double* part_lo, int n, double* lds) {
+    dd v = dd_zero();
+    for (int i = threadIdx.x & (kBlock - 1); i < n; i += kBlock) v = dd_add(v, dd{part_hi[i], part_lo[i]});
+    return group_reduce_dd(v, lds);
+}
+
+__device__ inline bool res_barrier(unsigned* sync, unsigned epoch) {
+    asm volatile("s_waitcnt vmcnt(0)" ::: "memory");
+    __syncthreads();
+    int bad = 0;
+    if (threadIdx.x == 0) {
+        const int x = blockIdx.x % kXcds, nx = min(kXcds, (int)gridDim.x), nbx = ((int)gridDim.x - x + kXcds - 1) / kXcds;
+        const unsigned old = __hip_atomic_fetch_add(sync + x * kSyncLine, 1u, __ATOMIC_ACQ_REL, __HIP_MEMORY_SCOPE_AGENT);
+        if (old == epoch * nbx - 1) {
+            const unsigned t = __hip_atomic_fetch_add(sync + kSyncTop, 1u, __ATOMIC_ACQ_REL, __HIP_MEMORY_SCOPE_AGENT);
+            if (t == epoch * nx - 1)
+                for (int k = 0; k < nx; ++k) __hip_atomic_store(sync + kSyncGen + k * kSyncLine, epoch, __ATOMIC_RELEASE, __HIP_MEMORY_SCOPE_AGENT);
+        }
+        const unsigned long long t0 = wall_clock64();
+        unsigned spins = 0;
+        while (__hip_atomic_load(sync + kSyncGen + x * kSyncLine, __ATOMIC_RELAXED, __HIP_MEMORY_SCOPE_AGENT) < epoch) {
+            __builtin_amdgcn_s_sleep(1);
+            if ((++spins & 63u) == 0 && (__hip_atomic_load(sync + kSyncFail, __ATOMIC_RELAXED, __HIP_MEMORY_SCOPE_AGENT) != 0 ||
+                                         wall_clock64() - t0 > kResBudget)) {
+                __hip_atomic_store(sync + kSyncFail, 1u, __ATOMIC_RELAXED, __HIP_MEMORY_SCOPE_AGENT);
+                bad = 1;
+                break;
+            }
+        }
+        __builtin_amdgcn_fence(__ATOMIC_ACQUIRE, "agent");
+    }
+    bad = __syncthreads_or(bad);
+    __builtin_amdgcn_fence(__ATOMIC_ACQUIRE, "workgroup");
+    return bad == 0;
+}
+
+__device__ inline void res_copy(const Geom& g, double* r, const LdsRes& res, int x, int lane, bool to_lds) {
+    typedef VecOf<double, 2>::type v2;
+    for (int k = 0; k < res.n; ++k) {
+        const int y = res.y0 + k;
+        const bool in = lane_off<double>(g, x, y <= g.half) != kOob;
+        v2* gp = reinterpret_cast<v2*>(r + (row_off(g, y) - g.base0 + x));
+        v2* lp = reinterpret_cast<v2*>(res.slots + k * (2 * kWave) + 2 * lane);
+        if (to_lds) { v2 v = {0.0, 0.0}; if (in) v = *gp; *lp = v; }
+        else if (in) *gp = *lp;
+    }
+}
+
+__global__ __launch_bounds__(kResBlock) void k_cg_resident(const ResidentArgs a) {
+    typedef double T;
+    extern __shared__ double res_lds[];
+    __shared__ double lds[2 * kResWaves];
+    __shared__ CgState stA, stB;
+    const int lane = threadIdx.x & (kWave - 1);
+    const int wave = __builtin_amdgcn_readfirstlane(threadIdx.x / kWave);
+    const int grp = wave / kWaves, vblock = (int)blockIdx.x + grp * (int)gridDim.x;
+    const bool grp_lead = (threadIdx.x & (kBlock - 1)) == 0 && vblock < a.nparts;
+    ItemSeq seq = item_seq(a.wl, wave % kWaves, min(vblock, a.nparts - 1), a.nparts);
+    if (vblock >= a.nparts) seq.first = seq.end;
+    const bool lead = blockIdx.x == 0 && threadIdx.x == 0;
+
+    LdsRes res{res_lds + 2 * kWave + wave * a.res_rows * (2 * kWave), res_lds, -1, 0, 0};
+    int res_x = 0;
+    if (seq.first < seq.end && a.res_rows > 0) {
+        const Item it = decode_item(a.wl, seq.first);
+        res.item = seq.first; res.y0 = it.ya + 1; res.n = max(0, min(a.res_rows, it.yb - it.ya - 1));
+        res_x = it.strip * (2 * kWave) + 2 * lane;
+    }
+    res_copy(a.g, a.r, res, res_x, lane, true);
+
+    StateLite s = load_state_lite(a.sB);
+    T a1 = scalar_load(&a.sB->alpha_hist[s.it & (kRing - 1)]), a2 = scalar_load(&a.sB->alpha_hist[(s.it - 1) & (kRing - 1)]),
+      a3 = scalar_load(&a.sB->alpha_hist[(s.it - 2) & (kRing - 1)]);
+    if (lead) { stB = *a.sB; stA = stB; }
+
+    StencilArgs<T> sa{};
+    sa.g = a.g; sa.wl = a.wl; sa.r = a.r;
+    UpdateStArgs<T> ua{};
+    ua.g = a.g; ua.wl = a.wl; ua.r = a.r; ua.x = a.x; ua.rule = 1; ua.reverse = 0;
+
+    int cur = a.cur0;
+    unsigned epoch = 0;
+    bool ok = true, done = s.done != 0;
+    for (int k = 0; k < a.m && ok && !done; ++k) {
+        sa.pin = a.p[cur]; sa.pout = a.p[(cur + 1) & 3];
+        auto preA = [&] { if (k > 0) ok = res_barrier(a.sync, ++epoch); };
+        auto proA = [&](T& beta) -> bool {
+            if (!ok) return false;
+            if (k > 0) s.stop = (int)__hip_atomic_load(a.sync + kSyncStop, __ATOMIC_RELAXED, __HIP_MEMORY_SCOPE_AGENT);
+            const double rr = dd_value(group_reduce_parts_dd(a.partB + FB_RR * a.stride, a.partB + (FB_RR + FB_LO) * a.stride, a.nparts, lds));
+            const Decision d = decide_after_update(s, a.rp, rr, 0, 0, 0, 0, 0);
+            if (lead) { stA = stB; apply_decision(&stA, a.hist, s, d); }
+            s.rr_prev = s.rr; s.rr = d.rr; s.r0norm = d.r0norm;
+            if (d.done) { done = true; return false; }
+            beta = d.beta;
+            return true;
+        };
+        dd pap = dd_zero(), rzs = dd_zero();
+        if (!stencil_sweep<T, 2, true, false, 3, true, false>(sa, seq, lane, res, preA, proA, pap, rzs)) break;
+        {
+            const dd tp = group_reduce_dd(pap, lds);
+            if (grp_lead) {
+                const int b = vblock, st = a.stride;
+                a.partA[FA_PAP * st + b] = tp.hi; a.partA[(FA_PAP + FA_LO) * st + b] = tp.lo;
+                a.partA[FA_RZ * st + b] = 0.0;    a.partA[(FA_RZ + FA_LO) * st + b] = 0.0;
+            }
+        }
+        cur = (cur + 1) & 3;
+
+        int stop_word = 0;
+        double alpha_d = 0.0;
+        ua.p = a.p[cur];
+#pragma unroll
+        for (int i = 0; i < 3; ++i) ua.pprev[i] = a.p[(cur + 3 - i) & 3];
+        auto preB = [&] { ok = res_barrier(a.sync, ++epoch); };
+        auto proB = [&](T& alpha, T* ap, int np) -> bool {
+            if (!ok) return false;
+            if (lead && a.stop_req) stop_word = __hip_atomic_load(a.stop_req, __ATOMIC_RELAXED, __HIP_MEMORY_SCOPE_SYSTEM);
+            const double pap_t = dd_value(group_reduce_parts_dd(a.partA + FA_PAP * a.stride, a.partA + (FA_PAP + FA_LO) * a.stride, a.nparts, lds));
+            alpha_d = s.rr / pap_t;
+            alpha = alpha_d;
+            if (np == 3) { ap[0] = a1; ap[1] = a2; ap[2] = a3; }
+            return true;
+        };
+        UpdAcc acc{dd_zero(), dd_zero(), dd_zero(), 0.0, 0.0, 0.0};
+        const bool ran = cur == 0 ? update_sweep<T, 2, 4, false, 3, true>(ua, seq, lane, res, preB, proB, acc)
+                                  : update_sweep<T, 2, 0, false, 3, true>(ua, seq, lane, res, preB, proB, acc);
+        if (!ran) break;
+        {
+            const dd t_rr = group_reduce_dd(acc.rr, lds);
+            const double t_rmax = group_reduce_max(acc.rmax, lds);
+            if (grp_lead) {
+                const int b = vblock, st = a.stride;
+                a.partB[FB_RR * st + b] = t_rr.hi; a.partB[(FB_RR + FB_LO) * st + b] = t_rr.lo;
+                a.partB[FB_D2 * st + b] = 0.0; a.partB[(FB_D2 + FB_LO) * st + b] = 0.0;
+                a.partB[FB_E2 * st + b] = 0.0; a.partB[(FB_E2 + FB_LO) * st + b] = 0.0;
+                a.partB[FB_RMAX * st + b] = t_rmax; a.partB[FB_DMAX * st + b] = 0.0; a.partB[FB_EMAX * st + b] = 0.0;
+            }
+        }
+        if (lead) {
+            stB = stA;
+            stB.it = s.it + 1; stB.first = 0; stB.alpha = alpha_d; stB.rz = 0.0; stB.alpha_hist[(s.it + 1) & (kRing - 1)] = alpha_d;
+            stB.stop = stop_word != 0;
+            __hip_atomic_store(a.sync + kSyncStop, (unsigned)(stop_word != 0), __ATOMIC_RELAXED, __HIP_MEMORY_SCOPE_AGENT);
+        }
+        s.it += 1; s.first = 0; s.alpha = alpha_d; s.rz = 0.0;
+        a3 = a2; a2 = a1; a1 = alpha_d;
+    }
+
+    res_copy(a.g, a.r, res, res_x, lane, false);
+    if (lead) { *a.sA = stA; *a.sB = done ? stA : stB; }
 }
 
 struct CheckArgs {
diff --git a/iterative_solvers_amd/csrc/mi355cg.hip b/iterative_solvers_amd/csrc/mi355cg.hip
--- a/iterative_solvers_amd/csrc/mi355cg.hip
+++ b/iterative_solvers_amd/csrc/mi355cg.hip
@@ -110,6 +110,16 @@
     mi355cg_params graph_prm{};
     bool graph_stop = false;
     int use_graph = -1;
+
+    int resident = -1;
+    int res_kib = 0;
+    int res_grid = 0;
+    int res_rows = 0;
+    long long res_cells = 0;
+    bool res_auto_ok = false;
+    bool res_refused = false;
+    unsigned* res_sync = nullptr;
+    unsigned* res_fail_h = nullptr;
 
     hipEvent_t ev_loop[2] = {nullptr, nullptr};
     bool profiling = false;
@@ -235,6 +245,7 @@
     return pl;
 }
 constexpr int kMaxRowsF64 = 800, kMaxRowsF32 = 64;
+constexpr bool kResidentAuto = false;
 
 void build_plans(mi355cg_ctx* c) {
     const Geom& g = c->g;
@@ -384,6 +395,75 @@
     a.partB = pb.ptr; a.nB = pb.n; a.strideB = pb.fstride; a.esB = pb.estride; a.src = pb.rec;
     a.s_in = c->sB; a.summary = c->summary; a.hist = c->hist; a.rp = cfg.rp; a.want_diag = cfg.want_diag;
     hipLaunchKernelGGL(k_check, dim3(1), dim3(kBlock), 0, stream, a);
+}
+
+int setup_resident(mi355cg_ctx* c) {
+    const char* mode = getenv("MI355CG_RESIDENT");
+    c->resident = (!mode || !*mode || !strcmp(mode, "auto")) ? -1 : (atoi(mode) != 0 ? 1 : 0);
+    c->res_kib = std::max(0, std::min(159, env_int("MI355CG_RESIDENT_KIB", 152)));
+    c->res_grid = 0;
+    if (c->resident == 0 || c->xsteps != 4 || c->whole.wl.nitems == 0) return MI355CG_OK;
+    int cus = 0, per_cu = 0;
+    HIPCK(hipDeviceGetAttribute(&cus, hipDeviceAttributeMultiprocessorCount, c->device));
+    c->res_rows = c->res_kib > 0 ? (c->res_kib - 1) / kResWaves : 0;
+    const size_t lds = c->res_rows > 0 ? (size_t)(1 + kResWaves * c->res_rows) * 1024 : 0;
+    HIPCK(hipFuncSetAttribute((const void*)k_cg_resident, hipFuncAttributeMaxDynamicSharedMemorySize, (int)lds));
+    HIPCK(hipOccupancyMaxActiveBlocksPerMultiprocessor(&per_cu, k_cg_resident, kResBlock, lds));
+    const int grid = (c->whole.grid + 1) / 2;
+    if (per_cu < 1 || grid > cus) return MI355CG_OK;
+    HIPCK(hipMalloc((void**)&c->res_sync, sizeof(unsigned) * kSyncWords));
+    HIPCK(hipHostMalloc((void**)&c->res_fail_h, sizeof(unsigned)));
+    *c->res_fail_h = 0;
+    c->res_grid = grid;
+    c->res_cells = 0;
+    const WorkList& wl = c->whole.wl;
+    for (int gi = 0; gi < c->whole.grid; ++gi) for (int w = 0; w < kWaves; ++w) {
+        int first = gi * kWaves + w;
+        if (wl.ncls == kXcds) {
+            const int cls = gi % kXcds;
+            first = wl.cls0[cls] + gi / kXcds * kWaves + w;
+            if (first >= wl.cls0[cls + 1]) continue;
+        } else if (first >= wl.nitems) continue;
+        const Panel* P = &wl.p[0];
+        for (int k = 1; k < wl.np; ++k) if (first >= wl.p[k].item0) P = &wl.p[k];
+        const int local = first - P->item0, chunk = local / P->ns, ya = P->y0 + chunk * P->ty, yb = std::min(P->y1, ya + P->ty - 1);
+        const int n = std::max(0, std::min(c->res_rows, yb - ya - 1));
+        int xa = 0, xb = 0;
+        own_cols(c, ya + 1, &xa, &xb);
+        const int x0 = std::max(xa, (P->s0 + local % P->ns) * kStripCols), x1 = std::min(xb, (P->s0 + local % P->ns + 1) * kStripCols);
+        c->res_cells += (long long)n * std::max(0, x1 - x0);
+    }
+    const bool knob = getenv("MI355CG_ITEM_ROWS") || getenv("MI355CG_DEPTH") || getenv("MI355CG_BLOCKS") || getenv("MI355CG_WAVES") ||
+                      getenv("MI355CG_XSTEPS") || getenv("MI355CG_XCD_CLASSES") || getenv("MI355CG_DYN_ROWS");
+    c->res_auto_ok = kResidentAuto && !knob;
+    return MI355CG_OK;
+}
+bool use_resident(const mi355cg_ctx* c, const IterCfg& cfg) {
+    if (c->res_grid == 0 || c->res_refused || !cfg.x2 || c->profiling || c->dtype != MI355CG_F64) return false;
+    return c->resident == 1 || (c->resident < 0 && c->res_auto_ok);
+}
+int launch_resident(mi355cg_ctx* c, const IterCfg& cfg, int m, bool* refused) {
+    *refused = false;
+    ResidentArgs a{};
+    a.g = kernel_geom<double, 2>(c); a.wl = c->whole.wl;
+    a.r = c->r; a.x = c->x;
+    for (int i = 0; i < kRing; ++i) a.p[i] = c->p[i];
+    a.partA = c->partA; a.partB = c->partB; a.nparts = c->whole.grid; a.stride = c->strideA;
+    a.sA = c->sA; a.sB = c->sB; a.hist = c->hist; a.rp = cfg.rp;
+    a.stop_req = c->stop_dev; a.sync = c->res_sync;
+    a.m = m; a.cur0 = c->cur; a.res_rows = c->res_rows;
+    HIPCK(hipMemsetAsync(c->res_sync, 0, sizeof(unsigned) * kSyncWords, c->stream));
+    void* args[] = {&a};
+    const size_t lds = c->res_rows > 0 ? (size_t)(1 + kResWaves * c->res_rows) * 1024 : 0;
+    const hipError_t e = hipLaunchCooperativeKernel((const void*)k_cg_resident, dim3(c->res_grid), dim3(kResBlock), args, lds, c->stream);
+    if (e == hipErrorCooperativeLaunchTooLarge || e == hipErrorNotSupported || e == hipErrorInvalidConfiguration) {
+        (void)hipGetLastError();
+        c->res_refused = true;
+        *refused = true;
+        return MI355CG_OK;
+    }
+    HIPCK(e);
+    return MI355CG_OK;
 }
 
 IterCfg make_cfg(const mi355cg_params* prm) {
@@ -789,6 +869,7 @@
     if (hipMalloc((void**)&c->qctr, sizeof(int) * 2 * kXcds * kQueueSubs * kQueuePitch) != hipSuccess || hipMemset(c->qctr, 0, sizeof(int) * 2 * kXcds * kQueueSubs * kQueuePitch) != hipSuccess) { rc = fail(MI355CG_ERR_HIP, "queue counter allocation failed"); return cleanup(); }
     if (hipHostMalloc((void**)&c->stop_h, sizeof(int)) != hipSuccess) { rc = fail(MI355CG_ERR_HIP, "stop word allocation failed"); return cleanup(); }
     *c->stop_h = 0;
+    if (!part && dtype == MI355CG_F64) if ((rc = setup_resident(c))) return cleanup();
     HIPCK(hipDeviceSynchronize());
 
     if (env_int("MI355CG_DEVICE_SETUP", 0)) {
@@ -890,7 +971,7 @@
     if (c->stream) hipStreamSynchronize(c->stream);
     void* dev[] = {c->x, c->r, c->p[0], c->p[1], c->p[2], c->p[3], c->p[4], c->p[5], c->p[6], c->p[7], c->ap, c->b, c->u, c->scratch[0], c->scratch[1], c->xf, c->rf,
                    c->pf[0], c->pf[1], c->pf[2], c->pf[3], c->pf[4], c->pf[5], c->pf[6], c->pf[7], c->apf,
-                   c->packed, c->partA, c->partB, c->partR, c->sumsA, c->sumsB, c->sA, c->sB, c->summary, c->hist, c->qctr};
+                   c->packed, c->partA, c->partB, c->partR, c->sumsA, c->sumsB, c->sA, c->sB, c->summary, c->hist, c->qctr, c->res_sync};
     for (void* p : dev) if (p) hipFree(p);
     if (c->csr_row_map) hipFree(c->csr_row_map);
     if (c->csr_entries) hipFree(c->csr_entries);
@@ -899,6 +980,7 @@
     if (c->hist_h) hipHostFree(c->hist_h);
     if (c->partR_h) hipHostFree(c->partR_h);
     if (c->stop_h) hipHostFree(c->stop_h);
+    if (c->res_fail_h) hipHostFree(c->res_fail_h);
     clear_graphs(c);
     c->events.destroy();
     for (hipEvent_t e : c->ev_loop) if (e) hipEventDestroy(e);
@@ -1040,11 +1122,16 @@
         }
         return MI355CG_OK;
     };
+    const bool resident = use_resident(c, cfg);
+    bool res_ran = false;
     auto poll = [&]() -> int {
         launch_check(c, cfg, c->stream, own_partB(c));
         HIPCK(hipMemcpyAsync(c->summary_h, c->summary, sizeof(CgState), hipMemcpyDeviceToHost, c->stream));
         HIPCK(hipMemcpyAsync(c->hist_h, c->hist, sizeof(HistEntry) * kHist, hipMemcpyDeviceToHost, c->stream));
-        return wait_stream();
+        if (res_ran) HIPCK(hipMemcpyAsync(c->res_fail_h, c->res_sync + kSyncFail, sizeof(unsigned), hipMemcpyDeviceToHost, c->stream));
+        if (int rc = wait_stream()) return rc;
+        if (res_ran && *c->res_fail_h) return fail(MI355CG_ERR_STATE, "resident launch: a grid barrier gave up waiting (the workgroups were not all resident)");
+        return MI355CG_OK;
     };
     *c->summary_h = CgState{};
     if (msg && cb) {
@@ -1064,7 +1151,7 @@
     if (std::memcmp(&c->graph_prm, prm, sizeof *prm) != 0 || c->graph_stop != (stop_flag != nullptr)) {
         clear_graphs(c); c->graph_prm = *prm; c->graph_stop = stop_flag != nullptr;
     }
-    const bool graph_ok = !c->profiling && !diag &&
+    const bool graph_ok = !resident && !c->profiling && !diag &&
                           (c->use_graph == 1 || (c->use_graph < 0 && c->g.own_len < (4LL << 20) && prm->max_iterations >= 4 * sync_every));
     while (!c->summary_h->done) {
         if (stop_flag && *stop_flag) { interrupted = true; break; }
@@ -1092,29 +1179,36 @@
             }
             return MI355CG_OK;
         };
-        if (graph_ok && m >= 8) {
-            std::vector<char> flags(m);
-            for (int k = 0; k < m; ++k) flags[k] = cfg.has_u && need_u(it_done + k + 1);
-            mi355cg_ctx::ChunkGraph* hit = nullptr;
-            for (auto& g : c->graphs) if (g.m == m && g.cur == c->cur && g.flags == flags) hit = &g;
-            if (!hit) {
-                hipGraph_t graph = nullptr; hipGraphExec_t exec = nullptr;
-                const int cur0 = c->cur;
-                HIPCK(hipStreamBeginCapture(c->stream, hipStreamCaptureModeThreadLocal));
-                const int rc = enqueue_chunk();
-                const hipError_t e1 = hipStreamEndCapture(c->stream, &graph);
-                c->cur = cur0;
-                if (rc) return rc;
-                HIPCK(e1);
-                HIPCK(hipGraphInstantiate(&exec, graph, nullptr, nullptr, 0));
-                HIPCK(hipGraphDestroy(graph));
-                c->graphs.push_back({m, cur0, flags, exec});
-                hit = &c->graphs.back();
+        bool refused = true;
+        if (resident && !c->res_refused) {
+            if (int rc = launch_resident(c, cfg, m, &refused)) return rc;
+            if (!refused) { c->cur = (c->cur + m) % c->xsteps; res_ran = true; }
+        }
+        if (refused) {
+            if (graph_ok && m >= 8) {
+                std::vector<char> flags(m);
+                for (int k = 0; k < m; ++k) flags[k] = cfg.has_u && need_u(it_done + k + 1);
+                mi355cg_ctx::ChunkGraph* hit = nullptr;
+                for (auto& g : c->graphs) if (g.m == m && g.cur == c->cur && g.flags == flags) hit = &g;
+                if (!hit) {
+                    hipGraph_t graph = nullptr; hipGraphExec_t exec = nullptr;
+                    const int cur0 = c->cur;
+                    HIPCK(hipStreamBeginCapture(c->stream, hipStreamCaptureModeThreadLocal));
+                    const int rc = enqueue_chunk();
+                    const hipError_t e1 = hipStreamEndCapture(c->stream, &graph);
+                    c->cur = cur0;
+                    if (rc) return rc;
+                    HIPCK(e1);
+                    HIPCK(hipGraphInstantiate(&exec, graph, nullptr, nullptr, 0));
+                    HIPCK(hipGraphDestroy(graph));
+                    c->graphs.push_back({m, cur0, flags, exec});
+                    hit = &c->graphs.back();
+                }
+                HIPCK(hipGraphLaunch(hit->exec, c->stream));
+                c->cur = (c->cur + m) % c->xsteps;
+            } else {
+                if (int rc = enqueue_chunk()) return rc;
             }
-            HIPCK(hipGraphLaunch(hit->exec, c->stream));
-            c->cur = (c->cur + m) % c->xsteps;
-        } else {
-            if (int rc = enqueue_chunk()) return rc;
         }
         HIPCK(hipGetLastError());
         if (int rc = poll()) return rc;
@@ -1208,6 +1302,14 @@
     if (!c || kernel < 0 || kernel > 1) return fail(MI355CG_ERR_INVALID, "bad argument");
     if (avg_ms) *avg_ms = c->kernel_ms[kernel];
     if (launches) *launches = c->kernel_launches[kernel];
+    return MI355CG_OK;
+}
+int mi355cg_get_resident(mi355cg_handle c, int* active, int* grid, int* rows_per_wave, long long* resident_cells) {
+    if (!c || !active || !grid || !rows_per_wave || !resident_cells) return fail(MI355CG_ERR_INVALID, "null argument");
+    IterCfg cfg{};
+    cfg.x2 = true;
+    *active = !c->is_csr && !c->is_slab && use_resident(c, cfg) ? 1 : 0;
+    *grid = c->res_grid; *rows_per_wave = c->res_rows; *resident_cells = c->res_cells;
     return MI355CG_OK;
 }
 int mi355cg_get_layout(mi355cg_handle c, long long* padded_len, int* pitch_bottom, int* pitch_upper,
diff --git a/iterative_solvers_amd/solver.py b/iterative_solvers_amd/solver.py
--- a/iterative_solvers_amd/solver.py
+++ b/iterative_solvers_amd/solver.py
@@ -124,6 +124,12 @@
         ms, n = C.c_double(), C.c_longlong()
         _capi.check(self._lib.mi355cg_get_kernel_time(self._h, kernel, C.byref(ms), C.byref(n)))
         return ms.value, n.value
+
+    def resident(self):
+        v = [C.c_int() for _ in range(3)]
+        cells = C.c_longlong()
+        _capi.check(self._lib.mi355cg_get_resident(self._h, *[C.byref(i) for i in v], C.byref(cells)))
+        return {"active": bool(v[0].value), "grid": v[1].value, "rows_per_wave": v[2].value, "resident_cells": cells.value}
 
     def layout(self):
         L = C.c_longlong()
```

Result: no change. 7187 iters/s, median of 3 (-0.2%).
